# bioinformatics-ua/polus

Measured on AMD Instinct MI355X. Metric: train samples/sec BioBERT-base NER seq256, higher is better.
Workload: dtype bf16; 1 GPU; BERT-base (L=12,H=768,A=12,I=3072,V=28996) token classification C=4, seq_len=256, 64 samples/GPU, AdamW lr 5e-5 wd 0.01 warm-up 10%, dropout 0.1 (hidden + attention) (BASELINE.json configs[2] per-GPU shape), random-init weights; global_batch=64, seq_len=256, parallelism=dp1, grad_allreduce=none

## Files before the change

### include/polus_hip.h

```cpp
#ifndef POLUS_HIP_H
#define POLUS_HIP_H

#include <stddef.h>
#include <stdint.h>

#ifdef __cplusplus
extern "C" {
#endif

#define POLUS_ABI_VERSION 1

enum { POLUS_OK = 0, POLUS_ERR_INVALID = 1, POLUS_ERR_HIP = 2, POLUS_ERR_WORKSPACE = 3 };
enum { POLUS_F32 = 0, POLUS_BF16 = 1 };
enum { POLUS_K_CONTIG = 0, POLUS_K_STRIDED = 1 };
enum { POLUS_ACT_NONE = 0, POLUS_ACT_GELU = 1, POLUS_ACT_SWISH = 2, POLUS_ACT_RELU = 3, POLUS_ACT_TANH = 4 };
enum {
    POLUS_GEMM_ACCUM_C = 1,
    POLUS_GEMM_ACT_FWD = 2,
    POLUS_GEMM_ACT_BWD = 4,
    POLUS_GEMM_DROPOUT = 8
};

const char* polus_last_error(void);
int polus_abi_version(void);
int polus_device_info(int* n_cu, int* lds_bytes_per_cu, char* arch, int arch_len);
int polus_reload_env(void);
int polus_set_reserve_active(int on);
int polus_set_dynamic_params(const void* dev_block16);

size_t polus_gemm_workspace_bytes(int M, int N, int split_k);
int polus_gemm_auto_split(int M, int N, int K);
int polus_gemm(int dtype, int a_layout, int b_layout, int c_dtype,
               const void* A, long lda, const void* B, long ldb, void* C, long ldc,
               int M, int N, int K, float alpha,
               const float* bias, const void* resid, long ldr, void* aux, long ldaux,
               int act, int flags, int split_k, void* workspace, size_t workspace_bytes,
               void* stream);

int polus_gemm_dropout(int dtype, int a_layout, int b_layout, int c_dtype,
                       const void* A, long lda, const void* B, long ldb, void* C, long ldc,
                       int M, int N, int K, float alpha,
                       const float* bias, const void* resid, long ldr, void* aux, long ldaux,
                       int act, int flags, int split_k, void* workspace, size_t workspace_bytes,
                       float drop_p, uint32_t seed, void* stream);
int polus_dropout(int dtype, const void* x, void* y, int64_t n, float drop_p, uint32_t seed, void* stream);
int polus_dropout_mask(uint32_t seed, float drop_p, uint32_t idx0, int64_t n, uint8_t* mask, void* stream);

size_t polus_dense_bwd_params_workspace_bytes(int T, int n_out, int n_in, int split_k);
int polus_dense_bwd_params(int dtype, const void* dY, long lddy, const void* X, long ldx,
                           float* dW, long lddw, float* db, int T, int n_out, int n_in,
                           int accumulate, int split_k, void* workspace, size_t workspace_bytes,
                           void* stream);

typedef struct polus_dw_problem {
    const void* dY; long lddy;
    const void* X;  long ldx;
    float* dW; long lddw;
    float* db;
    int n_out, n_in;
} polus_dw_problem;
size_t polus_dense_bwd_params_grouped_workspace_bytes(int n, const polus_dw_problem* problems, int T, int split_k);
int polus_dense_bwd_params_grouped(int dtype, int n, const polus_dw_problem* problems, int T, int accumulate,
                                   int split_k, void* workspace, size_t workspace_bytes, void* stream);

int polus_dense_thin_supported(int dtype, int H, int C);
int polus_dense_thin_fwd(int dtype, const void* x, long ldx, const void* W, long ldw, const float* bias,
                         int y_dtype, void* y, long ldy, int rows, int H, int C, void* stream);
size_t polus_dense_thin_bwd_workspace_bytes(int dtype, int rows, int H, int C);
int polus_dense_thin_bwd(int dtype, const void* x, long ldx, int dy_dtype, const void* dy, long lddy,
                         const void* W, long ldw, void* dx, long lddx, float* dW, long lddw, float* db,
                         int rows, int H, int C, int accumulate, void* workspace, size_t workspace_bytes, void* stream);

int polus_attention_route(int dtype, int S, int* fwd, int* bwd);
int polus_attention_fwd(int dtype, const void* qkv, const int32_t* mask, void* ctx, float* lse,
                        int B, int S, int n_heads, int head_dim, float drop_p, uint32_t seed, void* stream);
size_t polus_attention_bwd_workspace_bytes(int B, int S, int n_heads);
int polus_attention_bwd(int dtype, const void* qkv, const int32_t* mask, const void* ctx,
                        const void* dctx, const float* lse, void* dqkv,
                        int B, int S, int n_heads, int head_dim, float drop_p, uint32_t seed,
                        void* workspace, size_t workspace_bytes, void* stream);

size_t polus_layernorm_bwd_workspace_bytes(int rows, int H);
int polus_layernorm_fwd(int dtype, const void* x, const float* gamma, const float* beta,
                        void* y, float* mean, float* rstd, int rows, int H, float eps, void* stream);
int polus_layernorm_bwd(int dtype, const void* dy, const void* x, const float* gamma,
                        const float* mean, const float* rstd, void* dx,
                        float* dgamma, float* dbeta, float* dbias, int accumulate,
                        int rows, int H, void* dx_masked, float drop_p, uint32_t seed,
                        void* workspace, size_t workspace_bytes, void* stream);
int polus_layernorm_bwd_finalize(void* workspace, size_t workspace_bytes, int rows, int H, float* dgamma, float* dbeta,
                                 float* dbias, int accumulate, void* stream);

size_t polus_embed_bwd_workspace_bytes(int B, int S, int H);
int polus_embed_ln_fwd(int dtype, const int32_t* ids, const int32_t* type_ids,
                       const float* word, const float* pos, const float* type,
                       const float* gamma, const float* beta, void* y, float* mean, float* rstd,
                       int B, int S, int H, int vocab, int max_pos, int type_vocab, float eps,
                       float drop_p, uint32_t seed, void* stream);
int polus_embed_ln_bwd(int dtype, const void* dy, const int32_t* ids, const int32_t* type_ids,
                       const float* word, const float* pos, const float* type, const float* gamma,
                       const float* mean, const float* rstd,
                       float* gword, float* gpos, float* gtype, float* ggamma, float* gbeta,
                       int accumulate, int deterministic,
                       int B, int S, int H, int vocab, int max_pos, int type_vocab,
                       float drop_p, uint32_t seed,
                       void* workspace, size_t workspace_bytes, void* stream);

size_t polus_colsum_workspace_bytes(int rows, int cols);
int polus_colsum(int dtype, const void* x, long ldx, int rows, int cols, float* out, int accumulate,
                 void* workspace, size_t workspace_bytes, void* stream);

size_t polus_loss_workspace_bytes(int rows);
int polus_softmax_xent(int dtype, const float* logits, long ldl, const int32_t* labels,
                       const float* class_weights, float* loss, void* dlogits, long lddl,
                       int rows, int C, void* workspace, size_t workspace_bytes, void* stream);
int polus_sigmoid_xent(int dtype, const float* logits, long ldl, const float* y_true, long ldy,
                       const float* class_weights, float negative_weight, float* loss,
                       void* dlogits, long lddl, int rows, int C,
                       void* workspace, size_t workspace_bytes, void* stream);

size_t polus_crf_workspace_bytes(int B, int S, int C);
int polus_crf_nll(int dtype, const float* potentials, const int32_t* tags, const int32_t* lengths,
                  const float* trans, const float* sample_w, float* loss, void* dpot,
                  float* dtrans, int accumulate, int B, int S, int C,
                  void* workspace, size_t workspace_bytes, void* stream);
int polus_crf_viterbi(const float* potentials, const int32_t* lengths, const float* trans,
                      int32_t* out_tags, int B, int S, int C,
                      void* workspace, size_t workspace_bytes, void* stream);

int polus_maxsim_fwd(int dtype, const void* Q, const void* D, const int32_t* qmask, const int32_t* dmask,
                     float* score, long lds, int32_t* argmax, int B, int N, int Lq, int Ld, int E, void* stream);
int polus_maxsim_scores(int dtype, const void* Q, const void* D, const int32_t* qmask, const int32_t* dmask,
                        float* score, long lds, int B, int N, int Lq, int Ld, int E, void* stream);
int polus_maxsim_bwd(int dtype, const void* Q, const void* D, const float* dscore, long lds,
                     const int32_t* argmax, void* dQ, void* dD, int B, int N, int Lq, int Ld, int E, void* stream);
int polus_maxsim_rerank(int dtype, const void* Q, const void* D, const int32_t* qmask, const int32_t* dmask,
                        const int32_t* cand, long ldc, float* score, long lds,
                        int B, int C, int N, int Lq, int Ld, int E, void* stream);
int polus_l2norm_fwd(int dtype, const void* x, void* y, float* rnorm, int rows, int E, float eps, void* stream);
int polus_l2norm_bwd(int dtype, const void* y, const float* rnorm, const void* dy, void* dx, int rows, int E,
                     float eps, void* stream);

int polus_topk_merge(const float* scores, long lds, int rows, int n, int32_t id0,
                     float* top_val, int32_t* top_id, int k, int init, void* stream);
int polus_topk_merge_ids(const float* scores, long lds, const int32_t* ids, long ldi, int rows, int n,
                         float* top_val, int32_t* top_id, int k, int init, void* stream);

int polus_argmax(const float* x, long ldx, int32_t* out, int rows, int C, void* stream);

int polus_confusion_matrix(const int32_t* row_idx, const int32_t* col_idx, int64_t n, int C,
                           int32_t* cm, int32_t* rejected, void* stream);

int polus_bio_entity_counts(const int32_t* tags_a, long lda, const int32_t* tags_b, long ldb,
                            const int32_t* mask, long ldm, const int32_t* scheme, int C, int T, int B, int S,
                            int32_t* counts, int32_t* stats, void* stream);
int polus_bio_spans(const int32_t* tags, long ldt, const int32_t* mask, long ldm, const int32_t* scheme, int C,
                    int B, int S, int32_t* spans, int M, int32_t* count, int32_t* rejected, void* stream);

int polus_adam_step(float* p, const float* g, float* m, float* v, void* shadow_bf16,
                    const int64_t* seg, int n_seg, int64_t n,
                    float lr, float lr_t, float beta1, float beta2, float eps, float weight_decay,
                    float grad_scale, const float* clip_scale, void* stream);
size_t polus_sqnorm_workspace_bytes(int64_t n);
int polus_sqnorm(const float* g, int64_t n, float* out, void* workspace, size_t workspace_bytes, void* stream);
int polus_sqnorm_segments(const float* g, const int64_t* seg, int n_seg, float* out,
                          void* workspace, size_t workspace_bytes, void* stream);
int polus_clip_scale(const float* sqnorm, int n_terms, float grad_scale, float clip_norm, float* out_scale, void* stream);
int polus_cast(int src_dtype, const void* src, int dst_dtype, void* dst, int64_t n, void* stream);
int polus_transpose_bf16(const void* src, void* dst, int rows, int cols, void* stream);
int polus_transpose_bf16_batched(const void* src_base, void* dst_base, const void* segs_dev, int nseg,
                                 int total_tiles, void* stream);
int polus_act_bwd(int dtype, const void* dy, const void* u, void* du, int64_t n, int act, void* stream);
int polus_scale(float* x, float a, int64_t n, void* stream);

#define POLUS_COMM_ID_BYTES 128
int polus_comm_unique_id(void* out_id128);
int polus_comm_init(void** comm, int rank, int world, const void* unique_id128);
int polus_comm_destroy(void* comm);
int polus_comm_info(void* comm, int* n_ranks, int* rank, int* device);
int polus_comm_broadcast(void* comm, void* buf, size_t bytes, int root, void* stream);
int polus_comm_allreduce_sum(void* comm, void* buf, size_t count, int dtype, void* stream);
int polus_comm_reduce_scatter_sum(void* comm, const void* send, void* recv, size_t recv_count, int dtype, void* stream);
int polus_comm_all_gather(void* comm, const void* send, void* recv, size_t send_count, int dtype, void* stream);
int polus_comm_group_start(void);
int polus_comm_group_end(void);

#ifdef __cplusplus
}
#endif
#endif
```

### polus_amd/_lib.py

```python
import ctypes
import os

from . import build as _build

F32, BF16 = 0, 1
K_CONTIG, K_STRIDED = 0, 1
ACT_NONE, ACT_GELU, ACT_SWISH, ACT_RELU, ACT_TANH = 0, 1, 2, 3, 4
GEMM_ACCUM_C, GEMM_ACT_FWD, GEMM_ACT_BWD = 1, 2, 4

_c = ctypes
_vp, _i, _l, _f, _sz, _i64, _u32 = _c.c_void_p, _c.c_int, _c.c_long, _c.c_float, _c.c_size_t, _c.c_int64, _c.c_uint32

SIGNATURES = {
    "polus_last_error": (_c.c_char_p, []),
    "polus_abi_version": (_i, []),
    "polus_device_info": (_i, [_c.POINTER(_i), _c.POINTER(_i), _c.c_char_p, _i]),
    "polus_reload_env": (_i, []),
    "polus_set_reserve_active": (_i, [_i]),
    "polus_set_dynamic_params": (_i, [_vp]),
    "polus_gemm_workspace_bytes": (_sz, [_i, _i, _i]),
    "polus_gemm_auto_split": (_i, [_i, _i, _i]),
    "polus_gemm": (_i, [_i, _i, _i, _i, _vp, _l, _vp, _l, _vp, _l, _i, _i, _i, _f,
                        _vp, _vp, _l, _vp, _l, _i, _i, _i, _vp, _sz, _vp]),
    "polus_gemm_dropout": (_i, [_i, _i, _i, _i, _vp, _l, _vp, _l, _vp, _l, _i, _i, _i, _f,
                                _vp, _vp, _l, _vp, _l, _i, _i, _i, _vp, _sz, _f, _u32, _vp]),
    "polus_dropout_mask": (_i, [_u32, _f, _u32, _i64, _vp, _vp]),
    "polus_dropout": (_i, [_i, _vp, _vp, _i64, _f, _u32, _vp]),
    "polus_dense_bwd_params_workspace_bytes": (_sz, [_i, _i, _i, _i]),
    "polus_dense_bwd_params": (_i, [_i, _vp, _l, _vp, _l, _vp, _l, _vp, _i, _i, _i, _i, _i, _vp, _sz, _vp]),
    "polus_attention_route": (_i, [_i, _i, _c.POINTER(_i), _c.POINTER(_i)]),
    "polus_attention_fwd": (_i, [_i, _vp, _vp, _vp, _vp, _i, _i, _i, _i, _f, _u32, _vp]),
    "polus_attention_bwd_workspace_bytes": (_sz, [_i, _i, _i]),
    "polus_attention_bwd": (_i, [_i, _vp, _vp, _vp, _vp, _vp, _vp, _i, _i, _i, _i, _f, _u32, _vp, _sz, _vp]),
    "polus_layernorm_bwd_workspace_bytes": (_sz, [_i, _i]),
    "polus_layernorm_fwd": (_i, [_i, _vp, _vp, _vp, _vp, _vp, _vp, _i, _i, _f, _vp]),
    "polus_layernorm_bwd": (_i, [_i, _vp, _vp, _vp, _vp, _vp, _vp, _vp, _vp, _vp, _i, _i, _i, _vp, _f, _u32, _vp, _sz, _vp]),
    "polus_layernorm_bwd_finalize": (_i, [_vp, _sz, _i, _i, _vp, _vp, _vp, _i, _vp]),
    "polus_embed_bwd_workspace_bytes": (_sz, [_i, _i, _i]),
    "polus_embed_ln_fwd": (_i, [_i, _vp, _vp, _vp, _vp, _vp, _vp, _vp, _vp, _vp, _vp,
                                _i, _i, _i, _i, _i, _i, _f, _f, _u32, _vp]),
    "polus_embed_ln_bwd": (_i, [_i, _vp, _vp, _vp, _vp, _vp, _vp, _vp, _vp, _vp,
                                _vp, _vp, _vp, _vp, _vp, _i, _i,
                                _i, _i, _i, _i, _i, _i, _f, _u32, _vp, _sz, _vp]),
    "polus_colsum_workspace_bytes": (_sz, [_i, _i]),
    "polus_colsum": (_i, [_i, _vp, _l, _i, _i, _vp, _i, _vp, _sz, _vp]),
    "polus_loss_workspace_bytes": (_sz, [_i]),
    "polus_softmax_xent": (_i, [_i, _vp, _l, _vp, _vp, _vp, _vp, _l, _i, _i, _vp, _sz, _vp]),
    "polus_sigmoid_xent": (_i, [_i, _vp, _l, _vp, _l, _vp, _f, _vp, _vp, _l, _i, _i, _vp, _sz, _vp]),
    "polus_crf_workspace_bytes": (_sz, [_i, _i, _i]),
    "polus_crf_nll": (_i, [_i, _vp, _vp, _vp, _vp, _vp, _vp, _vp, _vp, _i, _i, _i, _i, _vp, _sz, _vp]),
    "polus_crf_viterbi": (_i, [_vp, _vp, _vp, _vp, _i, _i, _i, _vp, _sz, _vp]),
    "polus_confusion_matrix": (_i, [_vp, _vp, _i64, _i, _vp, _vp, _vp]),
    "polus_bio_entity_counts": (_i, [_vp, _l, _vp, _l, _vp, _l, _vp, _i, _i, _i, _i, _vp, _vp, _vp]),
    "polus_bio_spans": (_i, [_vp, _l, _vp, _l, _vp, _i, _i, _i, _vp, _i, _vp, _vp, _vp]),
    "polus_maxsim_fwd": (_i, [_i, _vp, _vp, _vp, _vp, _vp, _l, _vp, _i, _i, _i, _i, _i, _vp]),
    "polus_maxsim_scores": (_i, [_i, _vp, _vp, _vp, _vp, _vp, _l, _i, _i, _i, _i, _i, _vp]),
    "polus_maxsim_rerank": (_i, [_i, _vp, _vp, _vp, _vp, _vp, _l, _vp, _l, _i, _i, _i, _i, _i, _i, _vp]),
    "polus_maxsim_bwd": (_i, [_i, _vp, _vp, _vp, _l, _vp, _vp, _vp, _i, _i, _i, _i, _i, _vp]),
    "polus_l2norm_fwd": (_i, [_i, _vp, _vp, _vp, _i, _i, _f, _vp]),
    "polus_l2norm_bwd": (_i, [_i, _vp, _vp, _vp, _vp, _i, _i, _f, _vp]),
    "polus_topk_merge": (_i, [_vp, _l, _i, _i, _c.c_int32, _vp, _vp, _i, _i, _vp]),
    "polus_topk_merge_ids": (_i, [_vp, _l, _vp, _l, _i, _i, _vp, _vp, _i, _i, _vp]),
    "polus_argmax": (_i, [_vp, _l, _vp, _i, _i, _vp]),
    "polus_adam_step": (_i, [_vp, _vp, _vp, _vp, _vp, _vp, _i, _i64,
                             _f, _f, _f, _f, _f, _f, _f, _vp, _vp]),
    "polus_sqnorm_workspace_bytes": (_sz, [_i64]),
    "polus_sqnorm": (_i, [_vp, _i64, _vp, _vp, _sz, _vp]),
    "polus_sqnorm_segments": (_i, [_vp, _vp, _i, _vp, _vp, _sz, _vp]),
    "polus_clip_scale": (_i, [_vp, _i, _f, _f, _vp, _vp]),
    "polus_cast": (_i, [_i, _vp, _i, _vp, _i64, _vp]),
    "polus_scale": (_i, [_vp, _f, _i64, _vp]),
    "polus_act_bwd": (_i, [_i, _vp, _vp, _vp, _i64, _i, _vp]),
    "polus_transpose_bf16": (_i, [_vp, _vp, _i, _i, _vp]),
    "polus_transpose_bf16_batched": (_i, [_vp, _vp, _vp, _i, _i, _vp]),
    "polus_dense_bwd_params_grouped_workspace_bytes": (_sz, [_i, _vp, _i, _i]),
    "polus_dense_bwd_params_grouped": (_i, [_i, _i, _vp, _i, _i, _i, _vp, _sz, _vp]),
    "polus_dense_thin_supported": (_i, [_i, _i, _i]),
    "polus_dense_thin_fwd": (_i, [_i, _vp, _l, _vp, _l, _vp, _i, _vp, _l, _i, _i, _i, _vp]),
    "polus_dense_thin_bwd_workspace_bytes": (_sz, [_i, _i, _i, _i]),
    "polus_dense_thin_bwd": (_i, [_i, _vp, _l, _i, _vp, _l, _vp, _l, _vp, _l, _vp, _l, _vp, _i, _i, _i, _i, _vp, _sz, _vp]),
    "polus_comm_unique_id": (_i, [_vp]),
    "polus_comm_init": (_i, [_c.POINTER(_vp), _i, _i, _vp]),
    "polus_comm_destroy": (_i, [_vp]),
    "polus_comm_info": (_i, [_vp, _c.POINTER(_i), _c.POINTER(_i), _c.POINTER(_i)]),
    "polus_comm_broadcast": (_i, [_vp, _vp, _sz, _i, _vp]),
    "polus_comm_allreduce_sum": (_i, [_vp, _vp, _sz, _i, _vp]),
    "polus_comm_reduce_scatter_sum": (_i, [_vp, _vp, _vp, _sz, _i, _vp]),
    "polus_comm_all_gather": (_i, [_vp, _vp, _vp, _sz, _i, _vp]),
    "polus_comm_group_start": (_i, []),
    "polus_comm_group_end": (_i, []),
}


class DwProblem(ctypes.Structure):
    _fields_ = [("dY", ctypes.c_void_p), ("lddy", ctypes.c_long), ("X", ctypes.c_void_p), ("ldx", ctypes.c_long),
                ("dW", ctypes.c_void_p), ("lddw", ctypes.c_long), ("db", ctypes.c_void_p),
                ("n_out", ctypes.c_int), ("n_in", ctypes.c_int)]


class PolusHipError(RuntimeError):
    pass


_LIB = None


def load():
    global _LIB
    if _LIB is not None:
        return _LIB
    path = _build.lib_path()
    if not os.path.exists(path):
        raise PolusHipError(
            f"{path} is missing: build it with `python -m polus_amd.build` "
            "(or __graft_entry__.build()). There is no CPU fallback for the training path.")
    import torch
    bundled = os.path.join(os.path.dirname(torch.__file__), "lib", "libamdhip64.so")
    if os.path.exists(bundled):
        ctypes.CDLL(bundled, mode=ctypes.RTLD_GLOBAL)
    lib = ctypes.CDLL(path)
    for name, (res, args) in SIGNATURES.items():
        fn = getattr(lib, name)
        fn.restype = res
        fn.argtypes = args
    if lib.polus_abi_version() != 1:
        raise PolusHipError("libpolus_hip.so ABI version mismatch")
    _LIB = lib
    return lib


def check(rc, what=""):
    if rc != 0:
        msg = load().polus_last_error()
        raise PolusHipError(f"{what} failed (code {rc}): {msg.decode() if msg else ''}")


def ptr(t):
    return None if t is None else t.data_ptr()


_CUR_STREAM = [None]


def current_stream():
    h = _CUR_STREAM[0]
    if h is not None:
        return h
    import torch
    return torch.cuda.current_stream().cuda_stream


class pinned_stream:

    def __enter__(self):
        import torch
        self._prev = _CUR_STREAM[0]
        if self._prev is None and torch.cuda.is_available():
            _CUR_STREAM[0] = torch.cuda.current_stream().cuda_stream
        return self

    def __exit__(self, *exc):
        _CUR_STREAM[0] = self._prev
        return False


class stream_scope:

    def __init__(self, stream):
        import torch
        self._stream = stream
        self._ctx = torch.cuda.stream(stream)

    def __enter__(self):
        self._prev = _CUR_STREAM[0]
        self._ctx.__enter__()
        if self._prev is not None:
            _CUR_STREAM[0] = self._stream.cuda_stream
        return self

    def __exit__(self, *exc):
        _CUR_STREAM[0] = self._prev
        return self._ctx.__exit__(*exc)


def dtype_code(torch_dtype):
    import torch
    if torch_dtype == torch.float32:
        return F32
    if torch_dtype == torch.bfloat16:
        return BF16
    raise PolusHipError(f"unsupported dtype {torch_dtype}")
```

### polus_amd/csrc/gemm.hip

```cpp
#include <stdlib.h>
#include "gemm_common.h"

using namespace pgemm;

namespace {

constexpr int BM = 128, BN = 128, NTHREADS = 256;
constexpr int KC_STRIDE = 160;
constexpr int OPERAND_BYTES = 128 * KC_STRIDE;
constexpr int SMEM_BYTES = 4 * OPERAND_BYTES;

template <typename T> struct Cfg;
template <> struct Cfg<bf16_t> {
    static constexpr int BK = 64, EPC = 8, NSUB = 2;
    static constexpr int KS_STRIDE = 288, KS_SWZ = 7, LOG_RCH = 4;
};
template <> struct Cfg<float> {
    static constexpr int BK = 32, EPC = 4, NSUB = 1;
    static constexpr int KS_STRIDE = 512, KS_SWZ = 6, LOG_RCH = 5;
};

typedef unsigned int u32x4_t __attribute__((ext_vector_type(4)));
template <typename T> union Chunk { uint4 u; u32x4_t w; T e[16 / sizeof(T)]; };

// ... 374 lines not shown
                     const float* bias, const void* resid, long ldr, void* aux, long ldaux,
                     int act, int flags, int split_k, void* workspace, size_t workspace_bytes,
                     float drop_p, uint32_t seed, void* stream) {
    POLUS_REQUIRE(dtype == POLUS_F32 || dtype == POLUS_BF16, "polus_gemm: bad dtype %d", dtype);
    POLUS_REQUIRE(c_dtype == POLUS_F32 || c_dtype == dtype, "polus_gemm: c_dtype must be f32 or dtype");
    POLUS_REQUIRE(M > 0 && N > 0 && K > 0, "polus_gemm: empty problem M=%d N=%d K=%d", M, N, K);
    POLUS_REQUIRE(A && B && C, "polus_gemm: null operand");
    POLUS_REQUIRE((a_layout | 1) == 1 && (b_layout | 1) == 1, "polus_gemm: bad layout");
    POLUS_REQUIRE(lda >= (a_layout == POLUS_K_CONTIG ? K : M), "polus_gemm: lda %ld too small", lda);
    POLUS_REQUIRE(ldb >= (b_layout == POLUS_K_CONTIG ? K : N), "polus_gemm: ldb %ld too small", ldb);
    POLUS_REQUIRE(ldc >= N, "polus_gemm: ldc %ld < N %d", ldc, N);
    POLUS_REQUIRE(!resid || ldr >= N, "polus_gemm: ldr too small");
    POLUS_REQUIRE(!((flags & POLUS_GEMM_ACT_BWD) && !aux), "polus_gemm: ACT_BWD needs aux");
    POLUS_REQUIRE(!aux || ldaux >= N, "polus_gemm: ldaux too small");
    if (split_k < 1) split_k = 1;
    const size_t es = polus_dtype_size(dtype), ecs = polus_dtype_size(c_dtype);
    const int bk = dtype == POLUS_BF16 ? 64 : 32;
    const int nkt = (K + bk - 1) / bk;
    if (split_k > nkt) split_k = nkt;
    const bool both_kc = a_layout == POLUS_K_CONTIG && b_layout == POLUS_K_CONTIG;
    if (split_k > 1) {
        const bool epi = resid || aux || (flags & (POLUS_GEMM_ACT_FWD | POLUS_GEMM_ACT_BWD | POLUS_GEMM_DROPOUT));
        POLUS_REQUIRE(!epi || (dtype == POLUS_BF16 && c_dtype == POLUS_BF16 && both_kc && !(flags & POLUS_GEMM_ACCUM_C)),
                      "polus_gemm: split_k with a residual / activation / dropout epilogue needs bf16 K-contiguous operands and a bf16 C");
        if (!workspace || workspace_bytes < polus_gemm_workspace_bytes(M, N, split_k)) {
            polus_set_error("polus_gemm: workspace %zu < %zu", workspace_bytes, polus_gemm_workspace_bytes(M, N, split_k));
            return POLUS_ERR_WORKSPACE;
        }
    }
    POLUS_REQUIRE(!(flags & POLUS_GEMM_DROPOUT) || (both_kc && c_dtype == dtype), "polus_gemm_dropout: needs K-contiguous operands and c_dtype == dtype");
    GemmArgs a = {};
    a.A = A; a.B = B; a.C = C; a.lda = lda; a.ldb = ldb; a.ldc = ldc;
    a.M = M; a.N = N; a.K = K; a.alpha = alpha;
    a.bias = bias; a.resid = resid; a.ldr = ldr; a.aux = aux; a.ldaux = ldaux;
    a.act = act; a.flags = flags;
    a.drop_inv = 1.0f / (1.0f - drop_p); a.drop_thresh = polus_drop_thresh(drop_p); a.drop_seed = seed;
    a.dyn = polus_dyn();
    const int epc = (int)(16 / es);
    a.a_vec = polus_aligned16(A) && ((lda * es) % 16 == 0) && ((a_layout == POLUS_K_CONTIG ? K : M) % epc == 0);
    a.b_vec = polus_aligned16(B) && ((ldb * es) % 16 == 0) && ((b_layout == POLUS_K_CONTIG ? K : N) % epc == 0);
    bool ev = (((uintptr_t)C) % (4 * ecs) == 0) && (ldc % 4 == 0);
    if (bias) ev = ev && (((uintptr_t)bias) % 16 == 0);
    if (resid) ev = ev && (((uintptr_t)resid) % (4 * es) == 0) && (ldr % 4 == 0);
    if (aux) ev = ev && (((uintptr_t)aux) % (4 * es) == 0) && (ldaux % 4 == 0);
    a.epi_vec = ev;
    bool ev16 = (((uintptr_t)C) % 16 == 0) && ((ldc * ecs) % 16 == 0);
    if (bias) ev16 = ev16 && (((uintptr_t)bias) % 16 == 0);
    if (resid) ev16 = ev16 && (((uintptr_t)resid) % 16 == 0) && ((ldr * es) % 16 == 0);
    if (aux) ev16 = ev16 && (((uintptr_t)aux) % 16 == 0) && ((ldaux * es) % 16 == 0);
    a.epi_vec16 = ev16 && dtype == POLUS_BF16;
    a.order = polus_cfg().gemm_order;

    const int kt_per_split = (nkt + split_k - 1) / split_k;
    const bool c_is_f32 = c_dtype == POLUS_F32;
    const int a_ks = a_layout == POLUS_K_STRIDED, b_ks = b_layout == POLUS_K_STRIDED;
    const GemmRoute r = gemm_route(a, dtype, c_is_f32, a_ks, b_ks, (nkt + kt_per_split - 1) / kt_per_split);
    if (r.splits > 1) { a.k_per_split = kt_per_split * bk; a.partial = static_cast<float*>(workspace); }
    else a.k_per_split = r.kernel == GEMM_V1 ? nkt * bk : ((K + 31) / 32) * 32;

    hipStream_t st = static_cast<hipStream_t>(stream);
    int rc = POLUS_ERR_INVALID;
    switch (r.kernel) {
        case GEMM_V1: rc = launch_v1(dtype, c_dtype, a_layout, b_layout, a, r.drop, r.splits, st); break;
        case GEMM_RING:
            rc = r.splits > 1 ? polus_launch_gemm_ring(slab_args(a), 1, a_ks, b_ks, r.splits, -1, st)
                              : polus_launch_gemm_ring(a, c_is_f32, a_ks, b_ks, 1, r.mode, st);
            break;
        case GEMM_RING128: rc = polus_launch_gemm_ring128(a, r.mode, r.drop, st); break;
        case GEMM_RING_DROP: rc = polus_launch_gemm_ring_dropout(a, r.mode, st); break;
        case GEMM_PP:
        case GEMM_PP_PERSIST: rc = polus_launch_gemm_pp(a, r.mode, r.drop, r.tn, r.persist_cus, st); break;
    }
    if (rc != POLUS_OK) return rc;
    switch (r.reduce) {
        case REDUCE_NONE: break;
        case REDUCE_EPI: return launch_splitk_reduce_epi(a, r.splits, st);
        case REDUCE_PLAIN:
            return launch_splitk_reduce(c_dtype, a.partial, r.splits, M, N, C, ldc, alpha, bias, (flags & POLUS_GEMM_ACCUM_C) ? 1 : 0,
                                        "polus_gemm(splitk_reduce)", st);
    }
    return POLUS_OK;
}

extern "C" int polus_gemm(int dtype, int a_layout, int b_layout, int c_dtype,
                          const void* A, long lda, const void* B, long ldb, void* C, long ldc,
                          int M, int N, int K, float alpha,
                          const float* bias, const void* resid, long ldr, void* aux, long ldaux,
                          int act, int flags, int split_k, void* workspace, size_t workspace_bytes,
                          void* stream) {
    POLUS_REQUIRE(!(flags & POLUS_GEMM_DROPOUT), "polus_gemm: use polus_gemm_dropout for POLUS_GEMM_DROPOUT");
    return gemm_impl(dtype, a_layout, b_layout, c_dtype, A, lda, B, ldb, C, ldc, M, N, K, alpha, bias, resid, ldr,
                     aux, ldaux, act, flags, split_k, workspace, workspace_bytes, 0.0f, 0u, stream);
}

extern "C" int polus_gemm_dropout(int dtype, int a_layout, int b_layout, int c_dtype,
                                  const void* A, long lda, const void* B, long ldb, void* C, long ldc,
                                  int M, int N, int K, float alpha,
                                  const float* bias, const void* resid, long ldr, void* aux, long ldaux,
                                  int act, int flags, int split_k, void* workspace, size_t workspace_bytes,
                                  float drop_p, uint32_t seed, void* stream) {
    POLUS_REQUIRE(drop_p >= 0.0f && drop_p < 1.0f, "polus_gemm_dropout: need 0 <= p < 1 (got %f)", drop_p);
    POLUS_REQUIRE((long)M * N < (1LL << 32), "polus_gemm_dropout: M*N must fit 32 bits");
    if (drop_p > 0.0f) flags |= POLUS_GEMM_DROPOUT; else flags &= ~POLUS_GEMM_DROPOUT;
    return gemm_impl(dtype, a_layout, b_layout, c_dtype, A, lda, B, ldb, C, ldc, M, N, K, alpha, bias, resid, ldr,
                     aux, ldaux, act, flags, split_k, workspace, workspace_bytes, drop_p, seed, stream);
}

extern "C" size_t polus_dense_bwd_params_workspace_bytes(int T, int n_out, int n_in, int split_k) {
    if (split_k < 1) split_k = 1;
    size_t slabs = split_k > 1 ? (size_t)split_k * n_out * n_in * sizeof(float) : 0;
    size_t cs = (size_t)split_k * n_out * sizeof(float);
    size_t fallback = polus_colsum_workspace_bytes(T, n_out);
    return slabs + (cs > fallback ? cs : fallback) + 256;
}

namespace {
__global__ void colsum_splits_kernel(const float* __restrict__ partial, int splits, int n, float* __restrict__ out, int accumulate) {
    int c = blockIdx.x * blockDim.x + threadIdx.x;
    if (c >= n) return;
    float s = 0.f;
    for (int z = 0; z < splits; ++z) s += partial[(long)z * n + c];
    out[c] = accumulate ? out[c] + s : s;
}
}

static int launch_colsum_splits(const float* partial, int splits, int n, float* out, int accumulate, const char* what, hipStream_t st) {
    hipLaunchKernelGGL(colsum_splits_kernel, dim3((n + 255) / 256), dim3(256), 0, st, partial, splits, n, out, accumulate);
    POLUS_CHECK_LAUNCH(what);
    return POLUS_OK;
}

static GemmArgs dw_args(const polus_dw_problem& q, int T, int kps, float* colsum) {
    GemmArgs a = {};
    a.A = q.dY; a.B = q.X; a.lda = q.lddy; a.ldb = q.ldx;
    a.M = q.n_out; a.N = q.n_in; a.K = T; a.alpha = 1.0f;
    a.k_per_split = kps;
    a.a_vec = a.b_vec = 1;
    a.colsum_a = colsum;
    return a;
}
static void dw_dest(GemmArgs& a, const polus_dw_problem& q, void* slabs, int accumulate) {
    if (slabs) {
        a.C = slabs; a.ldc = q.n_in; a.c_split_stride = (long)q.n_out * q.n_in;
        a.epi_vec = a.epi_vec16 = (q.n_in % 4 == 0);
    } else {
        a.C = q.dW; a.ldc = q.lddw; a.flags = accumulate ? POLUS_GEMM_ACCUM_C : 0;
        a.epi_vec = a.epi_vec16 = polus_aligned16(q.dW) && (q.lddw % 4 == 0);
    }
}

extern "C" int polus_dense_bwd_params(int dtype, const void* dY, long lddy, const void* X, long ldx,
                                      float* dW, long lddw, float* db, int T, int n_out, int n_in,
                                      int accumulate, int split_k, void* workspace, size_t workspace_bytes,
                                      void* stream) {
    POLUS_REQUIRE(dY && X && dW, "polus_dense_bwd_params: null pointer");
    POLUS_REQUIRE(T > 0 && n_out > 0 && n_in > 0, "polus_dense_bwd_params: bad shape");
    if (split_k < 1) split_k = 1;
    size_t need = polus_dense_bwd_params_workspace_bytes(T, n_out, n_in, split_k);
    if (!workspace || workspace_bytes < need) { polus_set_error("polus_dense_bwd_params: workspace %zu < %zu", workspace_bytes, need); return POLUS_ERR_WORKSPACE; }
    hipStream_t st = static_cast<hipStream_t>(stream);
    const size_t es = polus_dtype_size(dtype);
    const int bk = dtype == POLUS_BF16 ? 64 : 32;
    int nkt = (T + bk - 1) / bk;
    if (split_k > nkt) split_k = nkt;
    const size_t slab_bytes = split_k > 1 ? (((size_t)split_k * n_out * n_in * sizeof(float) + 255) / 256) * 256 : 0;
    unsigned char* ws = static_cast<unsigned char*>(workspace);
    float* cs_ws = reinterpret_cast<float*>(ws + slab_bytes);
    const bool vec = polus_aligned16(dY) && polus_aligned16(X) && ((lddy * es) % 16 == 0) && ((ldx * es) % 16 == 0) &&
                     (n_out % (16 / es) == 0) && (n_in % (16 / es) == 0);
    const bool ring = dtype == POLUS_BF16 && vec && n_out >= 256 && n_in >= 128 && db != nullptr && !polus_cfg().gemm_v1;
    if (!ring) {
        int rc = polus_gemm(dtype, POLUS_K_STRIDED, POLUS_K_STRIDED, POLUS_F32, dY, lddy, X, ldx, dW, lddw, n_out, n_in, T,
                            1.0f, nullptr, nullptr, 0, nullptr, 0, 0, accumulate ? POLUS_GEMM_ACCUM_C : 0, split_k,
                            ws, slab_bytes, stream);
        if (rc != POLUS_OK || !db) return rc;
        return polus_colsum(dtype, dY, lddy, T, n_out, db, accumulate, cs_ws, workspace_bytes - slab_bytes, stream);
    }
    const polus_dw_problem q = {dY, lddy, X, ldx, dW, lddw, db, n_out, n_in};
    const int kt_per_split = (nkt + split_k - 1) / split_k;
    const int splits = (nkt + kt_per_split - 1) / kt_per_split;
    GemmArgs a = dw_args(q, T, kt_per_split * bk, cs_ws);
    dw_dest(a, q, splits > 1 ? ws : nullptr, accumulate);
    int rc = polus_launch_gemm_ring(a, 1, 1, 1, splits, -1, st);
    if (rc != POLUS_OK) return rc;
    if (splits > 1) {
        rc = launch_splitk_reduce(POLUS_F32, reinterpret_cast<const float*>(ws), splits, n_out, n_in, dW, lddw, 1.0f, nullptr,
                                  accumulate ? 1 : 0, "polus_dense_bwd_params(reduce)", st);
        if (rc != POLUS_OK) return rc;
    }
    return launch_colsum_splits(cs_ws, splits, n_out, db, accumulate ? 1 : 0, "polus_dense_bwd_params(colsum)", st);
}

static bool grouped_use_pp(int n, const polus_dw_problem* pr, int T) {
    if (polus_cfg().gemm_pp < 0 || T % 64 != 0) return false;
    for (int k = 0; k < n; ++k)
        if (pr[k].n_out < 256 || pr[k].n_in < 256) return false;
    return true;
}

static bool grouped_sk_plan(int n, const polus_dw_problem* pr, int T, int split_k, bool pp, PPKSSKPlan* pl) {
    if (!polus_cfg().dw_streamk || split_k > 0 || !pp) return false;
    int no[POLUS_MAX_GROUP], ni[POLUS_MAX_GROUP];
    for (int k = 0; k < n; ++k) { no[k] = pr[k].n_out; ni[k] = pr[k].n_in; }
    int ncu = polus_num_cus() - polus_reserved_cus();
    if (polus_cfg().dw_sk_cus > 0 && polus_cfg().dw_sk_cus < ncu) ncu = polus_cfg().dw_sk_cus;
    return polus_ppks_sk_plan(no, ni, n, T, ncu, polus_cfg().dw_sk_delta, pl) != 0;
}

static void grouped_splits(int n, const polus_dw_problem* pr, int T, int split_k, int* splits, bool pp) {
    const int nkt = (T + 63) / 64;
    int tiles[POLUS_MAX_GROUP], total = 0;
    for (int k = 0; k < n; ++k) {
        tiles[k] = pp ? polus_ppks_tiles(pr[k].n_out, pr[k].n_in) : ((pr[k].n_out + 255) / 256) * ((pr[k].n_in + 127) / 128);
        total += tiles[k];
    }
    if (split_k > 0) {
        for (int k = 0; k < n; ++k) splits[k] = split_k < nkt ? split_k : nkt;
        return;
    }
    const int slots_xcd = (pp ? 1 : 2) * polus_num_cus() / 8;
    int per_xcd[POLUS_MAX_GROUP], total_xcd = 0;
    for (int k = 0; k < n; ++k) { per_xcd[k] = (tiles[k] + 7) / 8; total_xcd += per_xcd[k]; }
    int base = slots_xcd / (total_xcd > 0 ? total_xcd : 1);
    if (base < 1) base = 1;
    const int cap = nkt / 4 > 0 ? nkt / 4 : 1;
    if (base > cap) base = cap;
    int used = 0;
    for (int k = 0; k < n; ++k) { splits[k] = base; used += per_xcd[k] * base; }
    bool given[POLUS_MAX_GROUP] = {false};
    for (;;) {
        int best = -1;
        for (int k = 0; k < n; ++k)
            if (!given[k] && splits[k] < cap && used + per_xcd[k] <= slots_xcd && (best < 0 || tiles[k] > tiles[best])) best = k;
        if (best < 0) break;
        given[best] = true; ++splits[best]; used += per_xcd[best];
    }
}

struct GroupedDwPlan {
    bool pp, sk;
    int splits[POLUS_MAX_GROUP];
    int kps[POLUS_MAX_GROUP], eff[POLUS_MAX_GROUP];
    size_t slab_off[POLUS_MAX_GROUP], cs_off[POLUS_MAX_GROUP];
    PPKSSKPlan skp;
    size_t sk_cs_off[POLUS_MAX_GROUP];
    size_t bytes;
};

static void grouped_dw_plan(int n, const polus_dw_problem* pr, int T, int split_k, GroupedDwPlan* pl) {
    pl->pp = grouped_use_pp(n, pr, T);
    grouped_splits(n, pr, T, split_k, pl->splits, pl->pp);
    const int nkt = (T + 63) / 64;
    size_t off = 0, single = 0;
    for (int k = 0; k < n; ++k) {
        const int sk = pl->splits[k] > nkt ? nkt : pl->splits[k];
        pl->kps[k] = ((nkt + sk - 1) / sk) * 64;
        pl->eff[k] = (nkt + (pl->kps[k] / 64) - 1) / (pl->kps[k] / 64);
        pl->slab_off[k] = off;
        if (pl->splits[k] > 1) off += (((size_t)pl->splits[k] * pr[k].n_out * pr[k].n_in * sizeof(float) + 255) / 256) * 256;
        pl->cs_off[k] = off;
        off += (((size_t)pl->splits[k] * pr[k].n_out * sizeof(float) + 255) / 256) * 256;
        const size_t b = polus_dense_bwd_params_workspace_bytes(T, pr[k].n_out, pr[k].n_in, pl->splits[k]);
        if (b > single) single = b;
    }
    pl->bytes = off + 256;
    pl->sk = grouped_sk_plan(n, pr, T, split_k, pl->pp, &pl->skp);
    if (pl->sk) {
        off = (size_t)pl->skp.ttot * pl->skp.slots * 256 * 256 * sizeof(float);
        for (int k = 0; k < n; ++k) {
            pl->sk_cs_off[k] = off;
            off += (((size_t)pl->skp.slots * pr[k].n_out * sizeof(float) + 255) / 256) * 256;
        }
        if (off + 256 > pl->bytes) pl->bytes = off + 256;
    }
    if (single > pl->bytes) pl->bytes = single;
}

extern "C" size_t polus_dense_bwd_params_grouped_workspace_bytes(int n, const polus_dw_problem* problems, int T, int split_k) {
    if (n < 1 || n > POLUS_MAX_GROUP || !problems || T < 1) return 0;
    GroupedDwPlan pl;
    grouped_dw_plan(n, problems, T, split_k, &pl);
    return pl.bytes;
}

struct DwGroupOut {
    const float* slabs[POLUS_MAX_GROUP]; float* cs[POLUS_MAX_GROUP];
    float* dW[POLUS_MAX_GROUP]; float* db[POLUS_MAX_GROUP];
    long lddw[POLUS_MAX_GROUP]; int n_out[POLUS_MAX_GROUP], n_in[POLUS_MAX_GROUP];
    bool aligned;
};
static DwGroupOut dw_group_out(int n, const polus_dw_problem* pr, unsigned char* ws, const size_t* cs_off, const size_t* slab_off, const int* eff) {
    DwGroupOut o;
    o.aligned = true;
    for (int k = 0; k < n; ++k) {
        const polus_dw_problem& q = pr[k];
        o.slabs[k] = slab_off && eff[k] > 1 ? reinterpret_cast<const float*>(ws + slab_off[k]) : nullptr;
        o.cs[k] = q.db ? reinterpret_cast<float*>(ws + cs_off[k]) : nullptr;
        o.dW[k] = q.dW; o.db[k] = q.db; o.lddw[k] = q.lddw; o.n_out[k] = q.n_out; o.n_in[k] = q.n_in;
        o.aligned = o.aligned && (q.n_in % 4 == 0) && (q.lddw % 4 == 0) && polus_aligned16(q.dW);
    }
    return o;
}

extern "C" int polus_dense_bwd_params_grouped(int dtype, int n, const polus_dw_problem* problems, int T, int accumulate,
                                              int split_k, void* workspace, size_t workspace_bytes, void* stream) {
    POLUS_REQUIRE(problems && n >= 1 && n <= POLUS_MAX_GROUP && T > 0, "polus_dense_bwd_params_grouped: bad arguments");
    const size_t es = polus_dtype_size(dtype);
    bool ring = dtype == POLUS_BF16 && !polus_cfg().gemm_v1 && !polus_cfg().dw_ungrouped;
    for (int k = 0; k < n; ++k) {
        const polus_dw_problem& q = problems[k];
        POLUS_REQUIRE(q.dY && q.X && q.dW && q.n_out > 0 && q.n_in > 0, "polus_dense_bwd_params_grouped: problem %d: bad arguments", k);
        ring = ring && polus_aligned16(q.dY) && polus_aligned16(q.X) && ((q.lddy * es) % 16 == 0) && ((q.ldx * es) % 16 == 0) &&
               (q.n_out % 8 == 0) && (q.n_in % 8 == 0) && q.n_out >= 256 && q.n_in >= 128;
    }
    GroupedDwPlan pl;
    grouped_dw_plan(n, problems, T, split_k, &pl);
    if (!workspace || workspace_bytes < pl.bytes) { polus_set_error("polus_dense_bwd_params_grouped: workspace %zu < %zu", workspace_bytes, pl.bytes); return POLUS_ERR_WORKSPACE; }
    if (!ring) {
        for (int k = 0; k < n; ++k) {
            const polus_dw_problem& q = problems[k];
            int rc;
            if (q.db) rc = polus_dense_bwd_params(dtype, q.dY, q.lddy, q.X, q.ldx, q.dW, q.lddw, q.db, T, q.n_out, q.n_in,
                                                  accumulate, pl.splits[k], workspace, workspace_bytes, stream);
            else rc = polus_gemm(dtype, POLUS_K_STRIDED, POLUS_K_STRIDED, POLUS_F32, q.dY, q.lddy, q.X, q.ldx, q.dW, q.lddw,
                                 q.n_out, q.n_in, T, 1.0f, nullptr, nullptr, 0, nullptr, 0, 0, accumulate ? POLUS_GEMM_ACCUM_C : 0,
                                 pl.splits[k], workspace, workspace_bytes, stream);
            if (rc != POLUS_OK) return rc;
        }
        return POLUS_OK;
    }
    hipStream_t st = static_cast<hipStream_t>(stream);
    unsigned char* ws = static_cast<unsigned char*>(workspace);
    GemmArgs ga[POLUS_MAX_GROUP];
    if (pl.sk) {
        const DwGroupOut o = dw_group_out(n, problems, ws, pl.sk_cs_off, nullptr, nullptr);
        if (o.aligned) {
            for (int k = 0; k < n; ++k) {
                ga[k] = dw_args(problems[k], T, 0, nullptr);
                ga[k].epi_vec = ga[k].epi_vec16 = 1;
            }
            int rc = polus_launch_gemm_ppks_sk(ga, pl.skp, reinterpret_cast<float*>(ws), o.cs, st);
            if (rc != POLUS_OK) return rc;
            return polus_launch_dw_group_reduce_sk(pl.skp, reinterpret_cast<const float*>(ws), o.cs, o.dW, o.db, o.lddw, o.n_out, o.n_in, accumulate ? 1 : 0, st);
        }
    }
    const DwGroupOut o = dw_group_out(n, problems, ws, pl.cs_off, pl.slab_off, pl.eff);
    for (int k = 0; k < n; ++k) {
        ga[k] = dw_args(problems[k], T, pl.kps[k], o.cs[k]);
        dw_dest(ga[k], problems[k], pl.eff[k] > 1 ? ws + pl.slab_off[k] : nullptr, accumulate);
    }
    int rc = pl.pp ? polus_launch_gemm_ppks_grouped_dw(ga, n, pl.eff, st) : polus_launch_gemm_ring_grouped_dw(ga, n, pl.eff, st);
    if (rc != POLUS_OK) return rc;
    if (polus_cfg().dw_fused_reduce && o.aligned)
        return polus_launch_dw_group_reduce(n, o.slabs, o.cs, o.dW, o.db, o.lddw, o.n_out, o.n_in, pl.eff, accumulate ? 1 : 0, st);
    for (int k = 0; k < n; ++k) {
        const polus_dw_problem& q = problems[k];
        if (pl.eff[k] > 1) {
            rc = launch_splitk_reduce(POLUS_F32, o.slabs[k], pl.eff[k], q.n_out, q.n_in, q.dW, q.lddw, 1.0f, nullptr, accumulate ? 1 : 0,
                                      "polus_dense_bwd_params_grouped(reduce)", st);
            if (rc != POLUS_OK) return rc;
        }
        if (q.db) {
            rc = launch_colsum_splits(o.cs[k], pl.eff[k], q.n_out, q.db, accumulate ? 1 : 0, "polus_dense_bwd_params_grouped(colsum)", st);
            if (rc != POLUS_OK) return rc;
        }
    }
    return POLUS_OK;
}
```

### polus_amd/csrc/gemm_common.h

```cpp
#pragma once
#include <type_traits>
#include "common.h"

namespace pgemm {

struct GemmArgs {
    const void* A; const void* B; void* C;
    long lda, ldb, ldc;
    int M, N, K;
    int k_per_split;
    float alpha;
    const float* bias;
    const void* resid; long ldr;
    void* aux; long ldaux;
    int act, flags;
    float* partial;
    int a_vec, b_vec, epi_vec;
    int epi_vec16;
    float drop_inv;
    unsigned drop_thresh, drop_seed;
    float* colsum_a;
    long c_split_stride;
    int unused0, unused1;
    int order;
// ... 160 lines not shown
                float* dst = reinterpret_cast<float*>(C) + m * p.ldc + ncol;
                *reinterpret_cast<float4*>(dst) = make_float4(v[0], v[1], v[2], v[3]);
                *reinterpret_cast<float4*>(dst + 4) = make_float4(v[4], v[5], v[6], v[7]);
            } else {
                bf16x8_t t;
#pragma unroll
                for (int r = 0; r < 8; ++r) t[r] = (bf16_t)v[r];
                *reinterpret_cast<bf16x8_t*>(reinterpret_cast<T*>(C) + m * p.ldc + ncol) = t;
            }
        }
      }
    }
}


template <int WN> struct EpiCfg {
    static constexpr int RS = WN * 4 + 16;
    static constexpr int BYTES = 9 * RS;
    static constexpr int SLOTS = 8 * (WN / 8);
    static constexpr int PASSES = (SLOTS + 63) / 64;
};
template <bool AGPR> __device__ __forceinline__ f32x4 acc_take(f32x4& acc) {
    if (AGPR) asm volatile("" : "+a"(acc) :: "memory");
    else asm volatile("" : "+v"(acc) :: "memory");
    return acc;
}
template <typename TC, int WN, bool DROP, int MODE, bool AGPR, int DEPTH_ = 0>
__device__ __forceinline__ void epilogue_wave(const GemmArgs& p, f32x4 (&acc)[8][WN / 16], int mb, int nb,
                                              int lane, unsigned char* lds) {
    typedef bf16_t T;
    constexpr int NT = WN / 16, RS = EpiCfg<WN>::RS, PASSES = EpiCfg<WN>::PASSES, CPR = 2 * NT;
    const int i = lane & 15, g = lane >> 4;
    const bool interior = p.epi_vec16 && (mb + 128 <= p.M) && (nb + WN <= p.N);
    if (!interior) {
#pragma clang loop unroll(full)
        for (int mt = 0; mt < 8; ++mt)
#pragma clang loop unroll(full)
            for (int nt = 0; nt < NT; ++nt)
                epilogue_tile<T, TC, DROP>(p, acc_take<AGPR>(acc[mt][nt]), mb + mt * 16 + i, nb + nt * 16 + 4 * g, 0);
        return;
    }
    constexpr bool act_fwd = MODE == 1, act_bwd = MODE == 3, accum = false, has_resid = MODE == 2;
    const T* resid = static_cast<const T*>(p.resid);
    T* aux = static_cast<T*>(p.aux);
    TC* C = static_cast<TC*>(p.C);
    constexpr int SLOTS = EpiCfg<WN>::SLOTS;
    int prow[PASSES], pcol[PASSES];
    float bv[PASSES][8];
#pragma unroll
    for (int ps = 0; ps < PASSES; ++ps) {
        const int slot = (ps * 64 + lane) % SLOTS;
        prow[ps] = slot / CPR;
        pcol[ps] = 8 * (slot % CPR);
        if (p.bias) {
            load4<float>(p.bias + nb + pcol[ps], *reinterpret_cast<float(*)[4]>(&bv[ps][0]));
            load4<float>(p.bias + nb + pcol[ps] + 4, *reinterpret_cast<float(*)[4]>(&bv[ps][4]));
        } else {
#pragma unroll
            for (int r = 0; r < 8; ++r) bv[ps][r] = 0.f;
        }
    }
    constexpr int DEPTH = DEPTH_ > 0 ? DEPTH_ : (AGPR ? 1 : 4), NBUF = DEPTH + 1;
    bf16x8_t pre[NBUF][2][PASSES];
    auto fetch = [&](int mt, bf16x8_t (&dst)[2][PASSES]) {
        const T* base = has_resid ? resid : static_cast<const T*>(aux);
        const long ld = has_resid ? p.ldr : p.ldaux;
#pragma unroll
        for (int h = 0; h < 2; ++h)
#pragma unroll
            for (int ps = 0; ps < PASSES; ++ps)
                dst[h][ps] = *reinterpret_cast<const bf16x8_t*>(base + (long)(mb + mt * 16 + h * 8 + prow[ps]) * ld + nb + pcol[ps]);
    };
    if (has_resid || act_bwd) {
#pragma unroll
        for (int d = 0; d < DEPTH; ++d) fetch(d, pre[d % NBUF]);
    }
#pragma clang loop unroll(full)
    for (int mt = 0; mt < 8; ++mt) {
        f32x4 t[NT];
#pragma unroll
        for (int nt = 0; nt < NT; ++nt) t[nt] = acc_take<AGPR>(acc[mt][nt]);
        if ((has_resid || act_bwd) && mt + DEPTH < 8) fetch(mt + DEPTH, pre[(mt + DEPTH) % NBUF]);
#pragma clang loop unroll(full)
        for (int h = 0; h < 2; ++h) {
            {
                unsigned char* wrow = lds + (((i >> 3) == h) ? (i & 7) : 8) * RS;
#pragma unroll
                for (int nt = 0; nt < NT; ++nt)
                    *reinterpret_cast<f32x4*>(wrow + (nt * 16 + 4 * g) * 4) = t[nt];
            }
#pragma clang loop unroll(full)
            for (int ps = 0; ps < PASSES; ++ps) {
                const long m = mb + mt * 16 + h * 8 + prow[ps];
                const int ncol = nb + pcol[ps];
                const unsigned char* src = lds + prow[ps] * RS + pcol[ps] * 4;
                f32x4 lo = *reinterpret_cast<const f32x4*>(src), hi = *reinterpret_cast<const f32x4*>(src + 16);
                float v[8] = {lo[0], lo[1], lo[2], lo[3], hi[0], hi[1], hi[2], hi[3]};
#pragma unroll
                for (int r = 0; r < 8; ++r) v[r] = v[r] * p.alpha + bv[ps][r];
                if (act_fwd) {
                    if (aux) {
                        bf16x8_t tt;
#pragma unroll
                        for (int r = 0; r < 8; ++r) tt[r] = (bf16_t)v[r];
                        __builtin_nontemporal_store(tt, reinterpret_cast<bf16x8_t*>(aux + m * p.ldaux + ncol));
                    }
                    apply_act_n<8, true>(p.act, v);
                }
                if (act_bwd) {
                    float u[8];
#pragma unroll
                    for (int r = 0; r < 8; ++r) u[r] = (float)pre[mt % NBUF][h][ps][r];
                    apply_act_grad_n<8, true>(p.act, v, u);
                }
                if (DROP) {
                    const unsigned base = (unsigned)m * (unsigned)p.N + (unsigned)ncol;
                    polus_dropout_run<8>(v, p.drop_seed, base, p.drop_thresh, p.drop_inv, (p.N & 3) == 0);
                }
                if (has_resid) {
#pragma unroll
                    for (int r = 0; r < 8; ++r) v[r] += (float)pre[mt % NBUF][h][ps][r];
                }
                if (sizeof(TC) == 4) {
                    float* dst = reinterpret_cast<float*>(C) + m * p.ldc + ncol;
                    *reinterpret_cast<float4*>(dst) = make_float4(v[0], v[1], v[2], v[3]);
                    *reinterpret_cast<float4*>(dst + 4) = make_float4(v[4], v[5], v[6], v[7]);
                } else {
                    bf16x8_t tt;
#pragma unroll
                    for (int r = 0; r < 8; ++r) tt[r] = (bf16_t)v[r];
                    *reinterpret_cast<bf16x8_t*>(reinterpret_cast<T*>(C) + m * p.ldc + ncol) = tt;
                }
            }
        }
    }
}

template <int WN> struct EpiDbCfg {
    static constexpr int RS = EpiCfg<WN>::RS;
    static constexpr int BUF = 16 * RS;
    static constexpr int BYTES = 2 * BUF;
};
template <typename TC, int WN, bool DROP, int MODE, int MT = 8>
__device__ __forceinline__ void epilogue_wave_db(const GemmArgs& p, f32x4 (&acc)[MT][WN / 16], int mb, int nb,
                                                 int lane, unsigned char* lds) {
    typedef bf16_t T;
    constexpr int NT = WN / 16, RS = EpiDbCfg<WN>::RS, BUF = EpiDbCfg<WN>::BUF, PASSES = EpiCfg<WN>::PASSES, CPR = 2 * NT;
    constexpr int SLOTS = EpiCfg<WN>::SLOTS;
    const int i = lane & 15, g = lane >> 4;
    const bool interior = p.epi_vec16 && (mb + 16 * MT <= p.M) && (nb + WN <= p.N);
    if (!interior) {
#pragma clang loop unroll(full)
        for (int mt = 0; mt < MT; ++mt)
#pragma clang loop unroll(full)
            for (int nt = 0; nt < NT; ++nt)
                epilogue_tile<T, TC, DROP>(p, acc_take<false>(acc[mt][nt]), mb + mt * 16 + i, nb + nt * 16 + 4 * g, 0);
        return;
    }
    constexpr bool act_fwd = MODE == 1, act_bwd = MODE == 3, has_resid = MODE == 2;
    const T* resid = static_cast<const T*>(p.resid);
    T* aux = static_cast<T*>(p.aux);
    TC* C = static_cast<TC*>(p.C);
    int prow[PASSES], pcol[PASSES];
    float bv[PASSES][8];
#pragma unroll
    for (int ps = 0; ps < PASSES; ++ps) {
        const int slot = (ps * 64 + lane) % SLOTS;
        prow[ps] = slot / CPR;
        pcol[ps] = 8 * (slot % CPR);
        if (p.bias) {
            load4<float>(p.bias + nb + pcol[ps], *reinterpret_cast<float(*)[4]>(&bv[ps][0]));
            load4<float>(p.bias + nb + pcol[ps] + 4, *reinterpret_cast<float(*)[4]>(&bv[ps][4]));
        } else {
#pragma unroll
            for (int r = 0; r < 8; ++r) bv[ps][r] = 0.f;
        }
    }
    constexpr int DEPTH = MT < 4 ? MT : 4, NBUF = DEPTH + 1;
    bf16x8_t pre[NBUF][2][PASSES];
    auto fetch = [&](int mt, bf16x8_t (&dst)[2][PASSES]) {
        const T* base = has_resid ? resid : static_cast<const T*>(aux);
        const long ld = has_resid ? p.ldr : p.ldaux;
#pragma unroll
        for (int h = 0; h < 2; ++h)
#pragma unroll
            for (int ps = 0; ps < PASSES; ++ps)
                dst[h][ps] = *reinterpret_cast<const bf16x8_t*>(base + (long)(mb + mt * 16 + h * 8 + prow[ps]) * ld + nb + pcol[ps]);
    };
    auto stage = [&](int mt) {
        unsigned char* wrow = lds + (mt & 1) * BUF + i * RS;
#pragma unroll
        for (int nt = 0; nt < NT; ++nt)
            *reinterpret_cast<f32x4*>(wrow + (nt * 16 + 4 * g) * 4) = acc_take<false>(acc[mt][nt]);
    };
    if (has_resid || act_bwd) {
#pragma unroll
        for (int d = 0; d < DEPTH; ++d) fetch(d, pre[d % NBUF]);
    }
    stage(0);
    stage(1);
#pragma clang loop unroll(full)
    for (int mt = 0; mt < MT; ++mt) {
        f32x4 lo[2][PASSES], hi[2][PASSES];
#pragma unroll
        for (int h = 0; h < 2; ++h)
#pragma unroll
            for (int ps = 0; ps < PASSES; ++ps) {
                const unsigned char* src = lds + (mt & 1) * BUF + (h * 8 + prow[ps]) * RS + pcol[ps] * 4;
                lo[h][ps] = *reinterpret_cast<const f32x4*>(src);
                hi[h][ps] = *reinterpret_cast<const f32x4*>(src + 16);
            }
        if (mt + 2 < MT) stage(mt + 2);
        if ((has_resid || act_bwd) && mt + DEPTH < MT) fetch(mt + DEPTH, pre[(mt + DEPTH) % NBUF]);
#pragma clang loop unroll(full)
        for (int h = 0; h < 2; ++h) {
#pragma clang loop unroll(full)
            for (int ps = 0; ps < PASSES; ++ps) {
                const long m = mb + mt * 16 + h * 8 + prow[ps];
                const int ncol = nb + pcol[ps];
                float v[8] = {lo[h][ps][0], lo[h][ps][1], lo[h][ps][2], lo[h][ps][3], hi[h][ps][0], hi[h][ps][1], hi[h][ps][2], hi[h][ps][3]};
#pragma unroll
                for (int r = 0; r < 8; ++r) v[r] = v[r] * p.alpha + bv[ps][r];
                if (act_fwd) {
                    if (aux) {
                        bf16x8_t tt;
#pragma unroll
                        for (int r = 0; r < 8; ++r) tt[r] = (bf16_t)v[r];
                        __builtin_nontemporal_store(tt, reinterpret_cast<bf16x8_t*>(aux + m * p.ldaux + ncol));
                    }
                    apply_act_n<8, true>(p.act, v);
                }
                if (act_bwd) {
                    float u[8];
#pragma unroll
                    for (int r = 0; r < 8; ++r) u[r] = (float)pre[mt % NBUF][h][ps][r];
                    apply_act_grad_n<8, true>(p.act, v, u);
                }
                if (DROP) {
                    const unsigned base = (unsigned)m * (unsigned)p.N + (unsigned)ncol;
                    polus_dropout_run<8>(v, p.drop_seed, base, p.drop_thresh, p.drop_inv, (p.N & 3) == 0);
                }
                if (has_resid) {
#pragma unroll
                    for (int r = 0; r < 8; ++r) v[r] += (float)pre[mt % NBUF][h][ps][r];
                }
                if (sizeof(TC) == 4) {
                    float* dst = reinterpret_cast<float*>(C) + m * p.ldc + ncol;
                    *reinterpret_cast<float4*>(dst) = make_float4(v[0], v[1], v[2], v[3]);
                    *reinterpret_cast<float4*>(dst + 4) = make_float4(v[4], v[5], v[6], v[7]);
                } else {
                    bf16x8_t tt;
#pragma unroll
                    for (int r = 0; r < 8; ++r) tt[r] = (bf16_t)v[r];
                    *reinterpret_cast<bf16x8_t*>(reinterpret_cast<T*>(C) + m * p.ldc + ncol) = tt;
                }
            }
        }
    }
}


__device__ __forceinline__ int xcd_remap(int bid, int nwg) {
    int xcd = bid & 7, q = nwg >> 3, r8 = nwg & 7;
    return (xcd < r8 ? xcd * (q + 1) : r8 * (q + 1) + (xcd - r8) * q) + (bid >> 3);
}

__device__ __forceinline__ void tile_of(int bid, int nwg, int tiles_n, int order, int& row, int& col) {
    const int per = nwg >> 3;
    if (order > 0 && (nwg & 7) == 0 && per % tiles_n == 0 && tiles_n % order == 0 && tiles_n > order) {
        const int xcd = bid & 7, j = bid >> 3, R = per / tiles_n, blk = R * order;
        const int b = j / blk, jj = j - b * blk;
        row = xcd * R + jj / order;
        col = b * order + jj % order;
        return;
    }
    const int wg = xcd_remap(bid, nwg);
    row = wg / tiles_n;
    col = wg - row * tiles_n;
}

}

template <typename F> int polus_dispatch_epi(int mode, int drop, F&& f) {
    typedef std::false_type no_drop;
    switch (mode) {
        case 0: return f(no_drop(), std::integral_constant<int, 0>());
        case 1: return f(no_drop(), std::integral_constant<int, 1>());
        case 2: return drop ? f(std::true_type(), std::integral_constant<int, 2>()) : f(no_drop(), std::integral_constant<int, 2>());
        case 3: return f(no_drop(), std::integral_constant<int, 3>());
    }
    return POLUS_ERR_INVALID;
}
int polus_launch_gemm_ring(const pgemm::GemmArgs& a, int c_is_f32, int a_ks, int b_ks, int splits, int mode, hipStream_t st);
int polus_launch_gemm_ring128(const pgemm::GemmArgs& a, int mode, int drop, hipStream_t st);
#define POLUS_MAX_GROUP 8
int polus_launch_gemm_ring_grouped_dw(const pgemm::GemmArgs* probs, int n, const int* splits, hipStream_t st);
int polus_launch_gemm_ring_dropout(const pgemm::GemmArgs& a, int mode, hipStream_t st);
int polus_launch_gemm_pp(const pgemm::GemmArgs& a, int mode, int drop, int tn, int persist_cus, hipStream_t st);
int polus_ppks_tiles(int n_out, int n_in);
int polus_launch_gemm_ppks_grouped_dw(const pgemm::GemmArgs* probs, int n, const int* splits, hipStream_t st);
int polus_launch_dw_group_reduce(int n, const float* const* slabs, const float* const* cs, float* const* dW, float* const* db,
                                 const long* lddw, const int* n_out, const int* n_in, const int* splits, int accumulate,
                                 hipStream_t st);

struct PPKSSKPlan {
    int tiles[POLUS_MAX_GROUP], tile0[POLUS_MAX_GROUP + 1], unit0[POLUS_MAX_GROUP + 1];
    int n, base, kr, krem, R, q_units, rem_units, slots, grid, ttot;
};
int polus_ppks_sk_plan(const int* n_out, const int* n_in, int n, int T, int ncu, int delta, PPKSSKPlan* pl);
int polus_launch_gemm_ppks_sk(const pgemm::GemmArgs* probs, const PPKSSKPlan& pl, float* slabs, float* const* cs, hipStream_t st);
int polus_launch_dw_group_reduce_sk(const PPKSSKPlan& pl, const float* slabs, const float* const* cs, float* const* dW, float* const* db,
                                    const long* lddw, const int* n_out, const int* n_in, int accumulate, hipStream_t st);
```

### polus_amd/csrc/optim.hip

```cpp
#include "common.h"

namespace {

constexpr int SEG_CHUNK_ELEMS = 1 << 14;

struct AdamArgs {
    float* p; const float* g; float* m; float* v; bf16_t* shadow;
    const int64_t* seg; int n_seg;
    float lr, lr_t, b1, b2, eps, wd, gscale;
    const float* clip;
    const PolusDyn* dyn;
};

__global__ __launch_bounds__(256) void adam_kernel(AdamArgs a) {
    if (a.dyn) { a.lr = a.dyn->lr; a.lr_t = a.dyn->lr_t; }
    const float gs = a.gscale * (a.clip ? *a.clip : 1.0f);
    for (int s = blockIdx.x; s < a.n_seg; s += gridDim.x) {
        const int64_t beg = a.seg[3 * s], end = a.seg[3 * s + 1], flags = a.seg[3 * s + 2];
        const float decay = (flags & 1) ? a.lr * a.wd : 0.0f;
        const bool shadow = (flags & 2) && a.shadow;
        int64_t body = (beg + 3) & ~(int64_t)3;
        if (body > end) body = end;
        const int64_t body_end = body + ((end - body) & ~(int64_t)3);
        for (int64_t i = beg + threadIdx.x; i < body; i += 256) {
            float g = a.g[i] * gs, p = a.p[i], m = a.m[i], v = a.v[i];
            p -= decay * p;
            m = a.b1 * m + (1.0f - a.b1) * g;
            v = a.b2 * v + (1.0f - a.b2) * g * g;
            p -= a.lr_t * m / (sqrtf(v) + a.eps);
            a.p[i] = p; a.m[i] = m; a.v[i] = v;
            if (shadow) a.shadow[i] = (bf16_t)p;
        }
        for (int64_t i = body + 4 * (int64_t)threadIdx.x; i < body_end; i += 4 * 256) {
            float4 g4 = *reinterpret_cast<const float4*>(a.g + i);
            float4 p4 = *reinterpret_cast<float4*>(a.p + i);
            float4 m4 = *reinterpret_cast<float4*>(a.m + i);
            float4 v4 = *reinterpret_cast<float4*>(a.v + i);
            float g[4] = {g4.x * gs, g4.y * gs, g4.z * gs, g4.w * gs};
            float p[4] = {p4.x, p4.y, p4.z, p4.w}, m[4] = {m4.x, m4.y, m4.z, m4.w}, v[4] = {v4.x, v4.y, v4.z, v4.w};
#pragma unroll
            for (int e = 0; e < 4; ++e) {
                p[e] -= decay * p[e];
                m[e] = a.b1 * m[e] + (1.0f - a.b1) * g[e];
                v[e] = a.b2 * v[e] + (1.0f - a.b2) * g[e] * g[e];
                p[e] -= a.lr_t * m[e] / (sqrtf(v[e]) + a.eps);
            }
            *reinterpret_cast<float4*>(a.p + i) = make_float4(p[0], p[1], p[2], p[3]);
            *reinterpret_cast<float4*>(a.m + i) = make_float4(m[0], m[1], m[2], m[3]);
            *reinterpret_cast<float4*>(a.v + i) = make_float4(v[0], v[1], v[2], v[3]);
            if (shadow) store4<bf16_t>(a.shadow + i, p);
        }
        for (int64_t i = body_end + threadIdx.x; i < end; i += 256) {
            float g = a.g[i] * gs, p = a.p[i], m = a.m[i], v = a.v[i];
            p -= decay * p;
            m = a.b1 * m + (1.0f - a.b1) * g;
            v = a.b2 * v + (1.0f - a.b2) * g * g;
            p -= a.lr_t * m / (sqrtf(v) + a.eps);
            a.p[i] = p; a.m[i] = m; a.v[i] = v;
            if (shadow) a.shadow[i] = (bf16_t)p;
        }
    }
}

__global__ __launch_bounds__(256) void sqnorm_partial_kernel(const float* __restrict__ g, int64_t n, float* __restrict__ partial) {
    __shared__ float red[4];
    float s = 0.f;
    int64_t i = ((int64_t)blockIdx.x * 256 + threadIdx.x) * 4;
    const int64_t stride = (int64_t)gridDim.x * 256 * 4;
    for (; i < n; i += stride) {
        if (i + 4 <= n) {
            float4 v = *reinterpret_cast<const float4*>(g + i);
            s += (v.x * v.x + v.y * v.y) + (v.z * v.z + v.w * v.w);
        } else {
            for (int64_t j = i; j < n; ++j) s += g[j] * g[j];
        }
    }
    s = wave_sum(s);
    if ((threadIdx.x & 63) == 0) red[threadIdx.x >> 6] = s;
    __syncthreads();
    if (threadIdx.x == 0) partial[blockIdx.x] = (red[0] + red[1]) + (red[2] + red[3]);
}

__global__ __launch_bounds__(256) void sqnorm_seg_kernel(const float* __restrict__ g, const int64_t* __restrict__ seg, int n_seg,
                                                         float* __restrict__ partial) {
    __shared__ float red[4];
    float s = 0.f;
    for (int k = blockIdx.x; k < n_seg; k += gridDim.x) {
        const int64_t b = seg[3 * k], e = seg[3 * k + 1];
        for (int64_t i = b + threadIdx.x; i < e; i += 256) s += g[i] * g[i];
    }
    s = wave_sum(s);
    if ((threadIdx.x & 63) == 0) red[threadIdx.x >> 6] = s;
    __syncthreads();
    if (threadIdx.x == 0) partial[blockIdx.x] = (red[0] + red[1]) + (red[2] + red[3]);
}

__global__ void sqnorm_final_kernel(const float* __restrict__ partial, int n, float* __restrict__ out) {
    __shared__ float red[256];
    float s = 0.f;
    for (int k = threadIdx.x; k < n; k += 256) s += partial[k];
    red[threadIdx.x] = s;
    __syncthreads();
    if (threadIdx.x == 0) {
        float t = 0.f;
        for (int k = 0; k < 256; ++k) t += red[k];
        *out = t;
    }
}

__global__ void clip_scale_kernel(const float* __restrict__ sq, int n, float gscale, float clip, float* __restrict__ out) {
    float t = 0.f;
    for (int k = 0; k < n; ++k) t += sq[k];
    float norm = sqrtf(t) * fabsf(gscale);
    *out = clip / fmaxf(norm, clip);
}

int sq_blocks(int64_t n) {
    int64_t b = (n / 4 + 255) / 256;
    return (int)(b < 1 ? 1 : (b > 1024 ? 1024 : b));
}

}

extern "C" int polus_adam_step(float* p, const float* g, float* m, float* v, void* shadow_bf16,
                               const int64_t* seg, int n_seg, int64_t n,
                               float lr, float lr_t, float beta1, float beta2, float eps, float weight_decay,
                               float grad_scale, const float* clip_scale, void* stream) {
    POLUS_REQUIRE(p && g && m && v && seg && n_seg > 0 && n > 0, "polus_adam_step: bad arguments");
    POLUS_REQUIRE(polus_aligned16(p) && polus_aligned16(g) && polus_aligned16(m) && polus_aligned16(v),
                  "polus_adam_step: arenas must be 16-byte aligned");
    POLUS_REQUIRE(!shadow_bf16 || ((uintptr_t)shadow_bf16 % 8) == 0, "polus_adam_step: shadow must be 8-byte aligned");
    AdamArgs a;
    a.p = p; a.g = g; a.m = m; a.v = v; a.shadow = static_cast<bf16_t*>(shadow_bf16);
    a.seg = seg; a.n_seg = n_seg;
    a.dyn = polus_dyn();
    a.lr = lr; a.lr_t = lr_t; a.b1 = beta1; a.b2 = beta2; a.eps = eps; a.wd = weight_decay;
    a.gscale = grad_scale; a.clip = clip_scale;
    int blocks = n_seg < 4096 ? n_seg : 4096;
    hipLaunchKernelGGL(adam_kernel, dim3(blocks), dim3(256), 0, static_cast<hipStream_t>(stream), a);
    POLUS_CHECK_LAUNCH("polus_adam_step");
    return POLUS_OK;
}

extern "C" size_t polus_sqnorm_workspace_bytes(int64_t n) { return (size_t)sq_blocks(n) * sizeof(float); }

extern "C" int polus_sqnorm(const float* g, int64_t n, float* out, void* workspace, size_t workspace_bytes, void* stream) {
    POLUS_REQUIRE(g && out && n > 0 && polus_aligned16(g), "polus_sqnorm: bad arguments");
    if (!workspace || workspace_bytes < polus_sqnorm_workspace_bytes(n)) { polus_set_error("polus_sqnorm: workspace too small"); return POLUS_ERR_WORKSPACE; }
    hipStream_t st = static_cast<hipStream_t>(stream);
    int blocks = sq_blocks(n);
    hipLaunchKernelGGL(sqnorm_partial_kernel, dim3(blocks), dim3(256), 0, st, g, n, static_cast<float*>(workspace));
    POLUS_CHECK_LAUNCH("polus_sqnorm(partial)");
    hipLaunchKernelGGL(sqnorm_final_kernel, dim3(1), dim3(256), 0, st, static_cast<const float*>(workspace), blocks, out);
    POLUS_CHECK_LAUNCH("polus_sqnorm(final)");
    return POLUS_OK;
}

extern "C" int polus_sqnorm_segments(const float* g, const int64_t* seg, int n_seg, float* out,
                                     void* workspace, size_t workspace_bytes, void* stream) {
    POLUS_REQUIRE(g && seg && out && n_seg > 0, "polus_sqnorm_segments: bad arguments");
    const int blocks = n_seg < 1024 ? n_seg : 1024;
    if (!workspace || workspace_bytes < (size_t)1024 * sizeof(float)) { polus_set_error("polus_sqnorm_segments: workspace too small"); return POLUS_ERR_WORKSPACE; }
    hipStream_t st = static_cast<hipStream_t>(stream);
    hipLaunchKernelGGL(sqnorm_seg_kernel, dim3(blocks), dim3(256), 0, st, g, seg, n_seg, static_cast<float*>(workspace));
    POLUS_CHECK_LAUNCH("polus_sqnorm_segments(partial)");
    hipLaunchKernelGGL(sqnorm_final_kernel, dim3(1), dim3(256), 0, st, static_cast<const float*>(workspace), blocks, out);
    POLUS_CHECK_LAUNCH("polus_sqnorm_segments(final)");
    return POLUS_OK;
}

extern "C" int polus_clip_scale(const float* sqnorm, int n_terms, float grad_scale, float clip_norm, float* out_scale, void* stream) {
    POLUS_REQUIRE(sqnorm && out_scale && clip_norm > 0.f && n_terms > 0, "polus_clip_scale: bad arguments");
    hipLaunchKernelGGL(clip_scale_kernel, dim3(1), dim3(1), 0, static_cast<hipStream_t>(stream), sqnorm, n_terms, grad_scale, clip_norm, out_scale);
    POLUS_CHECK_LAUNCH("polus_clip_scale");
    return POLUS_OK;
}
```

### polus_amd/layers.py

```python
import math
import os
import zlib

import numpy as np
import torch

from . import ops
from .tensor import DeviceScalar, to_device


class Layer:
    name = "layer"

    def build(self, arena, in_features, prefix):
        return in_features

    def variables(self):
        return []

    def forward(self, x, training=False):
        raise NotImplementedError

    def backward(self, dy, accumulate=False):
        raise NotImplementedError

    def _buf(self, key, shape, dtype, dev):
        cache = self.__dict__.setdefault("_bufs", {})
        t = cache.get(key)
        if t is None or t.shape != tuple(shape) or t.dtype != dtype:
            t = cache[key] = torch.empty(tuple(shape), dtype=dtype, device=dev)
        return t


def dw_split_k(out_rows, out_cols, contraction):
    tiles = ((out_rows + 255) // 256) * ((out_cols + 127) // 128)
    want = max(1, 512 // max(tiles, 1))
    return int(max(1, min(want, contraction // 256, 64)))


def dw_group_split_k(shapes, contraction):
    tiles = sum((((o + 255) // 256) * ((i + 127) // 128) + 7) // 8 * 8 for o, i in shapes)
    want = max(1, 512 // max(tiles, 1))
    return int(max(1, min(want, contraction // 256, 64)))


def dense_bwd_params_group(problems, accumulate=False):
    T = problems[0][0].shape[0]
    if problems[0][0].dtype == torch.bfloat16 and os.environ.get("POLUS_DW_UNGROUPED") is None:
        return ops.dense_bwd_params_grouped(problems, accumulate, 0)
    for dy, x, dw, db in problems:
        sk = dw_split_k(dy.shape[1], x.shape[1], T)
        if db is not None:
            ops.dense_bwd_params(dy, x, dw, db, accumulate, sk)
        else:
            ops.gemm(dy, x, dw, a_layout=ops.K_STRIDED, b_layout=ops.K_STRIDED,
                     flags=ops.GEMM_ACCUM_C if accumulate else 0, split_k=sk)


def gemm_dx(dy, w, dx, **kw):
    wt = w.compute_t
    if wt is not None:
        return ops.gemm(dy, wt, dx, split_k="auto", **kw)
    return ops.gemm(dy, w.compute, dx, b_layout=ops.K_STRIDED, **kw)


def glorot_uniform(rng, fan_in, fan_out, shape):
    lim = math.sqrt(6.0 / (fan_in + fan_out))
    return rng.uniform(-lim, lim, size=shape).astype(np.float32)


class Flatten(Layer):

    def __init__(self, input_shape=None):
        self.input_shape = input_shape

    def build(self, arena, in_features, prefix):
        if self.input_shape is not None:
            return int(np.prod(self.input_shape))
        return in_features

    def forward(self, x, training=False):
        self._shape = x.shape
        return x.reshape(x.shape[0], -1)

    def backward(self, dy, accumulate=False):
        return dy.reshape(self._shape)


class Dropout(Layer):
    _instances = 0

    def __init__(self, rate=0.0, input_shape=None, seed=None):
        self.rate = float(rate)
        if not 0.0 <= self.rate < 1.0:
            raise ValueError("dropout rate must be in [0, 1)")
        Dropout._instances += 1
        self.seed = (seed if seed is not None else 7919 * Dropout._instances) & 0xFFFFFFFF
        self.calls = 0
        self._active = None

    def forward(self, x, training=False):
        if not training or self.rate == 0.0:
            self._active = None
            return x
        self.calls += 1
        s = (self.seed + 0x9E3779B1 * self.calls) & 0xFFFFFFFF
        xc = x.contiguous()
        y = self._buf("y", xc.shape, xc.dtype, xc.device)
        ops.dropout(xc, y, self.rate, s)
        self._active = s
        return y

    def backward(self, dy, accumulate=False):
        if self._active is None:
            return dy
        dyc = dy.contiguous()
        dx = self._buf("dx", dyc.shape, dyc.dtype, dyc.device)
        ops.dropout(dyc, dx, self.rate, self._active)
        return dx


class Dense(Layer):

    def __init__(self, units, activation=None, input_shape=None, use_bias=True, out_dtype=None, name=None):
        self.units = int(units)
        self.activation = activation if activation not in ("linear",) else None
        self.input_shape = input_shape
        self.use_bias = use_bias
        self.out_dtype = out_dtype
        self.name = name or "dense"

    def build(self, arena, in_features, prefix):
        if in_features is None:
            in_features = self.input_shape[-1]
        self.in_features = int(in_features)
        rng = np.random.Generator(np.random.PCG64(zlib.crc32(f"{prefix}:{self.units}:{self.in_features}".encode())))
        self.w = arena.add(prefix + ".w", (self.units, self.in_features),
                           glorot_uniform(rng, self.in_features, self.units, (self.units, self.in_features)),
                           decay=True, matrix=True)
        self.b = arena.add(prefix + ".b", (self.units,), np.zeros(self.units, np.float32), decay=False) if self.use_bias else None
        self.arena = arena
        return self.units

    def variables(self):
        return [self.w] + ([self.b] if self.b is not None else [])

    def forward(self, x, training=False):
        lead = x.shape[:-1]
        x2 = x.reshape(-1, x.shape[-1])
        assert x2.shape[1] == self.in_features, f"{self.name}: expected {self.in_features} features, got {x2.shape[1]}"
        rows = x2.shape[0]
        odt = self.out_dtype or x2.dtype
        y = self._buf("y", (rows, self.units), odt, x2.device)
        bias = self.b.value if self.b is not None else None
        self._thin = (not self.activation and x2.is_cuda and x2.stride(1) == 1 and
                      (x2.data_ptr() % 16 == 0) and ((x2.stride(0) * x2.element_size()) % 16 == 0) and
                      os.environ.get("POLUS_DENSE_THIN", "1") != "0" and ops.dense_thin_supported(x2.dtype, self.in_features, self.units))
        if self._thin:
            ops.dense_thin_fwd(x2, self.w.compute, bias, y)
            self._x = x2
            return y.view(*lead, self.units)
        if self.activation:
            assert odt == x2.dtype, "an activated Dense keeps the compute dtype"
            u = self._buf("u", (rows, self.units), x2.dtype, x2.device)
            ops.gemm(x2, self.w.compute, y, bias=bias, aux=u, act=self.activation, flags=ops.GEMM_ACT_FWD, split_k="auto")
            self._u = u
        else:
            ops.gemm(x2, self.w.compute, y, bias=bias, split_k="auto")
        self._x = x2
        return y.view(*lead, self.units)

    def backward(self, dy, accumulate=False, need_dx=True, dx_resid=None):
        x = self._x
        dy2 = dy.reshape(-1, self.units)
        if getattr(self, "_thin", False) and dx_resid is None and dy2.dtype in (x.dtype, torch.float32):
            rows = x.shape[0]
            dx = self._buf("dx", (rows, self.in_features), x.dtype, x.device) if need_dx else None
            ops.dense_thin_bwd(x, dy2 if dy2.stride(1) == 1 else dy2.contiguous(), self.w.compute, dx, self.w.grad,
                               self.b.grad if self.b is not None else None, accumulate)
            return dx
        if dy2.dtype != x.dtype:
            d = self._buf("dy_cast", dy2.shape, x.dtype, x.device)
            ops.cast(dy2.contiguous(), d)
            dy2 = d
        if self.activation:
            du = self._buf("du", dy2.shape, x.dtype, x.device)
            ops.act_bwd(dy2.contiguous(), self._u, du, self.activation)
            dy2 = du
        rows = x.shape[0]
        acc = ops.GEMM_ACCUM_C if accumulate else 0
        ops.dense_bwd_params(dy2.contiguous() if dy2.stride(1) != 1 else dy2, x, self.w.grad,
                             self.b.grad if self.b is not None else None, accumulate,
                             dw_split_k(self.units, self.in_features, rows))
        if not need_dx:
            return None
        dx = self._buf("dx", (rows, self.in_features), x.dtype, x.device)
        if dx_resid is not None:
            gemm_dx(dy2, self.w, dx, resid=dx_resid)
        else:
            gemm_dx(dy2, self.w, dx)
        return dx


class CRF(Layer):

    def __init__(self, output_dim, sparse_target=True, mask_impossible_transitions=None, name="crf"):
        self.output_dim = int(output_dim)
        self.mask_impossible_transitions = mask_impossible_transitions
        self.sequence_lengths = None
        self.name = name

    def build(self, arena, in_features, prefix):
        if in_features != self.output_dim:
            raise ValueError("The last dimension of the input shape must be equal to output shape. "
                             "Use a linear layer if needed.")
        C = self.output_dim
        rng = np.random.Generator(np.random.PCG64(77 + C))
        self.transitions = arena.add(prefix + ".transitions", (C, C), glorot_uniform(rng, C, C, (C, C)), decay=True)
        self.arena = arena
        return C

    def variables(self):
        return [self.transitions]

    def get_transitions(self):
        t = self.transitions.value
        if self.mask_impossible_transitions is None:
            return t
        m = to_device(np.asarray(self.mask_impossible_transitions, np.float32), torch.float32, t.device)
        return t * m + (1.0 - m) * -10000.0

    def forward(self, x, training=False, sequence_lengths=None):
        assert x.dim() == 3 and x.shape[-1] == self.output_dim
        B, S, C = x.shape
        if sequence_lengths is not None:
            sl = to_device(sequence_lengths, torch.int32, x.device).reshape(-1)
        else:
            sl = torch.full((B,), S, dtype=torch.int32, device=x.device)
        self.sequence_lengths = sl
        self._pot = x
        if training:
            return x
        tags = self._buf("tags", (B, S), torch.int32, x.device)
        ops.crf_viterbi(x.float().contiguous() if x.dtype != torch.float32 else x.contiguous(), sl,
                        self.get_transitions().contiguous(), tags)
        return torch.nn.functional.one_hot(tags.long(), C).to(torch.float32)

    def backward(self, dy, accumulate=False):
        return dy

    def _nll(self, y_true, y_pred, sample_weights):
        pot = y_pred if y_pred.dtype == torch.float32 else y_pred.float()
        pot = pot.contiguous()
        B, S, C = pot.shape
        yt = to_device(y_true, None, pot.device)
        tags = (yt.argmax(-1) if yt.dim() == 3 else yt).to(torch.int32).contiguous()
        loss = torch.empty(1, dtype=torch.float32, device=pot.device)
        dpot = self._buf("dpot", (B, S, C), torch.float32, pot.device)
        dtr = self._buf("dtrans", (C, C), torch.float32, pot.device)
        ops.crf_nll(pot, tags, self.sequence_lengths, self.get_transitions().contiguous(), sample_weights, loss, dpot, dtr)
        if self.mask_impossible_transitions is not None:
            dtr = dtr * to_device(np.asarray(self.mask_impossible_transitions, np.float32), torch.float32, pot.device)
        self._dtrans, self._dpot = dtr, dpot
        return DeviceScalar(loss)

    @property
    def loss(self):
        layer = self

        class _CRFLoss:
            def __call__(self, y_true, y_pred):
                return layer._nll(y_true, y_pred, None)

            def backward(self, accumulate=False):
                g = layer.transitions.grad
                g.add_(layer._dtrans) if accumulate else g.copy_(layer._dtrans)
                return layer._dpot
        return _CRFLoss()

    def loss_sample_weights(self, mask_positive_classes, negative_weight):
        layer = self
        mpc = np.asarray(mask_positive_classes, np.float32)

        class _CRFWLoss:
            def __call__(self, y_true, y_pred):
                yt = to_device(y_true, torch.float32, y_pred.device)
                pos = yt * to_device(mpc, torch.float32, yt.device)
                neg = (pos == 0).all(-1).all(-1)
                w = (pos == 1).any(-1).any(-1).to(torch.float32) + neg.to(torch.float32) * float(negative_weight)
                return layer._nll(y_true, y_pred, w.contiguous())

            def backward(self, accumulate=False):
                g = layer.transitions.grad
                g.add_(layer._dtrans) if accumulate else g.copy_(layer._dtrans)
                return layer._dpot
        return _CRFWLoss()
```

### polus_amd/models.py

```python
import json
import os
import sys
from functools import wraps

import numpy as np
import torch

from . import _lib, ops
from .layers import CRF, Dense, Dropout, Flatten, Layer, dense_bwd_params_group, gemm_dx
from .tensor import ParamArena, to_device, device
from .utils import complex_json_deserializer, complex_json_serializer, flatten_dict, merge_dicts

COMPUTE_DTYPES = {"f32": torch.float32, "float32": torch.float32, torch.float32: torch.float32,
                  "bf16": torch.bfloat16, "bfloat16": torch.bfloat16, torch.bfloat16: torch.bfloat16}


def load_model(file_name_w_ext, change_config={}, external_module=None):
    file_name = os.path.splitext(file_name_w_ext)[0]
    with open(file_name_w_ext, "r") as f:
        cfg = complex_json_deserializer(json.load(f))
    cfg["model"] = merge_dicts(cfg.get("model", {}), change_config)
    module = external_module if external_module is not None else sys.modules[__name__]
    model = getattr(module, cfg["func_name"])(**cfg)
    if os.path.exists(file_name + ".init.npz"):
        z = np.load(file_name + ".init.npz", allow_pickle=False)
        spec = json.loads(str(z["__spec__"]))
        args = [z[k] for k in spec["args"]]
        kwargs = {k: z[v] for k, v in spec["kwargs"].items()}
        model.init_from_data(*args, **kwargs)
    from .checkpoint import load_weights
    load_weights(model, file_name)
    return model


def resolve_activation(activation_name):
    return activation_name


def from_config(func):
    @wraps(func)
    def function_wrapper(**kwargs):
        if "model" not in kwargs:
            kwargs = {"model": {k: v for k, v in kwargs.items() if k != "func_name"}}
        kwargs = {k: v for k, v in kwargs.items() if k != "func_name"}
        if "activation" in kwargs["model"]:
            _activation = kwargs["model"]["activation"]
            kwargs["model"]["activation"] = resolve_activation(_activation)
        model = func(**flatten_dict(kwargs))
        kwargs["func_name"] = func.__name__
        if "activation" in kwargs["model"]:
            kwargs["model"]["activation"] = _activation
        model._name = func.__name__
        model.savable_config = kwargs
        return model
    return function_wrapper


class BertConfig:

    def __init__(self, vocab_size=30522, hidden_size=768, num_hidden_layers=12, num_attention_heads=12,
                 intermediate_size=3072, max_position_embeddings=512, type_vocab_size=2, layer_norm_eps=1e-12,
                 hidden_dropout_prob=0.0, attention_probs_dropout_prob=0.0, _name_or_path=""):
        if hidden_size != num_attention_heads * 64:
            raise ValueError("the fused attention kernel is built for head_dim 64 (BERT-base/large, BioBERT, PubMedBERT)")
        if not (0.0 <= hidden_dropout_prob < 1.0 and 0.0 <= attention_probs_dropout_prob < 1.0):
            raise ValueError("dropout probabilities must be in [0, 1)")
        self.vocab_size, self.hidden_size = vocab_size, hidden_size
        self.num_hidden_layers, self.num_attention_heads = num_hidden_layers, num_attention_heads
        self.intermediate_size, self.max_position_embeddings = intermediate_size, max_position_embeddings
        self.type_vocab_size, self.layer_norm_eps = type_vocab_size, layer_norm_eps
        self.hidden_dropout_prob, self.attention_probs_dropout_prob = hidden_dropout_prob, attention_probs_dropout_prob
        self._name_or_path = _name_or_path

    @classmethod
    def bert_base(cls, **kw):
        return cls(**kw)

    @classmethod
    def bert_large(cls, **kw):
        return cls(hidden_size=1024, num_hidden_layers=24, num_attention_heads=16, intermediate_size=4096, **kw)

    def to_dict(self):
        return {k: v for k, v in self.__dict__.items()}


class BaseModelOutputWithPooling:

    def __init__(self, last_hidden_state, pooler_output):
        self.last_hidden_state, self.pooler_output = last_hidden_state, pooler_output

    def __getitem__(self, k):
        if isinstance(k, int):
            return (self.last_hidden_state, self.pooler_output)[k]
        return getattr(self, k)


_M32 = 0xFFFFFFFF


def dropout_seed_static(base, layer, site):
    return (base * 0x9E3779B1 + ((layer + 1) * 8 + site) * 0xC2B2AE35) & _M32


def dropout_salt(step):
    return (step * 0x85EBCA6B) & _M32


def dropout_seed(base, step, layer, site):
    x = (dropout_seed_static(base, layer, site) + dropout_salt(step)) & _M32
    x ^= x >> 15
    return (x * 0x2C1B3C6D) & _M32


def _trunc_normal(rng, shape, std=0.02):
    return (np.clip(rng.standard_normal(shape), -2.0, 2.0) * std).astype(np.float32)


class BertLayer:

    def __init__(self, cfg, arena, index, rng):
        H, I = cfg.hidden_size, cfg.intermediate_size
        self.cfg, self.index = cfg, index
        p = f"layer{index}."
        add = arena.add
        self.qkv_w = add(p + "qkv.w", (3 * H, H), _trunc_normal(rng, (3 * H, H)), matrix=True)
        self.qkv_b = add(p + "qkv.b", (3 * H,), np.zeros(3 * H, np.float32), decay=False)
        self.out_w = add(p + "out.w", (H, H), _trunc_normal(rng, (H, H)), matrix=True)
        self.out_b = add(p + "out.b", (H,), np.zeros(H, np.float32), decay=False)
        self.ln1_g = add(p + "ln1.g", (H,), np.ones(H, np.float32), decay=False)
        self.ln1_b = add(p + "ln1.b", (H,), np.zeros(H, np.float32), decay=False)
        self.ffn1_w = add(p + "ffn1.w", (I, H), _trunc_normal(rng, (I, H)), matrix=True)
        self.ffn1_b = add(p + "ffn1.b", (I,), np.zeros(I, np.float32), decay=False)
        self.ffn2_w = add(p + "ffn2.w", (H, I), _trunc_normal(rng, (H, I)), matrix=True)
        self.ffn2_b = add(p + "ffn2.b", (H,), np.zeros(H, np.float32), decay=False)
        self.ln2_g = add(p + "ln2.g", (H,), np.ones(H, np.float32), decay=False)
        self.ln2_b = add(p + "ln2.b", (H,), np.zeros(H, np.float32), decay=False)
        self._bufs = {}

    def variables(self):
        return [self.qkv_w, self.qkv_b, self.out_w, self.out_b, self.ln1_g, self.ln1_b,
                self.ffn1_w, self.ffn1_b, self.ffn2_w, self.ffn2_b, self.ln2_g, self.ln2_b]

    def _buf(self, key, shape, dtype, dev):
        t = self._bufs.get(key)
        if t is None or t.shape != tuple(shape) or t.dtype != dtype:
            t = self._bufs[key] = torch.empty(tuple(shape), dtype=dtype, device=dev)
        return t

    def forward(self, x, mask, B, S, p_hid=0.0, p_att=0.0, seeds=(0, 0, 0), for_backward=True):
        cfg = self.cfg
        H, I, A = cfg.hidden_size, cfg.intermediate_size, cfg.num_attention_heads
        T, dt, dev = B * S, x.dtype, x.device
        b = lambda k, shape, d=dt: self._buf(k, shape, d, dev)
        qkv, ctx, lse = b("qkv", (T, 3 * H)), b("ctx", (T, H)), b("lse", (B, A, S), torch.float32)
        z1, a1 = b("z1", (T, H)), b("a1", (T, H))
        m1, r1 = b("m1", (T,), torch.float32), b("r1", (T,), torch.float32)
        u, f = (b("u", (T, I)) if for_backward else None), b("f", (T, I))
        z2, y = b("z2", (T, H)), b("y", (T, H))
        m2, r2 = b("m2", (T,), torch.float32), b("r2", (T,), torch.float32)
        ops.gemm(x, self.qkv_w.compute, qkv, bias=self.qkv_b.value, split_k="auto")
        ops.attention_fwd(qkv, mask, ctx, lse, B, S, A, drop_p=p_att, seed=seeds[0])
        ops.gemm(ctx, self.out_w.compute, z1, bias=self.out_b.value, resid=x, drop_p=p_hid, seed=seeds[1], split_k="auto")
        ops.layernorm_fwd(z1, self.ln1_g.value, self.ln1_b.value, a1, m1, r1, cfg.layer_norm_eps)
        ops.gemm(a1, self.ffn1_w.compute, f, bias=self.ffn1_b.value, aux=u, act="gelu", flags=ops.GEMM_ACT_FWD, split_k="auto")
        ops.gemm(f, self.ffn2_w.compute, z2, bias=self.ffn2_b.value, resid=a1, drop_p=p_hid, seed=seeds[2], split_k="auto")
        ops.layernorm_fwd(z2, self.ln2_g.value, self.ln2_b.value, y, m2, r2, cfg.layer_norm_eps)
        self._stash = (x, mask, B, S, p_hid, p_att, seeds) if for_backward else None
        return y

    def backward(self, dy, scratch, accumulate=False, side=None):
        cfg = self.cfg
        H, I, A = cfg.hidden_size, cfg.intermediate_size, cfg.num_attention_heads
        if self._stash is None:
            raise RuntimeError("BertLayer.backward: the last forward pass ran with training=False (nothing was kept for backward)")
        x, mask, B, S, p_hid, p_att, seeds = self._stash
        T = B * S
        bb = self._bufs
        par = "" if side is None else str(self.index & 1)
        dz2, du = scratch("dz2" + par, (T, H)), scratch("du" + par, (T, I))
        da1, dz1 = scratch("da1", (T, H)), scratch("dz1" + par, (T, H))
        dctx, dqkv = scratch("dctx", (T, H)), scratch("dqkv" + par, (T, 3 * H))
        dx = scratch("dx%d" % (self.index & 1), (T, H))
        dz2m = scratch("dz2m" + par, (T, H)) if p_hid > 0 else None
        lnp = None
        if side is not None and os.environ.get("POLUS_LN_DEFER_FINALIZE", "1") != "0":
            nfl = ops.layernorm_bwd_partial_floats(T, H)
            lnp = [scratch("lnp2" + par, (nfl,), torch.float32), scratch("lnp1" + par, (nfl,), torch.float32)]
        ops.layernorm_bwd(dy, bb["z2"], self.ln2_g.value, bb["m2"], bb["r2"], dz2,
                          self.ln2_g.grad, self.ln2_b.grad, self.ffn2_b.grad, accumulate,
                          dx_masked=dz2m, drop_p=p_hid, seed=seeds[2], partials=lnp[0] if lnp else None)
        dz2d = dz2m if dz2m is not None else dz2
        gemm_dx(dz2d, self.ffn2_w, du, aux=bb["u"], act="gelu", flags=ops.GEMM_ACT_BWD)
        gemm_dx(du, self.ffn1_w, da1, resid=dz2)
        dz1m = scratch("dz1m" + par, (T, H)) if p_hid > 0 else None
        ops.layernorm_bwd(da1, bb["z1"], self.ln1_g.value, bb["m1"], bb["r1"], dz1,
                          self.ln1_g.grad, self.ln1_b.grad, self.out_b.grad, accumulate,
                          dx_masked=dz1m, drop_p=p_hid, seed=seeds[1], partials=lnp[1] if lnp else None)
        dz1d = dz1m if dz1m is not None else dz1
        gemm_dx(dz1d, self.out_w, dctx)
        ops.attention_bwd(bb["qkv"], mask, bb["ctx"], dctx, bb["lse"], dqkv, B, S, A, drop_p=p_att, seed=seeds[0])
        problems = [(dz2d, bb["f"], self.ffn2_w.grad, None), (du, bb["a1"], self.ffn1_w.grad, self.ffn1_b.grad),
                    (dz1d, bb["ctx"], self.out_w.grad, None), (dqkv, x, self.qkv_w.grad, self.qkv_b.grad)]
        if side is None:
            dense_bwd_params_group(problems, accumulate)
            self.dw_done = None
        else:
            main = torch.cuda.current_stream()
            if not hasattr(self, "_ev"):
                self._ev = [torch.cuda.Event(), torch.cuda.Event()]
            self._ev[0].record(main)
            side.wait_event(self._ev[0])
            with _lib.stream_scope(side):
                dense_bwd_params_group(problems, accumulate)
                if lnp:
                    ops.layernorm_bwd_finalize(lnp[0], T, H, self.ln2_g.grad, self.ln2_b.grad, self.ffn2_b.grad, accumulate)
                    ops.layernorm_bwd_finalize(lnp[1], T, H, self.ln1_g.grad, self.ln1_b.grad, self.out_b.grad, accumulate)
                self._ev[1].record(side)
            self.dw_done = self._ev[1]
        gemm_dx(dqkv, self.qkv_w, dx, resid=dz1)
        return dx


class BertEmbeddings:
    def __init__(self, cfg, arena, rng):
        H = cfg.hidden_size
        self.cfg = cfg
        self.word = arena.add("emb.word", (cfg.vocab_size, H), _trunc_normal(rng, (cfg.vocab_size, H)))
        self.pos = arena.add("emb.pos", (cfg.max_position_embeddings, H), _trunc_normal(rng, (cfg.max_position_embeddings, H)))
        self.type = arena.add("emb.type", (cfg.type_vocab_size, H), _trunc_normal(rng, (cfg.type_vocab_size, H)))
        self.ln_g = arena.add("emb.ln.g", (H,), np.ones(H, np.float32), decay=False)
        self.ln_b = arena.add("emb.ln.b", (H,), np.zeros(H, np.float32), decay=False)
        self._bufs = {}

    def variables(self):
        return [self.word, self.pos, self.type, self.ln_g, self.ln_b]

    def forward(self, input_ids, token_type_ids, dtype, p_hid=0.0, seed=0):
        B, S = input_ids.shape
        dev = input_ids.device
        key = (B, S, dtype)
        if self._bufs.get("key") != key:
            self._bufs = {"key": key,
                          "y": torch.empty((B * S, self.cfg.hidden_size), dtype=dtype, device=dev),
                          "mean": torch.empty(B * S, dtype=torch.float32, device=dev),
                          "rstd": torch.empty(B * S, dtype=torch.float32, device=dev)}
        bb = self._bufs
        ops.embed_ln_fwd(input_ids, token_type_ids, self.word.value, self.pos.value, self.type.value,
                         self.ln_g.value, self.ln_b.value, bb["y"], bb["mean"], bb["rstd"], self.cfg.layer_norm_eps,
                         drop_p=p_hid, seed=seed)
        self._stash = (input_ids, token_type_ids, p_hid, seed)
        return bb["y"]

    def backward(self, dy, accumulate=False, deterministic=False):
        ids, tts, p_hid, seed = self._stash
        bb = self._bufs
        ops.embed_ln_bwd(dy, ids, tts, self.word.value, self.pos.value, self.type.value, self.ln_g.value,
                         bb["mean"], bb["rstd"], self.word.grad, self.pos.grad, self.type.grad,
                         self.ln_g.grad, self.ln_b.grad, accumulate=accumulate, deterministic=deterministic,
                         drop_p=p_hid, seed=seed)


class PolusModel:

    def __init__(self, name=None):
        self._name = name or self.__class__.__name__.lower()
        self.grad_ready_hook = None
        self.deterministic = False
        self.savable_config = {}

    @property
    def name(self):
        return self._name

    def set_name(self, name):
        self._name = name

    def init_from_data(self, *args, **kwargs):
        self._init = (args, kwargs)
        return self(*args, **kwargs)

    @property
    def trainable_weights(self):
        return list(self.arena.vars)

    def __call__(self, *args, training=False, **kwargs):
        return self.call(*args, training=training, **kwargs)

    def get_weights(self):
        return [v.numpy() for v in self.trainable_weights]

    def set_weights(self, weights):
        for v, w in zip(self.trainable_weights, weights):
            v.assign(w)

    def _notify(self, variables):
        if self.grad_ready_hook is not None and variables:
            lo = min(v.offset for v in variables)
            hi = max(v.offset + v.size for v in variables)
            self.grad_ready_hook(lo, hi, variables)


def _to_numpy(a):
    return a.detach().cpu().numpy() if isinstance(a, torch.Tensor) else np.asarray(a)


class SavableModel(PolusModel):

    def save(self, base_path=os.path.join(".polus_cache", "saved_models"), extension=""):
        os.makedirs(base_path, exist_ok=True)
        path = os.path.join(base_path, self.name + extension)
        with open(path + ".cfg", "w") as f:
            json.dump(complex_json_serializer(self.savable_config), f)
        if hasattr(self, "_init"):
            args, kwargs = self._init
            arrs, spec = {}, {"args": [], "kwargs": {}}
            for i, a in enumerate(args):
                arrs[f"arg{i}"] = _to_numpy(a); spec["args"].append(f"arg{i}")
            for k, a in kwargs.items():
                if k == "training":
                    continue
                arrs[f"kw_{k}"] = _to_numpy(a); spec["kwargs"][k] = f"kw_{k}"
            np.savez(path + ".init.npz", __spec__=np.asarray(json.dumps(spec)), **arrs)
        w = self.get_weights()
        np.savez(path + ".npz", **{f"weight{i}": a for i, a in enumerate(w)})
        return path


class PolusClassifier(SavableModel):
    def inference(self, x):
        logits = self(x, training=False)
        l2 = logits.reshape(-1, logits.shape[-1])
        if l2.dtype != torch.float32:
            l2 = l2.float()
        out = torch.empty(l2.shape[0], dtype=torch.int32, device=l2.device)
        ops.argmax(l2.contiguous(), out)
        return out.view(logits.shape[:-1])


class Sequential(PolusModel):

    def __init__(self, layers, compute_dtype="f32", name=None, input_dim=None):
        super().__init__(name)
        self.layers = list(layers)
        self.compute_dtype = COMPUTE_DTYPES[compute_dtype]
        self.arena = ParamArena(self.compute_dtype)
        feat = input_dim
        for i, l in enumerate(self.layers):
            feat = l.build(self.arena, feat, f"{l.name}{i}")
        last_dense = [l for l in self.layers if isinstance(l, Dense)]
        if last_dense and last_dense[-1].activation is None and last_dense[-1].out_dtype is None:
            last_dense[-1].out_dtype = torch.float32
        self.arena.finalize()

    def call(self, x, training=False, **kw):
        x = to_device(x, None, self.arena.device)
        if x.is_floating_point() and x.dtype != self.compute_dtype:
            x = x.to(self.compute_dtype)
        for l in self.layers:
            x = l.forward(x, training=training)
        return x

    def backward(self, dy, accumulate=False):
        first_param_layer = next(i for i, l in enumerate(self.layers) if l.variables())
        for i in range(len(self.layers) - 1, -1, -1):
            l = self.layers[i]
            if isinstance(l, Dense):
                dy = l.backward(dy, accumulate, need_dx=(i > first_param_layer))
            else:
                dy = l.backward(dy, accumulate)
            self._notify(l.variables())
            if dy is None:
                break
        return dy


class SequentialSavableModel(Sequential, SavableModel):
    pass


class SequentialPolusClassifier(Sequential, PolusClassifier):
    pass


class BertModel(SavableModel):

    def __init__(self, cfg, compute_dtype="bf16", num_labels=None, seed=1234, name="bert", with_embeddings=True,
                 layer_indices=None, arena=None, add_pooling_layer=False):
        super().__init__(name)
        self.config = cfg
        self.compute_dtype = COMPUTE_DTYPES[compute_dtype]
        self.savable_config = {"func_name": "bert_model",
                               "model": dict(cfg.to_dict(), compute_dtype="bf16" if self.compute_dtype == torch.bfloat16 else "f32",
                                             num_labels=num_labels, seed=seed, add_pooling_layer=add_pooling_layer)}
        own = arena is None
        self.arena = arena or ParamArena(self.compute_dtype)
        rng = np.random.Generator(np.random.PCG64(seed))
        self.embeddings = BertEmbeddings(cfg, self.arena, rng) if with_embeddings else None
        idx = range(cfg.num_hidden_layers) if layer_indices is None else layer_indices
        self.layer = [BertLayer(cfg, self.arena, i, rng) for i in idx]
        self.pooler = None
        if add_pooling_layer:
            self.pooler = Dense(cfg.hidden_size, activation="tanh", name="pooler")
            self.pooler.build(self.arena, cfg.hidden_size, "pooler")
        self.head = None
        if num_labels:
            self.head = Dense(num_labels, out_dtype=torch.float32, name="head")
            self.head.build(self.arena, cfg.hidden_size, "head")
        if own:
            self.arena.finalize()
        self._scratch = {}
        self.dropout_base_seed = seed
        self.dropout_step = 0
        self.overlap_dw = os.environ.get("POLUS_OVERLAP_DW", "1") != "0"
        self._side = None

    def scratch(self, key, shape, dtype=None):
        dtype = dtype or self.compute_dtype
        t = self._scratch.get(key)
        if t is None or t.shape != tuple(shape) or t.dtype != dtype:
            t = self._scratch[key] = torch.empty(tuple(shape), dtype=dtype, device=self.arena.device)
        return t

    def load_numpy_params(self, params, head_w=None, head_b=None):
        for v in self.arena.vars:
            if v.name in params:
                v.assign(params[v.name])
        if self.head is not None and head_w is not None:
            self.head.w.assign(head_w)
            self.head.b.assign(head_b)

    def site_seed(self, layer, site, step=None):
        base = self.dropout_base_seed
        if not getattr(self, "identical_dropout_across_ranks", False):
            from . import comm
            if comm.size() > 1:
                base = (base ^ (comm.rank() * 0x9E3779B1)) & 0xFFFFFFFF
        if getattr(self, "graph_seeds", False):
            return dropout_seed_static(base, layer, site)
        return dropout_seed(base, self.dropout_step if step is None else step, layer, site)

    def encode(self, hidden, attention_mask, B, S, training=False):
        cfg = self.config
        p_hid = cfg.hidden_dropout_prob if training else 0.0
        p_att = cfg.attention_probs_dropout_prob if training else 0.0
        for l in self.layer:
            seeds = tuple(self.site_seed(l.index, k) for k in range(3))
            hidden = l.forward(hidden, attention_mask, B, S, p_hid, p_att, seeds, for_backward=training)
        return hidden

    def call(self, input_ids=None, attention_mask=None, token_type_ids=None, training=False, hidden_states=None, **kw):
        dev = self.arena.device
        if isinstance(input_ids, dict):
            d = input_ids
            input_ids, attention_mask = d.get("input_ids"), d.get("attention_mask", attention_mask)
            token_type_ids = d.get("token_type_ids", token_type_ids)
        if attention_mask is not None:
            attention_mask = to_device(attention_mask, torch.int32, dev)
        if hidden_states is None:
            input_ids = to_device(input_ids, torch.int32, dev)
            B, S = input_ids.shape
            if token_type_ids is not None:
                token_type_ids = to_device(token_type_ids, torch.int32, dev)
            hidden = self.embeddings.forward(input_ids, token_type_ids, self.compute_dtype,
                                             self.config.hidden_dropout_prob if training else 0.0, self.site_seed(-1, 0))
        else:
            hs = to_device(hidden_states, self.compute_dtype, dev)
            B, S = hs.shape[0], hs.shape[1]
            hidden = hs.reshape(B * S, -1)
        self._shape = (B, S)
        self.tokens_per_step = B * S
        hidden = self.encode(hidden, attention_mask, B, S, training)
        if training:
            self.dropout_step += 1
        H = self.config.hidden_size
        if self.head is not None:
            return self.head.forward(hidden).view(B, S, -1)
        h3 = hidden.view(B, S, H)
        if self.pooler is not None:
            return BaseModelOutputWithPooling(last_hidden_state=h3, pooler_output=self.pooler.forward(h3[:, 0, :], training))
        return BaseModelOutputWithPooling(last_hidden_state=h3, pooler_output=h3[:, 0, :])

    def backward(self, dy=None, accumulate=False, dpooled=None):
        B, S = self._shape
        H = self.config.hidden_size
        if self.head is not None:
            dy = self.head.backward(dy.reshape(B * S, -1), accumulate)
            self._notify(self.head.variables())
        else:
            if dy is None:
                dy = torch.zeros((B * S, H), dtype=self.compute_dtype, device=self.arena.device)
            else:
                dy = to_device(dy, self.compute_dtype, self.arena.device).reshape(B * S, H)
            if dpooled is not None:
                dy = dy.clone()
                d3 = dy.view(B, S, H)
                dp = to_device(dpooled, self.compute_dtype, self.arena.device).reshape(B, H)
                if self.pooler is not None:
                    dcls = self.pooler.backward(dp, accumulate, dx_resid=d3[:, 0, :])
                    self._notify(self.pooler.variables())
                else:
                    dcls = self.scratch("dcls", (B, H))
                    ops.gemm(dp, _identity(H, self.compute_dtype, self.arena.device), dcls, resid=d3[:, 0, :])
                d3[:, 0, :].copy_(dcls)
        if self.overlap_dw and self._side is None:
            self._side = torch.cuda.Stream(device=self.arena.device)
        side = self._side if self.overlap_dw else None
        pending = []
        main = torch.cuda.current_stream()

        def retire(lay):
            if lay.dw_done is not None:
                main.wait_event(lay.dw_done)
            self._notify(lay.variables())
        for l in reversed(self.layer):
            if len(pending) == 2:
                retire(pending.pop(0))
            dy = l.backward(dy, self.scratch, accumulate, side)
            pending.append(l)
        for lay in pending:
            retire(lay)
        if self.embeddings is not None:
            self.embeddings.backward(dy, accumulate, self.deterministic)
            self._notify(self.embeddings.variables())
            return None
        return dy.view(B, S, -1)

    def inference(self, x):
        logits = self(**x, training=False) if isinstance(x, dict) else self(x, training=False)
        l2 = logits.reshape(-1, logits.shape[-1]).contiguous()
        out = torch.empty(l2.shape[0], dtype=torch.int32, device=l2.device)
        ops.argmax(l2, out)
        return out.view(logits.shape[:-1])


_EYE = {}


def _identity(n, dtype, dev):
    k = (n, dtype, str(dev))
    if k not in _EYE:
        _EYE[k] = torch.eye(n, dtype=dtype, device=dev)
    return _EYE[k]


@from_config
def bert_model(**kw):
    cfg_keys = ("vocab_size", "hidden_size", "num_hidden_layers", "num_attention_heads", "intermediate_size",
                "max_position_embeddings", "type_vocab_size", "layer_norm_eps", "hidden_dropout_prob",
                "attention_probs_dropout_prob", "_name_or_path")
    cfg = BertConfig(**{k: kw[k] for k in cfg_keys if k in kw})
    return BertModel(cfg, compute_dtype=kw.get("compute_dtype", "bf16"), num_labels=kw.get("num_labels"),
                     seed=kw.get("seed", 1234), add_pooling_layer=kw.get("add_pooling_layer", False))


class TFBertSplited(PolusModel):

    def __init__(self, bert_layers, arena, config, run_in_training_mode=True, name="bert_splited"):
        super().__init__(name)
        self.layer = list(bert_layers)
        self.arena, self.config = arena, config
        self.run_in_training_mode = run_in_training_mode
        self.compute_dtype = arena.compute_dtype
        self._scratch = {}
        self.dropout_base_seed, self.dropout_step = 4321, 0

    scratch = BertModel.scratch
    site_seed = BertModel.site_seed

    @property
    def trainable_weights(self):
        return [v for l in self.layer for v in l.variables()]

    def call(self, hidden_states, attention_mask, training=False, **kw):
        dev = self.arena.device
        hs = to_device(hidden_states, self.compute_dtype, dev)
        B, S, H = hs.shape
        mask = to_device(attention_mask, torch.int32, dev)
        hidden = hs.reshape(B * S, H)
        train = bool(self.run_in_training_mode and training)
        p_hid = self.config.hidden_dropout_prob if train else 0.0
        p_att = self.config.attention_probs_dropout_prob if train else 0.0
        for l in self.layer:
            hidden = l.forward(hidden, mask, B, S, p_hid, p_att, tuple(self.site_seed(l.index, k) for k in range(3)), for_backward=bool(training))
        if train:
            self.dropout_step += 1
        self._shape = (B, S)
        self.tokens_per_step = B * S
        h3 = hidden.view(B, S, H)
        return BaseModelOutputWithPooling(last_hidden_state=h3, pooler_output=h3[:, 0, :])

    def backward(self, dy, accumulate=False):
        B, S = self._shape
        dy = to_device(dy, self.compute_dtype, self.arena.device).reshape(B * S, -1)
        for l in reversed(self.layer):
            dy = l.backward(dy, self.scratch, accumulate)
            self._notify(l.variables())
        return dy.view(B, S, -1)


def split_bert_model(bert_model, index_layer, init_models=False, return_pre_bert_model=True,
                     return_post_bert_model=True):
    assert return_pre_bert_model or return_post_bert_model
    L = bert_model.config.num_hidden_layers
    assert L > index_layer > -L and index_layer != 0
    post_model = None
    if return_post_bert_model:
        post_model = TFBertSplited(bert_model.layer[index_layer:], bert_model.arena, bert_model.config)
    if return_pre_bert_model:
        del bert_model.layer[index_layer:]
        bert_model.config.num_hidden_layers = len(bert_model.layer)
    if init_models and return_pre_bert_model:
        B, S = 1, min(50, bert_model.config.max_position_embeddings)
        ids = np.ones((B, S), np.int32)
        out = bert_model(input_ids=ids, attention_mask=np.ones((B, S), np.int32), token_type_ids=np.zeros((B, S), np.int32))
        if post_model is not None:
            post_model(hidden_states=out.last_hidden_state, attention_mask=np.ones((B, S), np.int32))
    if return_pre_bert_model and return_post_bert_model:
        return bert_model, post_model
    return bert_model if return_pre_bert_model else post_model


def split_bert_model_from_checkpoint(bert_model_checkpoint, index_layer, **kw):
    from .checkpoint import load_bert_from_local
    return split_bert_model(load_bert_from_local(bert_model_checkpoint), index_layer, **kw)
```

### polus_amd/ops.py

```python
import torch

from . import _lib
from ._lib import (F32, BF16, K_CONTIG, K_STRIDED, ACT_NONE, ACT_GELU, ACT_SWISH, ACT_RELU, ACT_TANH,
                   GEMM_ACCUM_C, GEMM_ACT_FWD, GEMM_ACT_BWD, check, ptr, dtype_code)

GEMM_PROFILE = None

ACT_CODES = {None: ACT_NONE, "linear": ACT_NONE, "gelu": ACT_GELU, "swish": ACT_SWISH,
             "relu": ACT_RELU, "tanh": ACT_TANH}


class Workspace:

    def __init__(self, device):
        self.device = device
        self.buf = None

    def get(self, nbytes):
        nbytes = int(nbytes)
        if self.buf is None or self.buf.numel() < nbytes:
            if self.buf is not None:
                torch.cuda.current_stream().synchronize()
            self.buf = torch.empty(max(nbytes, 1 << 20), dtype=torch.uint8, device=self.device)
        return self.buf


_WS = {}
WORKSPACE_OVERRIDE = None


_HAS_GPU = None


def workspace(device):
    global _HAS_GPU
    if WORKSPACE_OVERRIDE is not None:
        return WORKSPACE_OVERRIDE
    if _HAS_GPU is None:
        _HAS_GPU = torch.cuda.is_available()
    key = (device, _lib.current_stream() if _HAS_GPU else 0)
    ws = _WS.get(key)
    if ws is None:
        ws = _WS[key] = Workspace(device)
    return ws


def _st():
    return _lib.current_stream()


def set_dynamic_params(block):
    if block is not None:
        _req_cuda(block)
        assert block.numel() * block.element_size() >= 16 and block.is_contiguous()
    check(_lib.load().polus_set_dynamic_params(ptr(block)), "polus_set_dynamic_params")


def set_env(name, value=None):
    import os
    if value is None:
        os.environ.pop(name, None)
    else:
        os.environ[name] = str(value)
    check(_lib.load().polus_reload_env(), "polus_reload_env")
    _AUTO_SPLIT.clear()


def reserve_cus(active):
    check(_lib.load().polus_set_reserve_active(1 if active else 0), "polus_set_reserve_active")


def _req_cuda(*ts):
    for t in ts:
        if t is not None and not t.is_cuda:
            raise _lib.PolusHipError("polus_amd ops need device (HBM) tensors; there is no CPU path")


_AUTO_SPLIT = {}


def gemm(a, b, out, *, a_layout=K_CONTIG, b_layout=K_CONTIG, M=None, N=None, K=None, alpha=1.0,
         bias=None, resid=None, aux=None, act=None, flags=0, split_k=1, drop_p=0.0, seed=0):
    lib = _lib.load()
    _req_cuda(a, b, out, bias, resid, aux)
    dt = dtype_code(a.dtype)
    assert b.dtype == a.dtype and a.dim() == 2 and b.dim() == 2 and out.dim() == 2
    if a_layout == K_CONTIG:
        m_, k_ = a.shape
    else:
        k_, m_ = a.shape
    if b_layout == K_CONTIG:
        n_, kb_ = b.shape
    else:
        kb_, n_ = b.shape
    M = m_ if M is None else M
    N = n_ if N is None else N
    K = k_ if K is None else K
    assert kb_ == k_, f"contraction mismatch {k_} vs {kb_}"
    assert out.shape[0] >= M and out.shape[1] >= N
    assert a.stride(1) == 1 and b.stride(1) == 1 and out.stride(1) == 1
    ws = None
    ws_bytes = 0
    if split_k == "auto":
        split_k = 1
        if (a.dtype == torch.bfloat16 and out.dtype == a.dtype and a_layout == K_CONTIG and b_layout == K_CONTIG
                and not (flags & GEMM_ACCUM_C)):
            key = (M, N, K)
            split_k = _AUTO_SPLIT.get(key)
            if split_k is None:
                split_k = _AUTO_SPLIT[key] = int(lib.polus_gemm_auto_split(M, N, K))
    if split_k > 1:
        ws_bytes = lib.polus_gemm_workspace_bytes(M, N, split_k)
        ws = workspace(a.device).get(ws_bytes)
    prof = GEMM_PROFILE
    if prof is not None:
        e0, e1 = torch.cuda.Event(enable_timing=True), torch.cuda.Event(enable_timing=True)
        e0.record()
    common = (dt, a_layout, b_layout, dtype_code(out.dtype),
              ptr(a), a.stride(0), ptr(b), b.stride(0), ptr(out), out.stride(0),
              M, N, K, float(alpha), ptr(bias),
              ptr(resid), resid.stride(0) if resid is not None else 0,
              ptr(aux), aux.stride(0) if aux is not None else 0,
              ACT_CODES[act] if not isinstance(act, int) else act, flags, split_k, ptr(ws), ws_bytes)
    if drop_p > 0.0:
        check(lib.polus_gemm_dropout(*common, float(drop_p), int(seed) & 0xFFFFFFFF, _st()), "polus_gemm_dropout")
    else:
        check(lib.polus_gemm(*common, _st()), "polus_gemm")
    if prof is not None:
        e1.record()
        kind = "fwd" if (a_layout == K_CONTIG and b_layout == K_CONTIG) else ("dx" if a_layout == K_CONTIG else "dw")
        prof.append((kind, 2.0 * M * N * K, e0, e1))
    return out


def attention_fwd(qkv, mask, ctx, lse, B, S, n_heads, drop_p=0.0, seed=0):
    lib = _lib.load()
    _req_cuda(qkv, mask, ctx, lse)
    H = n_heads * 64
    assert qkv.shape == (B * S, 3 * H) and ctx.shape == (B * S, H) and qkv.is_contiguous() and ctx.is_contiguous()
    assert lse.dtype == torch.float32 and lse.numel() == B * n_heads * S
    assert mask is None or (mask.dtype == torch.int32 and mask.numel() == B * S and mask.is_contiguous())
    check(lib.polus_attention_fwd(dtype_code(qkv.dtype), ptr(qkv), ptr(mask), ptr(ctx), ptr(lse),
                                  B, S, n_heads, 64, float(drop_p), int(seed) & 0xFFFFFFFF, _st()), "polus_attention_fwd")


def attention_bwd(qkv, mask, ctx, dctx, lse, dqkv, B, S, n_heads, drop_p=0.0, seed=0):
    lib = _lib.load()
    _req_cuda(qkv, mask, ctx, dctx, lse, dqkv)
    H = n_heads * 64
    assert qkv.shape == (B * S, 3 * H) and dqkv.shape == (B * S, 3 * H) and dctx.shape == (B * S, H)
    assert qkv.is_contiguous() and dqkv.is_contiguous() and dctx.is_contiguous() and ctx.is_contiguous()
    nb = lib.polus_attention_bwd_workspace_bytes(B, S, n_heads)
    ws = workspace(qkv.device).get(nb)
    check(lib.polus_attention_bwd(dtype_code(qkv.dtype), ptr(qkv), ptr(mask), ptr(ctx), ptr(dctx), ptr(lse),
                                  ptr(dqkv), B, S, n_heads, 64, float(drop_p), int(seed) & 0xFFFFFFFF, ptr(ws), nb, _st()),
          "polus_attention_bwd")


def layernorm_fwd(x, gamma, beta, y, mean, rstd, eps):
    lib = _lib.load()
    _req_cuda(x, gamma, beta, y, mean, rstd)
    rows, H = x.shape
    assert x.is_contiguous() and y.is_contiguous() and y.shape == x.shape
    check(lib.polus_layernorm_fwd(dtype_code(x.dtype), ptr(x), ptr(gamma), ptr(beta), ptr(y), ptr(mean), ptr(rstd),
                                  rows, H, float(eps), _st()), "polus_layernorm_fwd")


def layernorm_bwd_partial_floats(rows, H):
    return (_lib.load().polus_layernorm_bwd_workspace_bytes(rows, H) + 3) // 4


def layernorm_bwd(dy, x, gamma, mean, rstd, dx, dgamma, dbeta, dbias=None, accumulate=False, dx_masked=None,
                  drop_p=0.0, seed=0, partials=None):
    lib = _lib.load()
    _req_cuda(dy, x, gamma, mean, rstd, dx, dgamma, dbeta, dbias)
    rows, H = x.shape
    assert dy.is_contiguous() and x.is_contiguous() and dx.is_contiguous()
    nb = lib.polus_layernorm_bwd_workspace_bytes(rows, H)
    if partials is not None:
        assert partials.dtype == torch.float32 and partials.numel() * 4 >= nb and partials.is_contiguous()
        check(lib.polus_layernorm_bwd(dtype_code(x.dtype), ptr(dy), ptr(x), ptr(gamma), ptr(mean), ptr(rstd), ptr(dx),
                                      None, None, ptr(dbias), int(accumulate), rows, H,
                                      ptr(dx_masked), float(drop_p), int(seed) & 0xFFFFFFFF, ptr(partials), partials.numel() * 4, _st()),
              "polus_layernorm_bwd")
        return
    ws = workspace(x.device).get(nb)
    check(lib.polus_layernorm_bwd(dtype_code(x.dtype), ptr(dy), ptr(x), ptr(gamma), ptr(mean), ptr(rstd), ptr(dx),
                                  ptr(dgamma), ptr(dbeta), ptr(dbias), int(accumulate), rows, H,
                                  ptr(dx_masked), float(drop_p), int(seed) & 0xFFFFFFFF, ptr(ws), nb, _st()), "polus_layernorm_bwd")


def layernorm_bwd_finalize(partials, rows, H, dgamma, dbeta, dbias=None, accumulate=False):
    _req_cuda(partials, dgamma, dbeta, dbias)
    check(_lib.load().polus_layernorm_bwd_finalize(ptr(partials), partials.numel() * 4, rows, H, ptr(dgamma), ptr(dbeta), ptr(dbias),
                                                   int(accumulate), _st()), "polus_layernorm_bwd_finalize")


def embed_ln_fwd(ids, type_ids, word, pos, typ, gamma, beta, y, mean, rstd, eps, drop_p=0.0, seed=0):
    lib = _lib.load()
    _req_cuda(ids, type_ids, word, pos, typ, gamma, beta, y, mean, rstd)
    B, S = ids.shape
    V, H = word.shape
    assert ids.dtype == torch.int32 and ids.is_contiguous()
    assert type_ids is None or (type_ids.dtype == torch.int32 and type_ids.is_contiguous())
    check(lib.polus_embed_ln_fwd(dtype_code(y.dtype), ptr(ids), ptr(type_ids), ptr(word), ptr(pos), ptr(typ),
                                 ptr(gamma), ptr(beta), ptr(y), ptr(mean), ptr(rstd),
                                 B, S, H, V, pos.shape[0], typ.shape[0], float(eps), float(drop_p), int(seed) & 0xFFFFFFFF,
                                 _st()), "polus_embed_ln_fwd")


def embed_ln_bwd(dy, ids, type_ids, word, pos, typ, gamma, mean, rstd, gword, gpos, gtyp, ggamma, gbeta,
                 accumulate=False, deterministic=False, drop_p=0.0, seed=0):
    lib = _lib.load()
    _req_cuda(dy, ids, word, gword)
    B, S = ids.shape
    V, H = word.shape
    nb = lib.polus_embed_bwd_workspace_bytes(B, S, H)
    ws = workspace(dy.device).get(nb)
    check(lib.polus_embed_ln_bwd(dtype_code(dy.dtype), ptr(dy), ptr(ids), ptr(type_ids), ptr(word), ptr(pos), ptr(typ),
                                 ptr(gamma), ptr(mean), ptr(rstd), ptr(gword), ptr(gpos), ptr(gtyp), ptr(ggamma),
                                 ptr(gbeta), int(accumulate), int(deterministic),
                                 B, S, H, V, pos.shape[0], typ.shape[0], float(drop_p), int(seed) & 0xFFFFFFFF,
                                 ptr(ws), nb, _st()), "polus_embed_ln_bwd")


def colsum(x, out, accumulate=False, rows=None, cols=None):
    lib = _lib.load()
    _req_cuda(x, out)
    rows = x.shape[0] if rows is None else rows
    cols = x.shape[1] if cols is None else cols
    nb = lib.polus_colsum_workspace_bytes(rows, cols)
    ws = workspace(x.device).get(nb)
    check(lib.polus_colsum(dtype_code(x.dtype), ptr(x), x.stride(0), rows, cols, ptr(out), int(accumulate),
                           ptr(ws), nb, _st()), "polus_colsum")


def softmax_xent(logits, labels, loss, dlogits, class_weights=None, rows=None, C=None):
    lib = _lib.load()
    _req_cuda(logits, labels, loss, dlogits, class_weights)
    rows = logits.shape[0] if rows is None else rows
    C = logits.shape[1] if C is None else C
    assert logits.dtype == torch.float32 and labels.dtype == torch.int32 and loss.dtype == torch.float32
    nb = lib.polus_loss_workspace_bytes(rows)
    ws = workspace(logits.device).get(nb)
    check(lib.polus_softmax_xent(dtype_code(dlogits.dtype), ptr(logits), logits.stride(0), ptr(labels),
                                 ptr(class_weights), ptr(loss), ptr(dlogits), dlogits.stride(0), rows, C,
                                 ptr(ws), nb, _st()), "polus_softmax_xent")


def sigmoid_xent(logits, y_true, class_weights, negative_weight, loss, dlogits):
    lib = _lib.load()
    _req_cuda(logits, y_true, class_weights, loss, dlogits)
    rows, C = logits.shape
    nb = lib.polus_loss_workspace_bytes(rows)
    ws = workspace(logits.device).get(nb)
    check(lib.polus_sigmoid_xent(dtype_code(dlogits.dtype), ptr(logits), logits.stride(0), ptr(y_true), y_true.stride(0),
                                 ptr(class_weights), float(negative_weight), ptr(loss), ptr(dlogits), dlogits.stride(0),
                                 rows, C, ptr(ws), nb, _st()), "polus_sigmoid_xent")


def crf_nll(potentials, tags, lengths, trans, sample_w, loss, dpot, dtrans, accumulate=False):
    lib = _lib.load()
    _req_cuda(potentials, tags, lengths, trans, sample_w, loss, dpot, dtrans)
    B, S, C = potentials.shape
    assert potentials.dtype == torch.float32 and potentials.is_contiguous() and dpot.is_contiguous()
    nb = lib.polus_crf_workspace_bytes(B, S, C)
    ws = workspace(potentials.device).get(nb)
    check(lib.polus_crf_nll(dtype_code(dpot.dtype), ptr(potentials), ptr(tags), ptr(lengths), ptr(trans), ptr(sample_w),
                            ptr(loss), ptr(dpot), ptr(dtrans), int(accumulate), B, S, C, ptr(ws), nb, _st()),
          "polus_crf_nll")


def crf_viterbi(potentials, lengths, trans, out_tags):
    lib = _lib.load()
    _req_cuda(potentials, lengths, trans, out_tags)
    B, S, C = potentials.shape
    nb = lib.polus_crf_workspace_bytes(B, S, C)
    ws = workspace(potentials.device).get(nb)
    check(lib.polus_crf_viterbi(ptr(potentials), ptr(lengths), ptr(trans), ptr(out_tags), B, S, C, ptr(ws), nb, _st()),
          "polus_crf_viterbi")


def _maxsim_mask(m, rows, L, name):
    if m is None:
        return None
    assert m.dtype == torch.int32 and m.is_contiguous() and m.numel() == rows * L, f"{name}: int32 [{rows}, {L}] expected"
    return m


def maxsim_fwd(q, d, qmask, dmask, score, argmax):
    _req_cuda(q, d, qmask, dmask, score, argmax)
    B, Lq, E = q.shape
    N, Ld = d.shape[0], d.shape[1]
    assert d.dim() == 3 and d.shape[2] == E and d.dtype == q.dtype and q.is_contiguous() and d.is_contiguous()
    assert score.dtype == torch.float32 and score.dim() == 2 and score.shape[0] >= B and score.shape[1] >= N and score.stride(1) == 1
    assert argmax.dtype == torch.int32 and argmax.is_contiguous() and argmax.numel() == B * N * Lq
    check(_lib.load().polus_maxsim_fwd(dtype_code(q.dtype), ptr(q), ptr(d), ptr(_maxsim_mask(qmask, B, Lq, "qmask")),
                                       ptr(_maxsim_mask(dmask, N, Ld, "dmask")), ptr(score), score.stride(0), ptr(argmax),
                                       B, N, Lq, Ld, E, _st()), "polus_maxsim_fwd")


def maxsim_scores(q, d, qmask, dmask, score):
    _req_cuda(q, d, qmask, dmask, score)
    B, Lq, E = q.shape
    N, Ld = d.shape[0], d.shape[1]
    assert d.dim() == 3 and d.shape[2] == E and d.dtype == q.dtype and q.is_contiguous() and d.is_contiguous()
    assert score.dtype == torch.float32 and score.dim() == 2 and score.shape[0] >= B and score.shape[1] >= N and score.stride(1) == 1
    check(_lib.load().polus_maxsim_scores(dtype_code(q.dtype), ptr(q), ptr(d), ptr(_maxsim_mask(qmask, B, Lq, "qmask")),
                                          ptr(_maxsim_mask(dmask, N, Ld, "dmask")), ptr(score), score.stride(0),
                                          B, N, Lq, Ld, E, _st()), "polus_maxsim_scores")


def maxsim_rerank(q, d, qmask, dmask, cand, score):
    _req_cuda(q, d, qmask, dmask, cand, score)
    B, Lq, E = q.shape
    assert d.dim() == 3 and d.shape[2] == E and d.dtype == q.dtype and q.is_contiguous() and d.is_contiguous()
    N, Ld = d.shape[0], d.shape[1]
    assert cand.dtype == torch.int32 and cand.dim() == 2 and cand.shape[0] == B and (cand.stride(1) == 1 or cand.shape[1] == 1)
    C = cand.shape[1]
    assert score.dtype == torch.float32 and tuple(score.shape) == (B, C) and (score.stride(1) == 1 or C == 1)
    check(_lib.load().polus_maxsim_rerank(dtype_code(q.dtype), ptr(q), ptr(d), ptr(_maxsim_mask(qmask, B, Lq, "qmask")),
                                          ptr(_maxsim_mask(dmask, N, Ld, "dmask")), ptr(cand), cand.stride(0), ptr(score),
                                          score.stride(0), B, C, N, Lq, Ld, E, _st()), "polus_maxsim_rerank")


def topk_merge(scores, top_val, top_id, id0=0, init=False, ids=None):
    _req_cuda(scores, top_val, top_id, ids)
    rows, n = scores.shape
    k = top_val.shape[1]
    assert scores.dtype == torch.float32 and scores.dim() == 2 and (scores.stride(1) == 1 or n == 1)
    assert top_val.dtype == torch.float32 and top_id.dtype == torch.int32 and top_val.is_contiguous() and top_id.is_contiguous()
    assert tuple(top_val.shape) == (rows, k) and tuple(top_id.shape) == (rows, k)
    if ids is not None:
        assert int(id0) == 0, "ids and a non-zero id0 exclude each other"
        assert ids.dtype == torch.int32 and tuple(ids.shape) == (rows, n) and (ids.stride(1) == 1 or n == 1)
        check(_lib.load().polus_topk_merge_ids(ptr(scores), scores.stride(0), ptr(ids), ids.stride(0), rows, n,
                                               ptr(top_val), ptr(top_id), k, 1 if init else 0, _st()),
              "polus_topk_merge_ids")
        return
    check(_lib.load().polus_topk_merge(ptr(scores), scores.stride(0), rows, n, int(id0), ptr(top_val), ptr(top_id), k,
                                       1 if init else 0, _st()), "polus_topk_merge")


def maxsim_bwd(q, d, dscore, argmax, dq, dd):
    _req_cuda(q, d, dscore, argmax, dq, dd)
    B, Lq, E = q.shape
    N, Ld = d.shape[0], d.shape[1]
    assert d.dim() == 3 and d.shape[2] == E and d.dtype == q.dtype and q.is_contiguous() and d.is_contiguous()
    assert dscore.dtype == torch.float32 and dscore.shape[0] >= B and dscore.shape[1] >= N and dscore.stride(1) == 1
    assert argmax.dtype == torch.int32 and argmax.is_contiguous() and argmax.numel() == B * N * Lq
    assert dq.shape == q.shape and dd.shape == d.shape and dq.dtype == q.dtype and dd.dtype == d.dtype
    assert dq.is_contiguous() and dd.is_contiguous()
    check(_lib.load().polus_maxsim_bwd(dtype_code(q.dtype), ptr(q), ptr(d), ptr(dscore), dscore.stride(0), ptr(argmax),
                                       ptr(dq), ptr(dd), B, N, Lq, Ld, E, _st()), "polus_maxsim_bwd")


def l2norm_fwd(x, y, rnorm, eps=1e-12):
    _req_cuda(x, y, rnorm)
    E = x.shape[-1]
    rows = x.numel() // E
    assert x.is_contiguous() and y.is_contiguous() and y.shape == x.shape and y.dtype == x.dtype
    assert rnorm.dtype == torch.float32 and rnorm.numel() == rows and rnorm.is_contiguous()
    check(_lib.load().polus_l2norm_fwd(dtype_code(x.dtype), ptr(x), ptr(y), ptr(rnorm), rows, E, float(eps), _st()),
          "polus_l2norm_fwd")


def l2norm_bwd(y, rnorm, dy, dx, eps=1e-12):
    _req_cuda(y, rnorm, dy, dx)
    E = y.shape[-1]
    rows = y.numel() // E
    assert y.is_contiguous() and dy.is_contiguous() and dx.is_contiguous()
    assert dy.shape == y.shape and dx.shape == y.shape and dy.dtype == y.dtype and dx.dtype == y.dtype
    assert rnorm.dtype == torch.float32 and rnorm.numel() == rows
    check(_lib.load().polus_l2norm_bwd(dtype_code(y.dtype), ptr(y), ptr(rnorm), ptr(dy), ptr(dx), rows, E, float(eps), _st()),
          "polus_l2norm_bwd")


def argmax(x, out, rows=None, C=None):
    lib = _lib.load()
    _req_cuda(x, out)
    rows = x.shape[0] if rows is None else rows
    C = x.shape[1] if C is None else C
    check(lib.polus_argmax(ptr(x), x.stride(0), ptr(out), rows, C, _st()), "polus_argmax")


def confusion_matrix(row_idx, col_idx, cm, rejected=None):
    _req_cuda(row_idx, col_idx, cm)
    assert row_idx.dtype == torch.int32 and col_idx.dtype == torch.int32 and cm.dtype == torch.int32
    assert row_idx.numel() == col_idx.numel() and row_idx.is_contiguous() and col_idx.is_contiguous() and cm.is_contiguous()
    check(_lib.load().polus_confusion_matrix(ptr(row_idx), ptr(col_idx), row_idx.numel(), cm.shape[0], ptr(cm),
                                             ptr(rejected) if rejected is not None else None, _st()),
          "polus_confusion_matrix")


def _bio_rows(t, B, S, what):
    assert t.dtype == torch.int32 and tuple(t.shape) == (B, S) and (t.stride(1) == 1 or S == 1), what
    return ptr(t), t.stride(0) if B > 1 else S


def bio_entity_counts(tags_a, tags_b, scheme, counts, stats, mask=None):
    _req_cuda(tags_a, tags_b, scheme, counts, stats, mask)
    assert tags_a.dim() == 2
    B, S = tags_a.shape
    pa, lda = _bio_rows(tags_a, B, S, "tags_a")
    pb, ldb = _bio_rows(tags_b, B, S, "tags_b")
    pm, ldm = _bio_rows(mask, B, S, "mask") if mask is not None else (None, 0)
    assert scheme.dtype == torch.int32 and scheme.dim() == 1 and scheme.is_contiguous()
    assert counts.dtype == torch.int32 and counts.dim() == 2 and counts.shape[1] == 3 and counts.is_contiguous()
    assert stats.dtype == torch.int32 and stats.numel() == 6 and stats.is_contiguous()
    check(_lib.load().polus_bio_entity_counts(pa, lda, pb, ldb, pm, ldm, ptr(scheme), scheme.numel(), counts.shape[0],
                                              B, S, ptr(counts), ptr(stats), _st()), "polus_bio_entity_counts")


def bio_spans(tags, scheme, spans, count, mask=None, rejected=None):
    _req_cuda(tags, scheme, spans, count, mask, rejected)
    assert tags.dim() == 2
    B, S = tags.shape
    pt, ldt = _bio_rows(tags, B, S, "tags")
    pm, ldm = _bio_rows(mask, B, S, "mask") if mask is not None else (None, 0)
    assert scheme.dtype == torch.int32 and scheme.dim() == 1 and scheme.is_contiguous()
    assert spans.dtype == torch.int32 and spans.dim() == 3 and spans.shape[0] == B and spans.shape[2] == 3 and spans.is_contiguous()
    assert count.dtype == torch.int32 and count.numel() == B and count.is_contiguous()
    assert rejected is None or (rejected.dtype == torch.int32 and rejected.numel() == 1)
    check(_lib.load().polus_bio_spans(pt, ldt, pm, ldm, ptr(scheme), scheme.numel(), B, S, ptr(spans), spans.shape[1],
                                      ptr(count), ptr(rejected), _st()), "polus_bio_spans")


def adam_step(p, g, m, v, shadow, seg, n_seg, lr, lr_t, beta1, beta2, eps, weight_decay, grad_scale=1.0,
              clip_scale=None):
    lib = _lib.load()
    _req_cuda(p, g, m, v, shadow, seg, clip_scale)
    check(lib.polus_adam_step(ptr(p), ptr(g), ptr(m), ptr(v), ptr(shadow), ptr(seg), n_seg, p.numel(),
                              float(lr), float(lr_t), float(beta1), float(beta2), float(eps), float(weight_decay),
                              float(grad_scale), ptr(clip_scale), _st()), "polus_adam_step")


def sqnorm(g, out):
    lib = _lib.load()
    _req_cuda(g, out)
    nb = lib.polus_sqnorm_workspace_bytes(g.numel())
    ws = workspace(g.device).get(nb)
    check(lib.polus_sqnorm(ptr(g), g.numel(), ptr(out), ptr(ws), nb, _st()), "polus_sqnorm")


def sqnorm_segments(g, seg, n_seg, out):
    lib = _lib.load()
    _req_cuda(g, seg, out)
    ws = workspace(g.device).get(4096)
    check(lib.polus_sqnorm_segments(ptr(g), ptr(seg), int(n_seg), ptr(out), ptr(ws), 4096, _st()), "polus_sqnorm_segments")


def clip_scale(sq, grad_scale, clip_norm, out):
    check(_lib.load().polus_clip_scale(ptr(sq), sq.numel(), float(grad_scale), float(clip_norm), ptr(out), _st()), "polus_clip_scale")


def cast(src, dst):
    _req_cuda(src, dst)
    assert src.numel() == dst.numel()
    check(_lib.load().polus_cast(dtype_code(src.dtype), ptr(src), dtype_code(dst.dtype), ptr(dst), src.numel(), _st()),
          "polus_cast")


def scale_(x, a):
    _req_cuda(x)
    check(_lib.load().polus_scale(ptr(x), float(a), x.numel(), _st()), "polus_scale")


def act_bwd(dy, u, du, act):
    _req_cuda(dy, u, du)
    assert dy.numel() == u.numel() == du.numel() and dy.is_contiguous() and u.is_contiguous() and du.is_contiguous()
    check(_lib.load().polus_act_bwd(dtype_code(dy.dtype), ptr(dy), ptr(u), ptr(du), dy.numel(),
                                    ACT_CODES[act] if not isinstance(act, int) else act, _st()), "polus_act_bwd")


def transpose_bf16(src, dst):
    _req_cuda(src, dst)
    R, C = src.shape
    assert src.dtype == torch.bfloat16 and dst.dtype == torch.bfloat16 and dst.numel() == src.numel()
    assert src.is_contiguous() and dst.is_contiguous()
    check(_lib.load().polus_transpose_bf16(ptr(src), ptr(dst), R, C, _st()), "polus_transpose_bf16")


def dense_bwd_params_grouped(problems, accumulate=False, split_k=1):
    lib = _lib.load()
    T = problems[0][0].shape[0]
    arr = (_lib.DwProblem * len(problems))()
    for k, (dy, x, dw, db) in enumerate(problems):
        _req_cuda(dy, x, dw, db)
        assert dy.dtype == x.dtype and dw.dtype == torch.float32 and dy.shape[0] == T and x.shape[0] == T
        assert dy.stride(1) == 1 and x.stride(1) == 1 and dw.stride(1) == 1
        n_out, n_in = dy.shape[1], x.shape[1]
        assert tuple(dw.shape) == (n_out, n_in) and (db is None or (db.dtype == torch.float32 and db.numel() == n_out))
        arr[k] = _lib.DwProblem(ptr(dy), dy.stride(0), ptr(x), x.stride(0), ptr(dw), dw.stride(0), ptr(db), n_out, n_in)
    dt = dtype_code(problems[0][0].dtype)
    nb = lib.polus_dense_bwd_params_grouped_workspace_bytes(len(problems), arr, T, int(split_k))
    ws = workspace(problems[0][0].device).get(nb)
    prof = GEMM_PROFILE
    if prof is not None:
        e0, e1 = torch.cuda.Event(enable_timing=True), torch.cuda.Event(enable_timing=True)
        e0.record()
    check(lib.polus_dense_bwd_params_grouped(dt, len(problems), arr, T, 1 if accumulate else 0, int(split_k),
                                             ptr(ws), ws.numel(), _st()), "polus_dense_bwd_params_grouped")
    if prof is not None:
        e1.record()
        prof.append(("dw", sum(2.0 * T * p[0].shape[1] * p[1].shape[1] for p in problems), e0, e1))


def dense_thin_supported(dtype, H, C):
    return bool(_lib.load().polus_dense_thin_supported(dtype_code(dtype), int(H), int(C)))


def dense_thin_fwd(x, w, bias, y):
    _req_cuda(x, w, bias, y)
    rows, H = x.shape
    C = w.shape[0]
    assert w.dtype == x.dtype and w.shape[1] == H and y.shape == (rows, C)
    assert x.stride(1) == 1 and w.stride(1) == 1 and y.stride(1) == 1
    check(_lib.load().polus_dense_thin_fwd(dtype_code(x.dtype), ptr(x), x.stride(0), ptr(w), w.stride(0), ptr(bias),
                                           dtype_code(y.dtype), ptr(y), y.stride(0), rows, H, C, _st()), "polus_dense_thin_fwd")


def dense_thin_bwd(x, dy, w, dx, dw, db, accumulate=False):
    lib = _lib.load()
    _req_cuda(x, dy, w, dx, dw, db)
    rows, H = x.shape
    C = w.shape[0]
    assert dy.shape == (rows, C) and dy.stride(1) == 1 and dw.dtype == torch.float32 and tuple(dw.shape) == (C, H) and dw.stride(1) == 1
    assert dx is None or (dx.dtype == x.dtype and dx.shape == x.shape and dx.stride(1) == 1)
    nb = lib.polus_dense_thin_bwd_workspace_bytes(dtype_code(x.dtype), rows, H, C)
    ws = workspace(x.device).get(nb)
    check(lib.polus_dense_thin_bwd(dtype_code(x.dtype), ptr(x), x.stride(0), dtype_code(dy.dtype), ptr(dy), dy.stride(0),
                                   ptr(w), w.stride(0), ptr(dx), dx.stride(0) if dx is not None else 0, ptr(dw), dw.stride(0), ptr(db),
                                   rows, H, C, 1 if accumulate else 0, ptr(ws), ws.numel(), _st()), "polus_dense_thin_bwd")


def transpose_bf16_batched(src_base, dst_base, segs_dev, nseg, total_tiles):
    _req_cuda(src_base, dst_base, segs_dev)
    assert src_base.dtype == torch.bfloat16 and dst_base.dtype == torch.bfloat16 and segs_dev.dtype == torch.int64
    check(_lib.load().polus_transpose_bf16_batched(ptr(src_base), ptr(dst_base), ptr(segs_dev), int(nseg), int(total_tiles), _st()),
          "polus_transpose_bf16_batched")


def dense_bwd_params(dy, x, dw, db, accumulate=False, split_k=1):
    lib = _lib.load()
    _req_cuda(dy, x, dw, db)
    T, n_out = dy.shape
    n_in = x.shape[1]
    assert x.shape[0] == T and dw.shape == (n_out, n_in) and dw.dtype == torch.float32
    assert dy.stride(1) == 1 and x.stride(1) == 1 and dw.stride(1) == 1
    nb = lib.polus_dense_bwd_params_workspace_bytes(T, n_out, n_in, split_k)
    ws = workspace(dy.device).get(nb)
    prof = GEMM_PROFILE
    if prof is not None:
        e0, e1 = torch.cuda.Event(enable_timing=True), torch.cuda.Event(enable_timing=True)
        e0.record()
    check(lib.polus_dense_bwd_params(dtype_code(dy.dtype), ptr(dy), dy.stride(0), ptr(x), x.stride(0), ptr(dw), dw.stride(0),
                                     ptr(db), T, n_out, n_in, int(accumulate), split_k, ptr(ws), nb, _st()),
          "polus_dense_bwd_params")
    if prof is not None:
        e1.record()
        prof.append(("dw", 2.0 * T * n_out * n_in, e0, e1))


def dropout(x, y, drop_p, seed):
    _req_cuda(x, y)
    assert x.is_contiguous() and y.is_contiguous() and x.numel() == y.numel()
    check(_lib.load().polus_dropout(dtype_code(x.dtype), ptr(x), ptr(y), x.numel(), float(drop_p), int(seed) & 0xFFFFFFFF, _st()),
          "polus_dropout")


def dropout_mask(seed, drop_p, n, idx0=0, device=None):
    m = torch.empty(int(n), dtype=torch.uint8, device=device or "cuda")
    check(_lib.load().polus_dropout_mask(int(seed) & 0xFFFFFFFF, float(drop_p), int(idx0), int(n), ptr(m), _st()), "polus_dropout_mask")
    return m
```

### polus_amd/optimizers.py

```python
import math

import numpy as np
import torch

from . import ops

_CHUNK = 1 << 14


class _LearningRate:

    def __init__(self, value):
        self._value = value

    def read_value(self):
        if callable(self._value):
            raise TypeError("learning rate is a schedule; scale its max_lr instead")
        return self._value

    def numpy(self):
        return self.read_value()

    def assign(self, v):
        self._value = float(v)

    def __call__(self, step):
        return float(self._value(step)) if callable(self._value) else float(self._value)

    def scale(self, k):
        if callable(self._value):
            inner = self._value
            self._value = lambda step, inner=inner, k=k: inner(step) * k
        else:
            self._value = self._value * k


class WarmUpLinearDecay:

    def __init__(self, num_train_steps, max_lr, warmup_percentage=0.1, end_lr=1e-7):
        self.num_train_steps, self.max_lr = num_train_steps, max_lr
        self.num_warmup_steps = int(num_train_steps * warmup_percentage)
        self.decay_steps = num_train_steps - self.num_warmup_steps
        self.end_lr = 1e-7

    def __call__(self, step):
        if step < self.num_warmup_steps:
            return self.max_lr * (step / self.num_warmup_steps)
        s = min(step - self.num_warmup_steps, self.decay_steps)
        return (self.max_lr - self.end_lr) * (1.0 - s / self.decay_steps) + self.end_lr


def default_no_decay(name):
    return name.endswith(".b") or ".ln" in name


class Adam:

    def __init__(self, learning_rate=0.001, beta_1=0.9, beta_2=0.999, epsilon=1e-7, weight_decay_rate=0.0,
                 exclude_from_weight_decay=default_no_decay, global_clipnorm=None, name="Adam"):
        self.learning_rate = _LearningRate(learning_rate)
        self.beta_1, self.beta_2, self.epsilon = beta_1, beta_2, epsilon
        self.weight_decay_rate = weight_decay_rate
        self.exclude = exclude_from_weight_decay
        self.global_clipnorm = global_clipnorm
        self.iterations = 0
        self.grad_scale = 1.0
        self._state = {}
        self._tables = {}
        self.name = name

    def variables(self):
        out = []
        for m, v in self._state.values():
            out += [m, v]
        return out

    def get_config(self):
        return {"name": self.name, "beta_1": self.beta_1, "beta_2": self.beta_2, "epsilon": self.epsilon,
                "weight_decay_rate": self.weight_decay_rate}

    def _slots(self, arena):
        st = self._state.get(id(arena))
        if st is None:
            st = (torch.zeros_like(arena.params), torch.zeros_like(arena.params))
            self._state[id(arena)] = st
        return st

    def _table(self, arena, variables, ranges=None):
        key = (id(arena), tuple(id(v) for v in variables), tuple(ranges) if ranges is not None else None)
        t = self._tables.get(key)
        if t is None:
            seg = []
            for v in variables:
                decay = v.decay and not (self.exclude and self.exclude(v.name))
                flags = (1 if (decay and self.weight_decay_rate) else 0) | (2 if v.matrix else 0)
                windows = [(v.offset, v.offset + v.size)]
                if ranges is not None:
                    windows = [(max(v.offset, lo), min(v.offset + v.size, hi)) for lo, hi in ranges]
                    windows = [(lo, hi) for lo, hi in windows if hi > lo]
                for wlo, whi in windows:
                    for b in range(wlo, whi, _CHUNK):
                        seg.append((b, min(whi, b + _CHUNK), flags))
            if not seg:
                seg = [(0, 0, 0)]
            t = (torch.from_numpy(np.asarray(seg, np.int64)).to(arena.device), len(seg))
            self._tables[key] = t
        return t

    def apply_gradients(self, grads_and_vars, _advance=True, _refresh=True, _ranges=None):
        variables = [v for _, v in grads_and_vars]
        if _advance:
            self._lr_now = self.learning_rate(self.iterations)
            self.iterations += 1
        lr = self._lr_now
        t = self.iterations
        lr_t = lr * math.sqrt(1.0 - self.beta_2 ** t) / (1.0 - self.beta_1 ** t)
        arenas = {}
        for v in variables:
            arenas.setdefault(id(v.arena), (v.arena, []))[1].append(v)
        clip = None
        if self.global_clipnorm:
            dev0 = next(iter(arenas.values()))[0].device
            sq = torch.empty(len(arenas), dtype=torch.float32, device=dev0)
            clip = torch.empty(1, dtype=torch.float32, device=dev0)
            for k, (arena, vs) in enumerate(arenas.values()):
                seg, n_seg = self._table(arena, vs, _ranges)
                ops.sqnorm_segments(arena.grads, seg, n_seg, sq[k:k + 1])
            ops.clip_scale(sq, self.grad_scale, self.global_clipnorm, clip)
        for arena, vs in arenas.values():
            m, v = self._slots(arena)
            seg, n_seg = self._table(arena, vs, _ranges)
            ops.adam_step(arena.params, arena.grads, m, v, arena.shadow, seg, n_seg, lr, lr_t,
                          self.beta_1, self.beta_2, self.epsilon, self.weight_decay_rate,
                          grad_scale=self.grad_scale, clip_scale=clip)
            if _refresh:
                arena.refresh_transposed()


class AdamWeightDecay(Adam):

    def __init__(self, learning_rate=0.001, weight_decay_rate=0.01, **kw):
        super().__init__(learning_rate=learning_rate, weight_decay_rate=weight_decay_rate,
                         name=kw.pop("name", "AdamWeightDecay"), **kw)
```

### polus_amd/training.py

```python
import os

from . import _lib, comm
from .optimizers import Adam
from .callbacks import CallbackCoordinator, Profiler
from .context import PolusContext, logger

hvd = comm


class _UpdateInBackward:

    def __init__(self, trainer, arena):
        import torch
        self.trainer, self.arena = trainer, arena
        self.stream = torch.cuda.Stream(device=arena.device)
        self.fork, self.done = torch.cuda.Event(), torch.cuda.Event()
        self.vars = sorted(trainer.trainable_weights, key=lambda v: v.offset)

    def begin(self):
        self.first = True
        self.left = {id(v): v for v in self.vars}

    def _apply(self, vs):
        import torch
        main = torch.cuda.current_stream()
        self.fork.record(main)
        self.stream.wait_event(self.fork)
        with _lib.stream_scope(self.stream):
            self.trainer.optimizer.apply_gradients([(v.grad, v) for v in vs], _advance=self.first, _refresh=False)
            self.arena.refresh_transposed_of(vs)
        self.first = False
        for v in vs:
            del self.left[id(v)]

    def on_ready(self, lo, hi, variables=None):
        vs = [v for v in (variables or ()) if id(v) in self.left]
        if vs:
            self._apply(vs)

    def finish(self):
        import torch
        if self.left:
            self._apply(list(self.left.values()))
        with _lib.stream_scope(self.stream):
            self.done.record(self.stream)
        torch.cuda.current_stream().wait_event(self.done)


class _UpdateBehindAllReduce(_UpdateInBackward):

    def begin(self):
        super().begin()
        self.part_left = {}

    def on_bucket(self, lo, hi, work):
        vs = [v for v in self.vars if id(v) in self.left and lo <= v.offset and v.offset + v.size <= hi]
        parts = [v for v in self.vars if id(v) in self.left and v.offset < hi and v.offset + v.size > lo and
                 not (lo <= v.offset and v.offset + v.size <= hi)]
        opt = self.trainer.optimizer
        with _lib.stream_scope(self.stream):
            work.wait()
            if vs:
                opt.apply_gradients([(v.grad, v) for v in vs], _advance=self.first, _refresh=False)
                self.arena.refresh_transposed_of(vs)
                self.first = False
            for v in parts:
                a, b = max(lo, v.offset), min(hi, v.offset + v.size)
                opt.apply_gradients([(v.grad, v)], _advance=self.first, _refresh=False, _ranges=[(a, b)])
                self.first = False
                self.part_left[id(v)] = self.part_left.get(id(v), v.size) - (b - a)
                if self.part_left[id(v)] <= 0:
                    self.arena.refresh_transposed_of([v])
                    del self.left[id(v)]
        for v in vs:
            del self.left[id(v)]


class BaseTrainer:

    def __init__(self, model, optimizer, loss, metrics=[], post_process_logits=None, post_process_grads=None):
        if self.__class__.__name__ == "BaseTrainer":
            raise Exception("This is an abstraction that cannot be instantiated")
        super().__init__()
        self.model = model
        self.loss = loss
        self.optimizer = optimizer
        self.post_process_logits = post_process_logits
        self.post_process_grads = post_process_grads
        self.metrics = metrics
        self.early_stop = False
        self.train_config = {}
        self.step_counter = 0
        self.grad_accum_steps = 1

        if not hasattr(self, "trainable_weights"):
            logger.warning(f"Since no specific trainable_weights were defined during the {self.__class__.__name__} "
                           "instantiation, the trainer will optimizer all the variables found on the model instance")
            self.trainable_weights = model.trainable_weights

        self.use_horovod = PolusContext().is_horovod_enabled()
        self._reducers = {}
        if self.use_horovod:
            if hasattr(optimizer, "learning_rate"):
                optimizer.learning_rate.scale(hvd.size())
                logger.info("The learning rate was adjusted to account for the multiGPU training")
            else:
                logger.info("It was not possible to change the learning rate for the multiGPU training, "
                            "please multiply the learning rate by hvd.size()")

    def __str__(self):
        return "Trainer"

    def forward_without_grads(self, *inputs):
        return inputs

    def forward_with_grads(self, *inputs):
        raise NotImplementedError("forward_with_grads function must be implemented in order to compute a loss "
                                  "value for optimization")

    def backward_from_loss(self, accumulate=False):
        dlogits = self.loss.backward(accumulate)
        self.model.backward(dlogits, accumulate=accumulate)

    def _arenas(self):
        seen, out = set(), []
        for v in self.trainable_weights:
            if id(v.arena) not in seen:
                seen.add(id(v.arena))
                out.append(v.arena)
        return out

    def _dp_mode(self):
        m = getattr(self, "_dp_mode_cached", None)
        if m is None:
            arenas = self._arenas()
            want = os.environ.get("POLUS_DP_MODE", "allreduce") == "rs"
            ok = (len(arenas) == 1 and isinstance(self.optimizer, Adam) and not self.optimizer.global_clipnorm and
                  self.post_process_grads is None and hasattr(arenas[0], "size") and
                  arenas[0].grads.numel() % (64 * hvd.size()) == 0 and
                  all(v.arena is arenas[0] for v in self.trainable_weights) and want)
            if want and not ok:
                logger.warning("POLUS_DP_MODE=rs was requested but this trainer cannot use it (it needs ONE arena swept by the "
                               "fused Adam, no post_process_grads / global_clipnorm, and an arena of a multiple of "
                               f"64 x {hvd.size()} elements): exchanging gradients by all-reduce instead")
            m = self._dp_mode_cached = "rs" if ok else "allreduce"
        return m

    def _updater(self):
        if getattr(self, "_graphed", None) is not None or not getattr(self, "update_in_backward", True):
            return None
        key = tuple(id(v) for v in self.trainable_weights)
        u = getattr(self, "_updater_cached", False)
        if u is False or getattr(self, "_updater_key", None) != key:
            self._updater_key = key
            arenas = self._arenas()
            ok = (os.environ.get("POLUS_UPDATE_IN_BACKWARD", "1") != "0" and len(arenas) == 1 and
                  hasattr(self.model, "grad_ready_hook") and isinstance(self.optimizer, Adam) and
                  hasattr(self.optimizer, "grad_scale") and not self.optimizer.global_clipnorm and
                  self.post_process_grads is None and hasattr(arenas[0], "refresh_transposed") and
                  arenas[0].grads.is_cuda and all(v.arena is arenas[0] for v in self.trainable_weights))
            u = self._updater_cached = _UpdateInBackward(self, arenas[0]) if ok else None
        if u is not None and "POLUS_UPDATE_IN_BACKWARD" not in os.environ:
            tokens = getattr(self.model, "tokens_per_step", None)
            if tokens is not None and tokens < 6144:
                return None
        return u

    def _updater_dp(self, reducer):
        if self._dp_mode() != "allreduce" or reducer.mode == "rs" or not getattr(self, "update_in_backward", True):
            return None
        key = tuple(id(v) for v in self.trainable_weights)
        u = getattr(self, "_updater_dp_cached", False)
        if u is False or getattr(self, "_updater_dp_key", None) != key:
            self._updater_dp_key = key
            arena = self._arenas()[0]
            ok = (os.environ.get("POLUS_UPDATE_IN_BACKWARD", "1") != "0" and isinstance(self.optimizer, Adam) and
                  hasattr(self.optimizer, "grad_scale") and not self.optimizer.global_clipnorm and
                  self.post_process_grads is None and hasattr(arena, "refresh_transposed") and arena.grads.is_cuda and
                  all(v.arena is arena for v in self.trainable_weights) and getattr(self, "_graphed", None) is None)
            u = self._updater_dp_cached = _UpdateBehindAllReduce(self, arena) if ok else None
        return u

    def _reducer(self, arena):
        r = self._reducers.get(id(arena))
        if r is None:
            import torch
            bucket = int(float(getattr(self, "bucket_mb", None) or os.environ.get("POLUS_BUCKET_MB", "64")) * (1 << 20))
            mode = self._dp_mode()
            bf16 = os.environ.get("POLUS_DP_BF16", "0") == "1" and arena.grads.is_cuda
            r = comm.GradBucketReducer(arena.grads, bucket_bytes=bucket, boundaries=[v.offset for v in arena.vars],
                                       mode=mode, transport_dtype=torch.bfloat16 if bf16 else None)
            self._reducers[id(arena)] = r
        return r

    def train_step(self, *inputs):
        g = getattr(self, "_graphed", None)
        if g is not None:
            return g(*inputs)
        return self._eager_step(*inputs)

    def _eager_step(self, *inputs):
        with _lib.pinned_stream():
            return self._train_step(*inputs)

    def enable_step_graph(self, warmup=3):
        from .graph import GraphedStep
        self._graphed = GraphedStep(self, warmup)
        return self

    def disable_step_graph(self):
        self._graphed = None

    def _train_step(self, *inputs):
        micro = self.step_counter_micro = getattr(self, "step_counter_micro", 0)
        accum = self.grad_accum_steps
        first, last = (micro % accum == 0), (micro % accum == accum - 1)

        inputs = self.forward_without_grads(*inputs)
        inputs = self.forward_with_grads(*inputs)
        loss_value = self.loss(*inputs)

        reducers, dp_updater = [], None
        if self.use_horovod and last:
            arenas = self._arenas()
            if len(arenas) == 1 and hasattr(self.model, "grad_ready_hook"):
                r = self._reducer(arenas[0])
                r.begin()
                self.model.grad_ready_hook = r.on_ready
                reducers = [r]
                dp_updater = self._updater_dp(r)
                if dp_updater is not None:
                    self.optimizer.grad_scale = 1.0 / (hvd.size() * accum)
                    dp_updater.begin()
                    r.on_launched = dp_updater.on_bucket
        updater = self._updater() if (last and not self.use_horovod) else None
        if updater is not None:
            self.optimizer.grad_scale = 1.0 / accum
            updater.begin()
            self.model.grad_ready_hook = updater.on_ready
        reserve = bool(reducers) and getattr(self, "reserve_cus_in_backward", True)
        if reserve:
            from . import ops
            ops.reserve_cus(True)
        try:
            self.backward_from_loss(accumulate=not first)
        finally:
            if reserve:
                ops.reserve_cus(False)
        self.step_counter_micro = micro + 1
        self._exposed_mark(0)
        if updater is not None:
            self.model.grad_ready_hook = None
            updater.finish()
            return loss_value
        if not last:
            return loss_value

        scale = 1.0 / (hvd.size() * accum)
        split_at, owned = None, None
        if self.use_horovod:
            if not reducers:
                reducers = [self._reducer(a) for a in self._arenas()]
                for r in reducers:
                    r.begin()
            if self._dp_mode() == "rs":
                reducers[0].finish()
                owned = reducers[0].owned_ranges()
            elif dp_updater is not None:
                reducers[0].finish()
                reducers[0].on_launched = None
                if hasattr(self.model, "grad_ready_hook"):
                    self.model.grad_ready_hook = None
                dp_updater.finish()
                self._exposed_mark(1)
                return loss_value
            else:
                can_split = (len(reducers) == 1 and self.post_process_grads is None and
                             isinstance(self.optimizer, Adam) and not self.optimizer.global_clipnorm and
                             os.environ.get("POLUS_DP_SPLIT_ADAM", "1") != "0" and
                             all(v.arena.grads is reducers[0].grads for v in self.trainable_weights))
                split_at = reducers[0].finish(keep_last=True) if can_split else None
                if not can_split:
                    for r in reducers:
                        r.finish()
            if hasattr(self.model, "grad_ready_hook"):
                self.model.grad_ready_hook = None

        grads = [v.grad for v in self.trainable_weights]
        if self.post_process_grads is not None:
            if scale != 1.0:
                from . import ops
                for a in self._arenas():
                    ops.scale_(a.grads, scale)
                scale = 1.0
            grads = self.post_process_grads(grads)
        if hasattr(self.optimizer, "grad_scale"):
            self.optimizer.grad_scale = scale
        if owned is not None:
            arena = self._arenas()[0]
            self.optimizer.apply_gradients(list(zip(grads, self.trainable_weights)), _ranges=owned, _refresh=False)
            self._opt_state_synced = False
            reducers[0].allgather(arena.params)
            arena.refresh_shadow()
        elif split_at is not None:
            upper = [v for v in self.trainable_weights if v.offset >= split_at]
            lower = [v for v in self.trainable_weights if v.offset < split_at]
            self.optimizer.apply_gradients([(v.grad, v) for v in upper], _refresh=not lower)
            reducers[0].finish_last()
            if lower:
                self.optimizer.apply_gradients([(v.grad, v) for v in lower], _advance=False)
        else:
            self.optimizer.apply_gradients(zip(grads, self.trainable_weights))
        self._exposed_mark(1)
        return loss_value

    def tune_data_parallel(self, one_step, steps=4, bucket_mb=(16, 32, 128)):
        import time
        import torch
        if not self.use_horovod or hvd.size() == 1 or not torch.cuda.is_available():
            return None

        def measure():
            one_step()
            torch.cuda.synchronize()
            comm.barrier()
            t0 = time.perf_counter()
            for _ in range(steps):
                one_step()
            torch.cuda.synchronize()
            return comm.max_over_ranks(time.perf_counter() - t0) / steps * 1e3

        out = {}
        per = {}
        for setting in (True, False):
            self.reserve_cus_in_backward = setting
            per[setting] = measure()
        self.reserve_cus_in_backward = per[True] <= per[False]
        out.update(reserve_on_ms=round(per[True], 3), reserve_off_ms=round(per[False], 3),
                   reserve_cus_in_backward=self.reserve_cus_in_backward)
        if "POLUS_BUCKET_MB" not in os.environ and bucket_mb:
            best_mb, best = 64, min(per.values())
            out["bucket_64_ms"] = round(best, 3)
            for mb in bucket_mb:
                self.bucket_mb = mb
                self._reducers.clear()
                t = measure()
                out[f"bucket_{mb}_ms"] = round(t, 3)
                if t < best:
                    best_mb, best = mb, t
            self.bucket_mb = best_mb
            self._reducers.clear()
            out["bucket_mb"] = best_mb
        return out

    def _exposed_mark(self, which):
        if not (self.use_horovod and getattr(self, "measure_exposed", False)):
            return
        import torch
        ev = torch.cuda.Event(enable_timing=True)
        ev.record()
        if which == 0:
            self._exposed_begin = ev
        elif getattr(self, "_exposed_begin", None) is not None:
            self.exposed_events = (self._exposed_begin, ev)
            self._exposed_begin = None

    def lr_finder(self, tf_dataset, use_lr_found=False):
        pass

    def changing_train_config(self, **config):
        for k, v in config.items():
            self.train_config[k] = v

    def sync_optimizer_state(self):
        if not self.use_horovod or self._dp_mode() != "rs" or getattr(self, "_opt_state_synced", True):
            return
        arena = self._arenas()[0]
        if hasattr(self.optimizer, "_slots"):
            reducer = self._reducer(arena)
            for moment in self.optimizer._slots(arena):
                reducer.allgather(moment)
        self._opt_state_synced = True

    def broadcast_init_vars(self):
        self.sync_optimizer_state()
        hvd.broadcast_variables(self.trainable_weights, root_rank=0)
        hvd.broadcast_variables(self.optimizer.variables(), root_rank=0)

    _MISSING = {"tf_dataset": "You need to pass a training dataset to the trainer.train method",
                "epochs": "You need to pass the epochs variable to the trainer.train method"}

    def _resolve_train_args(self, given):
        resolved = {}
        for name, value in given.items():
            unset = value is None or (name == "callbacks" and len(value) == 0)
            if unset and name in self.train_config:
                value = self.train_config[name]
            elif unset and name in self._MISSING:
                raise ValueError(self._MISSING[name])
            resolved[name] = value
        return resolved

    def _one_epoch(self, epoch, dataset, transform):
        batches = iter(dataset)
        in_epoch = 0
        while True:
            self.callbacks.on_train_batch_begin(epoch, in_epoch)
            batch = next(batches, None)
            if batch is None:
                return
            if transform is not None:
                batch = transform(batch)
            if in_epoch == 0 and self.use_horovod:
                self.broadcast_init_vars()
            loss = self.train_step(*batch)
            self.callbacks.on_train_batch_end(epoch, in_epoch, loss)
            self.step_counter += 1
            in_epoch += 1
            if self.early_stop:
                return

    def train(self, tf_dataset=None, epochs=None, callbacks=[], train_map_f=None, steps=None, **kwargs):
        a = self._resolve_train_args(dict(tf_dataset=tf_dataset, epochs=epochs, callbacks=callbacks,
                                          train_map_f=train_map_f, steps=steps))
        dataset, n_epochs, hooks, transform = a["tf_dataset"], a["epochs"], a["callbacks"], a["train_map_f"]
        transform = kwargs.pop("custom_data_transform_f", transform)

        steps_per_epoch = a["steps"]
        if steps_per_epoch is None:
            try:
                steps_per_epoch = len(dataset)
            except TypeError:
                steps_per_epoch = -2

        if os.getenv("POLUS_PROFILER", "False").lower() in ("true", "1", "t", "y", "yes"):
            lo_hi = [int(x) for x in os.getenv("POLUS_PROFILER_RANGE", "10:20").split(":")]
            logger.info("POLUS_PROFILER env was set to True, so the Profiler callback was added to training")
            hooks = list(hooks) + [Profiler(steps_interval=lo_hi)]

        if not isinstance(hooks, CallbackCoordinator):
            hooks = CallbackCoordinator(hooks, trainer=self, epochs=n_epochs, steps=steps_per_epoch)
        self.callbacks = hooks

        self.callbacks.on_train_begin()
        for epoch in range(n_epochs):
            self.callbacks.on_epoch_begin(epoch)
            self._one_epoch(epoch, dataset, transform)
            self.callbacks.on_epoch_end(epoch)
            if self.early_stop:
                break
        self.callbacks.on_train_end()


class ClassifierTrainer(BaseTrainer):

    def __init__(self, *args, **kwargs):
        super().__init__(*args, **kwargs)

    def forward_with_grads(self, x, y):
        if isinstance(x, dict):
            logits = self.model(**x, training=True)
        else:
            logits = self.model(x, training=True)
        if self.post_process_logits is not None:
            logits = self.post_process_logits(logits)
        return y, logits


Trainer = ClassifierTrainer
```

Before: 5336 samples/s.

## Fuse AdamW update into grouped dW split-K reduction kernel per encoder layer

Adds a grouped dW reduce kernel that applies AdamW (params, moments, bf16 shadow) directly after summing the split-K slabs for each encoder layer's weight gradients, on the side stream. The goal is to avoid writing gradients and then reading them back in a separate optimizer pass. The trainer also enables this fused path at small token counts (64x256 tokens is above the 6144 threshold, so the update-in-backward path applies here) and reorders the dx GEMM ahead of the dW work. Risks include extra event waits, added bookkeeping for fused vs unfused variables, and a kernel that does more work per element.

Result: no change. 5347 samples/s, median of 6 (+0.2%).

```diff
diff --git a/include/polus_hip.h b/include/polus_hip.h
--- a/include/polus_hip.h
+++ b/include/polus_hip.h
@@ -62,6 +62,14 @@
 size_t polus_dense_bwd_params_grouped_workspace_bytes(int n, const polus_dw_problem* problems, int T, int split_k);
 int polus_dense_bwd_params_grouped(int dtype, int n, const polus_dw_problem* problems, int T, int accumulate,
                                    int split_k, void* workspace, size_t workspace_bytes, void* stream);
+
+int polus_dense_bwd_params_grouped_update(int dtype, int n, const polus_dw_problem* problems, int T, int accumulate,
+                                          int split_k, void* workspace, size_t workspace_bytes,
+                                          const float* grads, float* p, float* m, float* v, void* shadow_bf16, int64_t arena_n,
+                                          const int* wflags, const int* bflags,
+                                          float lr, float lr_t, float beta1, float beta2, float eps, float weight_decay,
+                                          float grad_scale, const float* clip_scale, void* after_event,
+                                          int* fused, void* stream);
 
 int polus_dense_thin_supported(int dtype, int H, int C);
 int polus_dense_thin_fwd(int dtype, const void* x, long ldx, const void* W, long ldw, const float* bias,
diff --git a/polus_amd/_lib.py b/polus_amd/_lib.py
--- a/polus_amd/_lib.py
+++ b/polus_amd/_lib.py
@@ -75,6 +75,8 @@
     "polus_transpose_bf16_batched": (_i, [_vp, _vp, _vp, _i, _i, _vp]),
     "polus_dense_bwd_params_grouped_workspace_bytes": (_sz, [_i, _vp, _i, _i]),
     "polus_dense_bwd_params_grouped": (_i, [_i, _i, _vp, _i, _i, _i, _vp, _sz, _vp]),
+    "polus_dense_bwd_params_grouped_update": (_i, [_i, _i, _vp, _i, _i, _i, _vp, _sz, _vp, _vp, _vp, _vp, _vp, _i64, _vp, _vp,
+                                                   _f, _f, _f, _f, _f, _f, _f, _vp, _vp, _c.POINTER(_i), _vp]),
     "polus_dense_thin_supported": (_i, [_i, _i, _i]),
     "polus_dense_thin_fwd": (_i, [_i, _vp, _l, _vp, _l, _vp, _i, _vp, _l, _i, _i, _i, _vp]),
     "polus_dense_thin_bwd_workspace_bytes": (_sz, [_i, _i, _i, _i]),
diff --git a/polus_amd/csrc/gemm.hip b/polus_amd/csrc/gemm.hip
--- a/polus_amd/csrc/gemm.hip
+++ b/polus_amd/csrc/gemm.hip
@@ -700,8 +700,24 @@
     return o;
 }
 
-extern "C" int polus_dense_bwd_params_grouped(int dtype, int n, const polus_dw_problem* problems, int T, int accumulate,
-                                              int split_k, void* workspace, size_t workspace_bytes, void* stream) {
+static bool dw_update_fits(int n, const polus_dw_problem* pr, const PolusDwUpdate& u) {
+    if (!u.grads || !u.p || !u.m || !u.v || !u.wflags || !u.bflags || u.n <= 0) return false;
+    if (!polus_aligned16(u.grads) || !polus_aligned16(u.p) || !polus_aligned16(u.m) || !polus_aligned16(u.v)) return false;
+    if (u.shadow_bf16 && ((uintptr_t)u.shadow_bf16 % 8) != 0) return false;
+    for (int k = 0; k < n; ++k) {
+        const polus_dw_problem& q = pr[k];
+        if (q.lddw < q.n_in) return false;
+        const int64_t extent = (int64_t)(q.n_out - 1) * q.lddw + q.n_in;
+        if (q.dW < u.grads || q.dW - u.grads > u.n - extent) return false;
+        if (q.db && (q.db < u.grads || q.db - u.grads > u.n - q.n_out || (u.bflags[k] & 2) || !polus_aligned16(q.db) || q.n_out % 4 != 0))
+            return false;
+    }
+    return true;
+}
+
+static int dense_bwd_params_grouped_impl(int dtype, int n, const polus_dw_problem* problems, int T, int accumulate,
+                                         int split_k, void* workspace, size_t workspace_bytes, void* stream,
+                                         const PolusDwUpdate* up, int* fused) {
     POLUS_REQUIRE(problems && n >= 1 && n <= POLUS_MAX_GROUP && T > 0, "polus_dense_bwd_params_grouped: bad arguments");
     const size_t es = polus_dtype_size(dtype);
     bool ring = dtype == POLUS_BF16 && !polus_cfg().gemm_v1 && !polus_cfg().dw_ungrouped;
@@ -749,6 +765,12 @@
     }
     int rc = pl.pp ? polus_launch_gemm_ppks_grouped_dw(ga, n, pl.eff, st) : polus_launch_gemm_ring_grouped_dw(ga, n, pl.eff, st);
     if (rc != POLUS_OK) return rc;
+    if (up && polus_cfg().dw_fused_reduce && o.aligned && dw_update_fits(n, problems, *up)) {
+        if (up->after_event) POLUS_HIP(hipStreamWaitEvent(st, static_cast<hipEvent_t>(up->after_event), 0));
+        rc = polus_launch_dw_group_reduce_adam(n, o.slabs, o.cs, o.dW, o.db, o.lddw, o.n_out, o.n_in, pl.eff, accumulate ? 1 : 0, *up, st);
+        if (rc == POLUS_OK) *fused = 1;
+        return rc;
+    }
     if (polus_cfg().dw_fused_reduce && o.aligned)
         return polus_launch_dw_group_reduce(n, o.slabs, o.cs, o.dW, o.db, o.lddw, o.n_out, o.n_in, pl.eff, accumulate ? 1 : 0, st);
     for (int k = 0; k < n; ++k) {
@@ -765,3 +787,22 @@
     }
     return POLUS_OK;
 }
+
+extern "C" int polus_dense_bwd_params_grouped(int dtype, int n, const polus_dw_problem* problems, int T, int accumulate,
+                                              int split_k, void* workspace, size_t workspace_bytes, void* stream) {
+    return dense_bwd_params_grouped_impl(dtype, n, problems, T, accumulate, split_k, workspace, workspace_bytes, stream, nullptr, nullptr);
+}
+
+extern "C" int polus_dense_bwd_params_grouped_update(int dtype, int n, const polus_dw_problem* problems, int T, int accumulate,
+                                                     int split_k, void* workspace, size_t workspace_bytes,
+                                                     const float* grads, float* p, float* m, float* v, void* shadow_bf16, int64_t arena_n,
+                                                     const int* wflags, const int* bflags,
+                                                     float lr, float lr_t, float beta1, float beta2, float eps, float weight_decay,
+                                                     float grad_scale, const float* clip_scale, void* after_event,
+                                                     int* fused, void* stream) {
+    POLUS_REQUIRE(fused, "polus_dense_bwd_params_grouped_update: fused is null");
+    *fused = 0;
+    const PolusDwUpdate u = {grads, p, m, v, shadow_bf16, arena_n, wflags, bflags,
+                             lr, lr_t, beta1, beta2, eps, weight_decay, grad_scale, clip_scale, after_event};
+    return dense_bwd_params_grouped_impl(dtype, n, problems, T, accumulate, split_k, workspace, workspace_bytes, stream, &u, fused);
+}
diff --git a/polus_amd/csrc/gemm_common.h b/polus_amd/csrc/gemm_common.h
--- a/polus_amd/csrc/gemm_common.h
+++ b/polus_amd/csrc/gemm_common.h
@@ -486,6 +486,16 @@
 int polus_launch_dw_group_reduce(int n, const float* const* slabs, const float* const* cs, float* const* dW, float* const* db,
                                  const long* lddw, const int* n_out, const int* n_in, const int* splits, int accumulate,
                                  hipStream_t st);
+struct PolusDwUpdate {
+    const float* grads; float* p; float* m; float* v; void* shadow_bf16; int64_t n;
+    const int* wflags; const int* bflags;
+    float lr, lr_t, beta1, beta2, eps, weight_decay, grad_scale;
+    const float* clip_scale;
+    void* after_event;
+};
+int polus_launch_dw_group_reduce_adam(int n, const float* const* slabs, const float* const* cs, float* const* dW, float* const* db,
+                                      const long* lddw, const int* n_out, const int* n_in, const int* splits, int accumulate,
+                                      const PolusDwUpdate& u, hipStream_t st);
 
 struct PPKSSKPlan {
     int tiles[POLUS_MAX_GROUP], tile0[POLUS_MAX_GROUP + 1], unit0[POLUS_MAX_GROUP + 1];
diff --git a/polus_amd/csrc/optim.hip b/polus_amd/csrc/optim.hip
--- a/polus_amd/csrc/optim.hip
+++ b/polus_amd/csrc/optim.hip
@@ -1,4 +1,5 @@
 #include "common.h"
+#include "gemm_common.h"
 
 namespace {
 
@@ -62,6 +63,93 @@
     }
 }
 
+struct DwUpdateArgs {
+    const float* slabs[POLUS_MAX_GROUP];
+    const float* cs[POLUS_MAX_GROUP];
+    const float* dW[POLUS_MAX_GROUP];
+    const float* db[POLUS_MAX_GROUP];
+    long lddw[POLUS_MAX_GROUP];
+    long woff[POLUS_MAX_GROUP], boff[POLUS_MAX_GROUP];
+    int n_out[POLUS_MAX_GROUP], n_in[POLUS_MAX_GROUP], splits[POLUS_MAX_GROUP];
+    int wflags[POLUS_MAX_GROUP], bflags[POLUS_MAX_GROUP];
+    int blk0[POLUS_MAX_GROUP + 1];
+    int n, accumulate;
+    AdamArgs a;
+};
+
+__device__ __forceinline__ void adam_quad(const AdamArgs& a, const float gs, const float decay, const bool shadow, const long i,
+                                          const float4 g4) {
+    const float4 p4 = *reinterpret_cast<const float4*>(a.p + i);
+    const float4 m4 = *reinterpret_cast<const float4*>(a.m + i);
+    const float4 v4 = *reinterpret_cast<const float4*>(a.v + i);
+    const float g[4] = {g4.x * gs, g4.y * gs, g4.z * gs, g4.w * gs};
+    float p[4] = {p4.x, p4.y, p4.z, p4.w}, m[4] = {m4.x, m4.y, m4.z, m4.w}, v[4] = {v4.x, v4.y, v4.z, v4.w};
+    const float c1 = 1.0f - a.b1, c2 = 1.0f - a.b2;
+#pragma unroll
+    for (int e = 0; e < 4; ++e) {
+        p[e] = __builtin_fmaf(-decay, p[e], p[e]);
+        m[e] = __builtin_fmaf(a.b1, m[e], c1 * g[e]);
+        const float t = c2 * g[e];
+        v[e] = __builtin_fmaf(a.b2, v[e], t * g[e]);
+        const float num = a.lr_t * m[e], den = sqrtf(v[e]) + a.eps;
+        p[e] -= num / den;
+    }
+    *reinterpret_cast<float4*>(a.p + i) = make_float4(p[0], p[1], p[2], p[3]);
+    *reinterpret_cast<float4*>(a.m + i) = make_float4(m[0], m[1], m[2], m[3]);
+    *reinterpret_cast<float4*>(a.v + i) = make_float4(v[0], v[1], v[2], v[3]);
+    if (shadow) store4<bf16_t>(a.shadow + i, p);
+}
+
+__global__ __launch_bounds__(256) void dw_group_reduce_adam_kernel(DwUpdateArgs ra) {
+    AdamArgs& a = ra.a;
+    if (a.dyn) { a.lr = a.dyn->lr; a.lr_t = a.dyn->lr_t; }
+    const float gs = a.gscale * (a.clip ? *a.clip : 1.0f);
+    const int b = blockIdx.x;
+    int q = 0;
+#pragma unroll
+    for (int k = 1; k < POLUS_MAX_GROUP; ++k)
+        if (k < ra.n && b >= ra.blk0[k]) q = k;
+    const float* slabs = nullptr; const float* cs = nullptr; const float* dW = nullptr; const float* db = nullptr;
+    long lddw = 0, woff = 0, boff = 0; int n_out = 0, n_in = 0, splits = 0, wflags = 0, bflags = 0, blk0 = 0;
+#pragma unroll
+    for (int k = 0; k < POLUS_MAX_GROUP; ++k)
+        if (k == q) { slabs = ra.slabs[k]; cs = ra.cs[k]; dW = ra.dW[k]; db = ra.db[k]; lddw = ra.lddw[k];
+                      woff = ra.woff[k]; boff = ra.boff[k]; n_out = ra.n_out[k]; n_in = ra.n_in[k]; splits = ra.splits[k];
+                      wflags = ra.wflags[k]; bflags = ra.bflags[k]; blk0 = ra.blk0[k]; }
+    const long total = (long)n_out * n_in;
+    const long quads = total / 4;
+    const long idx = (long)(b - blk0) * 256 + threadIdx.x;
+    if (idx < quads) {
+        const long e = idx * 4;
+        const int mr = (int)(e / n_in), nc = (int)(e % n_in);
+        const float4* c = reinterpret_cast<const float4*>(dW + (long)mr * lddw + nc);
+        float4 s;
+        if (slabs != nullptr) {
+            s = *reinterpret_cast<const float4*>(slabs + e);
+            for (int z = 1; z < splits; ++z) {
+                const float4 t = *reinterpret_cast<const float4*>(slabs + (long)z * total + e);
+                s.x += t.x; s.y += t.y; s.z += t.z; s.w += t.w;
+            }
+            if (ra.accumulate) { const float4 o = *c; s.x += o.x; s.y += o.y; s.z += o.z; s.w += o.w; }
+        } else {
+            s = *c;
+        }
+        adam_quad(a, gs, (wflags & 1) ? a.lr * a.wd : 0.0f, (wflags & 2) && a.shadow, woff + (long)mr * lddw + nc, s);
+    }
+    if (cs != nullptr && db != nullptr && idx * 4 < n_out) {
+        float4 s = make_float4(0.f, 0.f, 0.f, 0.f);
+        for (int z = 0; z < splits; ++z) {
+            const float4 t = *reinterpret_cast<const float4*>(cs + (long)z * n_out + idx * 4);
+            s.x += t.x; s.y += t.y; s.z += t.z; s.w += t.w;
+        }
+        if (ra.accumulate) {
+            const float4 o = *reinterpret_cast<const float4*>(db + idx * 4);
+            s = make_float4(o.x + s.x, o.y + s.y, o.z + s.z, o.w + s.w);
+        }
+        adam_quad(a, gs, (bflags & 1) ? a.lr * a.wd : 0.0f, false, boff + idx * 4, s);
+    }
+}
+
 __global__ __launch_bounds__(256) void sqnorm_partial_kernel(const float* __restrict__ g, int64_t n, float* __restrict__ partial) {
     __shared__ float red[4];
     float s = 0.f;
@@ -142,6 +230,33 @@
     return POLUS_OK;
 }
 
+int polus_launch_dw_group_reduce_adam(int n, const float* const* slabs, const float* const* cs, float* const* dW, float* const* db,
+                                      const long* lddw, const int* n_out, const int* n_in, const int* splits, int accumulate,
+                                      const PolusDwUpdate& u, hipStream_t st) {
+    DwUpdateArgs ra;
+    memset(&ra, 0, sizeof(ra));
+    ra.n = n; ra.accumulate = accumulate;
+    int b0 = 0;
+    for (int k = 0; k < n; ++k) {
+        ra.slabs[k] = slabs[k]; ra.cs[k] = cs[k]; ra.dW[k] = dW[k]; ra.db[k] = db[k]; ra.lddw[k] = lddw[k];
+        ra.woff[k] = dW[k] - u.grads; ra.boff[k] = db[k] ? db[k] - u.grads : 0;
+        ra.n_out[k] = n_out[k]; ra.n_in[k] = n_in[k]; ra.splits[k] = splits[k];
+        ra.wflags[k] = u.wflags[k]; ra.bflags[k] = u.bflags[k];
+        ra.blk0[k] = b0;
+        b0 += (int)(((long)n_out[k] * n_in[k] / 4 + 255) / 256);
+    }
+    ra.blk0[n] = b0;
+    AdamArgs& a = ra.a;
+    a.p = u.p; a.g = nullptr; a.m = u.m; a.v = u.v; a.shadow = static_cast<bf16_t*>(u.shadow_bf16);
+    a.seg = nullptr; a.n_seg = 0;
+    a.dyn = polus_dyn();
+    a.lr = u.lr; a.lr_t = u.lr_t; a.b1 = u.beta1; a.b2 = u.beta2; a.eps = u.eps; a.wd = u.weight_decay;
+    a.gscale = u.grad_scale; a.clip = u.clip_scale;
+    hipLaunchKernelGGL(dw_group_reduce_adam_kernel, dim3(b0), dim3(256), 0, st, ra);
+    POLUS_CHECK_LAUNCH("polus_dense_bwd_params_grouped_update(reduce + AdamW)");
+    return POLUS_OK;
+}
+
 extern "C" size_t polus_sqnorm_workspace_bytes(int64_t n) { return (size_t)sq_blocks(n) * sizeof(float); }
 
 extern "C" int polus_sqnorm(const float* g, int64_t n, float* out, void* workspace, size_t workspace_bytes, void* stream) {
diff --git a/polus_amd/layers.py b/polus_amd/layers.py
--- a/polus_amd/layers.py
+++ b/polus_amd/layers.py
@@ -44,10 +44,10 @@
     return int(max(1, min(want, contraction // 256, 64)))
 
 
-def dense_bwd_params_group(problems, accumulate=False):
+def dense_bwd_params_group(problems, accumulate=False, update=None):
     T = problems[0][0].shape[0]
     if problems[0][0].dtype == torch.bfloat16 and os.environ.get("POLUS_DW_UNGROUPED") is None:
-        return ops.dense_bwd_params_grouped(problems, accumulate, 0)
+        return ops.dense_bwd_params_grouped(problems, accumulate, 0, update)
     for dy, x, dw, db in problems:
         sk = dw_split_k(dy.shape[1], x.shape[1], T)
         if db is not None:
diff --git a/polus_amd/models.py b/polus_amd/models.py
--- a/polus_amd/models.py
+++ b/polus_amd/models.py
@@ -168,7 +168,7 @@
         self._stash = (x, mask, B, S, p_hid, p_att, seeds) if for_backward else None
         return y
 
-    def backward(self, dy, scratch, accumulate=False, side=None):
+    def backward(self, dy, scratch, accumulate=False, side=None, update_hook=None):
         cfg = self.cfg
         H, I, A = cfg.hidden_size, cfg.intermediate_size, cfg.num_attention_heads
         if self._stash is None:
@@ -207,16 +207,26 @@
         else:
             main = torch.cuda.current_stream()
             if not hasattr(self, "_ev"):
-                self._ev = [torch.cuda.Event(), torch.cuda.Event()]
+                self._ev = [torch.cuda.Event(), torch.cuda.Event(), torch.cuda.Event()]
+            update = None
+            if update_hook is not None:
+                update = update_hook([(self.ffn2_w, None), (self.ffn1_w, self.ffn1_b), (self.out_w, None), (self.qkv_w, self.qkv_b)])
             self._ev[0].record(main)
             side.wait_event(self._ev[0])
+            if update is not None:
+                gemm_dx(dqkv, self.qkv_w, dx, resid=dz1)
+                self._ev[2].record(main)
+                update["after"] = self._ev[2]
             with _lib.stream_scope(side):
-                dense_bwd_params_group(problems, accumulate)
+                if dense_bwd_params_group(problems, accumulate, update):
+                    update["done"]()
                 if lnp:
                     ops.layernorm_bwd_finalize(lnp[0], T, H, self.ln2_g.grad, self.ln2_b.grad, self.ffn2_b.grad, accumulate)
                     ops.layernorm_bwd_finalize(lnp[1], T, H, self.ln1_g.grad, self.ln1_b.grad, self.out_b.grad, accumulate)
                 self._ev[1].record(side)
             self.dw_done = self._ev[1]
+            if update is not None:
+                return dx
         gemm_dx(dqkv, self.qkv_w, dx, resid=dz1)
         return dx
 
@@ -265,6 +275,7 @@
     def __init__(self, name=None):
         self._name = name or self.__class__.__name__.lower()
         self.grad_ready_hook = None
+        self.dw_update_hook = None
         self.deterministic = False
         self.savable_config = {}
 
@@ -515,7 +526,7 @@
         for l in reversed(self.layer):
             if len(pending) == 2:
                 retire(pending.pop(0))
-            dy = l.backward(dy, self.scratch, accumulate, side)
+            dy = l.backward(dy, self.scratch, accumulate, side, self.dw_update_hook)
             pending.append(l)
         for lay in pending:
             retire(lay)
diff --git a/polus_amd/ops.py b/polus_amd/ops.py
--- a/polus_amd/ops.py
+++ b/polus_amd/ops.py
@@ -1,3 +1,5 @@
+import ctypes
+
 import torch
 
 from . import _lib
@@ -481,7 +483,11 @@
     check(_lib.load().polus_transpose_bf16(ptr(src), ptr(dst), R, C, _st()), "polus_transpose_bf16")
 
 
-def dense_bwd_params_grouped(problems, accumulate=False, split_k=1):
+DW_FUSED_UPDATE_CALLS = 0
+
+
+def dense_bwd_params_grouped(problems, accumulate=False, split_k=1, update=None):
+    global DW_FUSED_UPDATE_CALLS
     lib = _lib.load()
     T = problems[0][0].shape[0]
     arr = (_lib.DwProblem * len(problems))()
@@ -499,11 +505,30 @@
     if prof is not None:
         e0, e1 = torch.cuda.Event(enable_timing=True), torch.cuda.Event(enable_timing=True)
         e0.record()
-    check(lib.polus_dense_bwd_params_grouped(dt, len(problems), arr, T, 1 if accumulate else 0, int(split_k),
-                                             ptr(ws), ws.numel(), _st()), "polus_dense_bwd_params_grouped")
+    fused = False
+    if update is None:
+        check(lib.polus_dense_bwd_params_grouped(dt, len(problems), arr, T, 1 if accumulate else 0, int(split_k),
+                                                 ptr(ws), ws.numel(), _st()), "polus_dense_bwd_params_grouped")
+    else:
+        u = update
+        _req_cuda(u["grads"], u["params"], u["m"], u["v"], u.get("shadow"))
+        n = len(problems)
+        assert len(u["wflags"]) == n and len(u["bflags"]) == n
+        wf, bf = (ctypes.c_int * n)(*u["wflags"]), (ctypes.c_int * n)(*u["bflags"])
+        after = u.get("after")
+        out = ctypes.c_int(0)
+        check(lib.polus_dense_bwd_params_grouped_update(
+            dt, n, arr, T, 1 if accumulate else 0, int(split_k), ptr(ws), ws.numel(),
+            ptr(u["grads"]), ptr(u["params"]), ptr(u["m"]), ptr(u["v"]), ptr(u.get("shadow")), u["grads"].numel(),
+            wf, bf, float(u["lr"]), float(u["lr_t"]), float(u["beta_1"]), float(u["beta_2"]), float(u["epsilon"]),
+            float(u["weight_decay"]), float(u["grad_scale"]), None, after.cuda_event if after is not None else None,
+            ctypes.byref(out), _st()), "polus_dense_bwd_params_grouped_update")
+        fused = bool(out.value)
+        DW_FUSED_UPDATE_CALLS += fused
     if prof is not None:
         e1.record()
         prof.append(("dw", sum(2.0 * T * p[0].shape[1] * p[1].shape[1] for p in problems), e0, e1))
+    return fused
 
 
 def dense_thin_supported(dtype, H, C):
diff --git a/polus_amd/optimizers.py b/polus_amd/optimizers.py
--- a/polus_amd/optimizers.py
+++ b/polus_amd/optimizers.py
@@ -86,14 +86,25 @@
             self._state[id(arena)] = st
         return st
 
+    def segment_flags(self, v):
+        decay = v.decay and not (self.exclude and self.exclude(v.name))
+        return (1 if (decay and self.weight_decay_rate) else 0) | (2 if v.matrix else 0)
+
+    def step_scalars(self, advance=True):
+        if advance:
+            self._lr_now = self.learning_rate(self.iterations)
+            self.iterations += 1
+        lr = self._lr_now
+        t = self.iterations
+        return lr, lr * math.sqrt(1.0 - self.beta_2 ** t) / (1.0 - self.beta_1 ** t)
+
     def _table(self, arena, variables, ranges=None):
         key = (id(arena), tuple(id(v) for v in variables), tuple(ranges) if ranges is not None else None)
         t = self._tables.get(key)
         if t is None:
             seg = []
             for v in variables:
-                decay = v.decay and not (self.exclude and self.exclude(v.name))
-                flags = (1 if (decay and self.weight_decay_rate) else 0) | (2 if v.matrix else 0)
+                flags = self.segment_flags(v)
                 windows = [(v.offset, v.offset + v.size)]
                 if ranges is not None:
                     windows = [(max(v.offset, lo), min(v.offset + v.size, hi)) for lo, hi in ranges]
@@ -109,12 +120,7 @@
 
     def apply_gradients(self, grads_and_vars, _advance=True, _refresh=True, _ranges=None):
         variables = [v for _, v in grads_and_vars]
-        if _advance:
-            self._lr_now = self.learning_rate(self.iterations)
-            self.iterations += 1
-        lr = self._lr_now
-        t = self.iterations
-        lr_t = lr * math.sqrt(1.0 - self.beta_2 ** t) / (1.0 - self.beta_1 ** t)
+        lr, lr_t = self.step_scalars(_advance)
         arenas = {}
         for v in variables:
             arenas.setdefault(id(v.arena), (v.arena, []))[1].append(v)
diff --git a/polus_amd/training.py b/polus_amd/training.py
--- a/polus_amd/training.py
+++ b/polus_amd/training.py
@@ -6,6 +6,10 @@
 from .context import PolusContext, logger
 
 hvd = comm
+
+
+def dw_update_applies(enabled, variables, left, arena):
+    return bool(enabled and variables and all(id(v) in left and v.arena is arena for v in variables))
 
 
 class _UpdateInBackward:
@@ -16,32 +20,61 @@
         self.stream = torch.cuda.Stream(device=arena.device)
         self.fork, self.done = torch.cuda.Event(), torch.cuda.Event()
         self.vars = sorted(trainer.trainable_weights, key=lambda v: v.offset)
+        self.fuse_dw = os.environ.get("POLUS_DW_FUSED_UPDATE", "1") != "0"
+        self.fused_calls = 0
+        self.windows = True
 
     def begin(self):
         self.first = True
         self.left = {id(v): v for v in self.vars}
-
-    def _apply(self, vs):
+        self.fused = {}
+
+    def dw_update(self, pairs):
+        vs = [v for pr in pairs for v in pr if v is not None]
+        if not dw_update_applies(self.fuse_dw, vs, self.left, self.arena):
+            return None
+        opt = self.trainer.optimizer
+        m, v = opt._slots(self.arena)
+        lr, lr_t = opt.step_scalars(self.first)
+        self.first = False
+
+        def done():
+            for x in vs:
+                self.fused[id(x)] = self.left.pop(id(x))
+            self.fused_calls += 1
+        return {"grads": self.arena.grads, "params": self.arena.params, "m": m, "v": v, "shadow": self.arena.shadow,
+                "wflags": [opt.segment_flags(w) for w, _ in pairs],
+                "bflags": [opt.segment_flags(b) if b is not None else 0 for _, b in pairs],
+                "lr": lr, "lr_t": lr_t, "beta_1": opt.beta_1, "beta_2": opt.beta_2, "epsilon": opt.epsilon,
+                "weight_decay": opt.weight_decay_rate, "grad_scale": opt.grad_scale, "done": done}
+
+    def _apply(self, vs, fused=()):
         import torch
         main = torch.cuda.current_stream()
         self.fork.record(main)
         self.stream.wait_event(self.fork)
         with _lib.stream_scope(self.stream):
-            self.trainer.optimizer.apply_gradients([(v.grad, v) for v in vs], _advance=self.first, _refresh=False)
-            self.arena.refresh_transposed_of(vs)
-        self.first = False
+            if vs:
+                self.trainer.optimizer.apply_gradients([(v.grad, v) for v in vs], _advance=self.first, _refresh=False)
+                self.first = False
+            self.arena.refresh_transposed_of(list(vs) + list(fused))
         for v in vs:
             del self.left[id(v)]
+        for v in fused:
+            del self.fused[id(v)]
 
     def on_ready(self, lo, hi, variables=None):
+        if not self.windows:
+            return
         vs = [v for v in (variables or ()) if id(v) in self.left]
-        if vs:
-            self._apply(vs)
+        fz = [v for v in (variables or ()) if id(v) in self.fused]
+        if vs or fz:
+            self._apply(vs, fz)
 
     def finish(self):
         import torch
-        if self.left:
-            self._apply(list(self.left.values()))
+        if self.left or self.fused:
+            self._apply(list(self.left.values()), list(self.fused.values()))
         with _lib.stream_scope(self.stream):
             self.done.record(self.stream)
         torch.cuda.current_stream().wait_event(self.done)
@@ -164,6 +197,20 @@
             tokens = getattr(self.model, "tokens_per_step", None)
             if tokens is not None and tokens < 6144:
                 return None
+        if u is not None:
+            u.windows = True
+        return u
+
+    def _updater_dw_only(self):
+        if "POLUS_UPDATE_IN_BACKWARD" in os.environ or os.environ.get("POLUS_DW_FUSED_UPDATE_SMALL", "1") == "0":
+            return None
+        tokens = getattr(self.model, "tokens_per_step", None)
+        if tokens is None or tokens >= 6144 or self._updater() is not None:
+            return None
+        u = getattr(self, "_updater_cached", None)
+        if not u or not u.fuse_dw:
+            return None
+        u.windows = False
         return u
 
     def _updater_dp(self, reducer):
@@ -233,11 +280,13 @@
                     self.optimizer.grad_scale = 1.0 / (hvd.size() * accum)
                     dp_updater.begin()
                     r.on_launched = dp_updater.on_bucket
-        updater = self._updater() if (last and not self.use_horovod) else None
+        updater = (self._updater() or self._updater_dw_only()) if (last and not self.use_horovod) else None
         if updater is not None:
             self.optimizer.grad_scale = 1.0 / accum
             updater.begin()
             self.model.grad_ready_hook = updater.on_ready
+            if hasattr(self.model, "dw_update_hook"):
+                self.model.dw_update_hook = updater.dw_update
         reserve = bool(reducers) and getattr(self, "reserve_cus_in_backward", True)
         if reserve:
             from . import ops
@@ -251,6 +300,8 @@
         self._exposed_mark(0)
         if updater is not None:
             self.model.grad_ready_hook = None
+            if hasattr(self.model, "dw_update_hook"):
+                self.model.dw_update_hook = None
             updater.finish()
             return loss_value
         if not last:
```
